# achraf-15/neural_image_compression

Hardware: AMD Instinct MI355X
Metric: images/sec (256x256 RGB, batch 32) fwd+bwd (higher is better)
Workload: dtype f32; 1 GPU; cfg2: JointAutoregressiveHierarchical(M=192,K=1) fwd+rd_loss(lambda=0.01)+bwd+Adam, 32x3x256x256 per GPU, fp32; global_batch=32, parallelism=dp1, step=eager (autograd)

## Files before the change

### include/lic.h

```cpp
#ifndef LIC_H
#define LIC_H

#include <stddef.h>
#include <stdint.h>

#ifdef __cplusplus
extern "C" {
#endif

#define LIC_ABI_VERSION 4

typedef void* lic_stream_t;

enum lic_status {
  LIC_OK = 0,
  LIC_ERR_INVALID = -1,
  LIC_ERR_UNSUPPORTED = -2,
  LIC_ERR_LAUNCH = -3,
  LIC_ERR_WORKSPACE = -4
};

enum lic_epilogue {
  LIC_EPI_NONE = 0,
  LIC_EPI_LEAKY = 1,
// ... 143 lines not shown
                    const float* x_hat, const float* x, int64_t nx, int32_t B, int64_t num_pixels,
                    float lambda_rd, float* out, void* workspace, size_t workspace_bytes,
                    lic_stream_t stream);
int lic_rd_loss_bwd(const float* x_hat, const float* x, int64_t ny, int64_t nz, int64_t nx,
                    int32_t B, int64_t num_pixels, float lambda_rd, const float* gl, float* dlogp_y,
                    float* dlogp_z, float* dx_hat, lic_stream_t stream);
int lic_rd_loss_fwd_lam(const float* logp_y, int64_t ny, const float* logp_z, int64_t nz, const float* x_hat, const float* x,
                        int64_t nx, int32_t B, int64_t num_pixels, const float* lambda_img, float* out, void* workspace,
                        size_t workspace_bytes, lic_stream_t stream);
int lic_rd_loss_bwd_lam(const float* x_hat, const float* x, int64_t ny, int64_t nz, int64_t nx, int32_t B,
                        int64_t num_pixels, const float* lambda_img, const float* gl, float* dlogp_y, float* dlogp_z,
                        float* dx_hat, lic_stream_t stream);

int64_t lic_packed_weight_bf16_elems(int32_t taps, int32_t K, int32_t N);
int lic_pack_weight_bf16(const float* src, void* dst, int32_t taps, int32_t K, int32_t N, int64_t s_tap,
                         int64_t s_k, int64_t s_n, lic_stream_t stream);
int lic_igemm_bf16(const lic_igemm_desc* d, int32_t out_f32, lic_stream_t stream);
size_t lic_igemm_bf16_workspace_bytes(const lic_igemm_desc* d);
int lic_igemm_bf16_fused_gdn_supported(int32_t Cin, int32_t Cout);
int lic_stem_gdn_bf16_supported(int32_t Cin, int32_t Cout, int32_t kh, int32_t kw, int32_t stride, int32_t pad);
int64_t lic_stem_weight_bf16_elems(int32_t Cout);
int lic_pack_stem_weight_bf16(const float* w, void* dst, int32_t Cout, lic_stream_t stream);
int lic_stem_gdn_bf16(const float* x, const void* w_packed, const float* bias, const void* gamma_packed,
                      const float* beta_eff, void* y, void* conv_out, void* norm, int32_t B, int32_t H, int32_t W,
                      int32_t Cout, int32_t inverse, lic_stream_t stream);
int lic_pack_weight_bf16_kperm(const float* src, void* dst, int32_t taps, int32_t K, int32_t N, int64_t s_tap,
                               int64_t s_k, int64_t s_n, lic_stream_t stream);
int lic_igemm_bf16_kernel_name(const lic_igemm_desc* d, char* buf, size_t n);
int lic_wgrad_bf16_kernel_name(const lic_wgrad_desc* d, char* buf, size_t n);
size_t lic_wgrad_bf16_workspace_bytes(const lic_wgrad_desc* d);
int lic_wgrad_bf16(const lic_wgrad_desc* d, void* workspace, size_t workspace_bytes, lic_stream_t stream);
int lic_im2col_bf16(const float* x, void* col, int32_t B, int32_t H, int32_t W, int32_t C, int32_t Ho,
                    int32_t Wo, int32_t kh, int32_t kw, int32_t stride, int32_t pad, int32_t Kpad,
                    lic_stream_t stream);
int lic_col2im_bf16(const void* col, const float* bias, float* out, int32_t B, int32_t Hi, int32_t Wi,
                    int32_t C, int32_t Ho, int32_t Wo, int32_t kh, int32_t kw, int32_t stride, int32_t pad,
                    int32_t Kpad, lic_stream_t stream);
int lic_gdn_bwd_bf16_supported(int32_t C);
int64_t lic_gdn_bwd_bf16_partial_rows(int64_t P);
int lic_gdn_bwd_bf16(const void* g, const void* x, const void* norm, const void* gamma_packed, void* dx, void* t,
                     float* colsum_t_partial, float* colsum_dx_partial, int64_t P, int32_t C, int32_t inverse,
                     lic_stream_t stream);
int lic_gdn_bwd_bf16_recompute(const void* g, const void* x, const void* gamma_packed, const void* gammaT_packed,
                               const float* beta_eff, void* dx, void* t, float* colsum_t_partial,
                               float* colsum_dx_partial, int64_t P, int32_t C, int32_t inverse, lic_stream_t stream);
int lic_colsum2_bf16(const void* in_a, const void* in_b, int64_t ld, int64_t P, int32_t C, float scale, float* out_a,
                     float* out_b, void* workspace, size_t workspace_bytes, lic_stream_t stream);
size_t lic_colsum_bf16_workspace_bytes(int64_t P, int32_t C);
int lic_colsum_bf16(const void* in, int64_t ld, int64_t P, int32_t C, float scale, float* out,
                    void* workspace, size_t workspace_bytes, lic_stream_t stream);
int lic_leaky_bwd_bf16(const void* y, const void* dy, void* dx, int64_t n, float slope, lic_stream_t stream);
int lic_gdn_dnorm_bf16(const void* g, const void* x, const void* norm, void* t, int64_t n, int32_t inverse,
                       lic_stream_t stream);
int lic_quantize_bf16(const float* v, const float* u, float* out, void* v_bf16, void* out_bf16, int64_t n,
                      int32_t training, lic_stream_t stream);
int lic_quantize_anchor_bf16(const float* v, const float* u, float* out, float* out_anchor, void* v_bf16, void* out_bf16,
                             void* anchor_bf16, int32_t B, int32_t h, int32_t w, int32_t C, int32_t training,
                             lic_stream_t stream);

int lic_gdn_supported(int32_t C);
int lic_gdn_fwd(const float* x, const float* gammaT_packed, const float* beta_eff, const float* res, float* y,
                float* norm, int64_t P, int32_t C, int32_t inverse, lic_stream_t stream);
int64_t lic_gdn_bwd_partial_rows(int64_t P);
int lic_gdn_bwd(const float* g, const float* x, const float* norm, const float* gamma_packed, float* dx, float* t,
                float* colsum_t_partial, float* colsum_dx_partial, int64_t P, int32_t C, int32_t inverse,
                lic_stream_t stream);

int lic_factorized_cdf_tables(const float* fe_params, int32_t C, int32_t lo, int32_t S, uint32_t* out,
                              lic_stream_t stream);
int lic_gmm_cdf_tables(const float* params, int64_t P, int32_t M, int32_t K, int32_t W, int32_t* center,
                       uint32_t* out, lic_stream_t stream);

#define LIC_CTX_AUTO 0
#define LIC_CTX_VECTOR 1
#define LIC_CTX_ELEMENT 2
int lic_ctx_gather(const float* y, int64_t y_batch, int64_t y_row, int64_t y_pix, int64_t y_origin, int32_t B,
                   int32_t h, int32_t w, int32_t M, const int32_t* taps, int32_t nt, int32_t slice_rows,
                   const int64_t* pix, int64_t n, float* win, const float* psi, int32_t Cpsi, float* comb,
                   int64_t comb_ld, int32_t path, lic_stream_t stream);

#define LIC_CTX_IMAGE_WORDS 8
#define LIC_CTX_IMAGE_Y_BASE 0
#define LIC_CTX_IMAGE_Y_ROW 1
#define LIC_CTX_IMAGE_Y_ORIGIN 2
#define LIC_CTX_IMAGE_PSI_BASE 3
#define LIC_CTX_IMAGE_H 4
#define LIC_CTX_IMAGE_W 5
#define LIC_CTX_IMAGE_R 6
int lic_ctx_gather_ragged(const float* y, int64_t y_len, int64_t y_pix, const int64_t* images, int32_t nimg, int32_t M,
                          const int32_t* taps, int32_t nt, const int64_t* row_image, const int64_t* row_pix,
                          int64_t rows, float* win, const float* psi, int64_t psi_len, int32_t Cpsi, float* comb,
                          int64_t comb_ld, int32_t path, lic_stream_t stream);

#define LIC_MAX_LAYERS 4
typedef struct lic_ctx_layer {
  float* win;
  float* comb;
  int64_t comb_ld;
  int32_t c0, M;
} lic_ctx_layer;
int lic_ctx_gather_layers(const float* y, int64_t y_batch, int64_t y_row, int64_t y_pix, int64_t y_origin, int32_t B,
                          int32_t h, int32_t w, const int32_t* taps, int32_t nt, int32_t slice_rows, const int64_t* pix,
                          int64_t n, const float* psi, int32_t Cpsi, const lic_ctx_layer* layers, int32_t L,
                          int32_t path, lic_stream_t stream);

int lic_ctx_gather_layers_ragged(const float* y, int64_t y_len, int64_t y_pix, const int64_t* images, int32_t nimg,
                                 const int32_t* taps, int32_t nt, const int64_t* row_image, const int64_t* row_pix,
                                 int64_t rows, const float* psi, int64_t psi_len, int32_t Cpsi,
                                 const lic_ctx_layer* layers, int32_t L, int32_t path, lic_stream_t stream);

#define LIC_RANS_LANES 64
#define LIC_RANS_STATE_WORDS 67
#define LIC_RANS_ERR_RANGE 1u
#define LIC_RANS_ERR_STREAM 2u
int lic_rans_decode_step(const uint8_t* streams, const int64_t* stream_off, const int64_t* stream_bytes,
                         const uint32_t* escapes, const int64_t* esc_off, uint32_t* state, const uint32_t* tables,
                         const int32_t* center, int32_t B, int32_t n, int32_t M, int32_t W, const int64_t* dest,
                         float* ypad, int64_t pixels, lic_stream_t stream);

#define LIC_RANS_MAX_GROUPS 8
int lic_rans_decode_step_groups(const uint8_t* streams, const int64_t* stream_off, const int64_t* stream_bytes,
                                const uint32_t* escapes, const int64_t* esc_off, uint32_t* state,
                                const uint32_t* tables, const int32_t* center, int32_t B, int32_t G, int32_t n,
                                int32_t M, int32_t W, const int64_t* dest, float* ypad, int64_t pixels,
                                lic_stream_t stream);

int lic_rans_decode_step_ragged(const uint8_t* streams, const int64_t* stream_off, const int64_t* stream_bytes,
                                const uint32_t* escapes, const int64_t* esc_off, uint32_t* state,
                                const uint32_t* tables, const int32_t* center, const int32_t* seg, int32_t nimg,
                                int32_t G, int64_t total_rows, int32_t M, int32_t W, const int64_t* dest, float* ypad,
                                const int64_t* y_base, const int64_t* pixels, int64_t ypad_len, lic_stream_t stream);

typedef struct lic_rans_layer {
  const uint32_t* tables;
  const int32_t* center;
  int32_t c0, M;
} lic_rans_layer;
int lic_rans_decode_step_layers(const uint8_t* streams, const int64_t* stream_off, const int64_t* stream_bytes,
                                const uint32_t* escapes, const int64_t* esc_off, uint32_t* state,
                                const lic_rans_layer* layers, int32_t L, int32_t B, int32_t G, int32_t n, int32_t W,
                                const int64_t* dest, float* ypad, int64_t pixels, int64_t y_pix, lic_stream_t stream);

int lic_rans_decode_step_layers_ragged(const uint8_t* streams, const int64_t* stream_off, const int64_t* stream_bytes,
                                       const uint32_t* escapes, const int64_t* esc_off, uint32_t* state,
                                       const lic_rans_layer* layers, int32_t L, const int32_t* seg, int32_t nimg,
                                       int32_t G, int64_t total_rows, int32_t W, const int64_t* dest, float* ypad,
                                       const int64_t* y_base, const int64_t* pixels, int64_t ypad_len, int64_t y_pix,
                                       lic_stream_t stream);

int lic_rans_encode_pick(const uint32_t* tables, const int32_t* center, const int32_t* y, const int64_t* order,
                         int32_t B, int64_t P, int32_t M, int32_t W, uint32_t* sf, uint32_t* exc, uint32_t* state,
                         lic_stream_t stream);
int lic_rans_encode(const uint32_t* sf, const uint32_t* exc, const int64_t* step_len, int64_t nsteps, int32_t B,
                    int64_t nsym, uint8_t* words, int64_t slot, uint32_t* esc_out, uint32_t* state,
                    lic_stream_t stream);

int lic_rans_encode_groups(const uint32_t* sf, const uint32_t* exc, const int64_t* step_len, int64_t nsteps,
                           int32_t B, int32_t G, int64_t nsym, uint8_t* words, int64_t slot, uint32_t* esc_out,
                           int64_t esc_cap, uint32_t* state, lic_stream_t stream);

#define LIC_RANS_IMAGE_WORDS 4
#define LIC_RANS_IMAGE_ROW0 0
#define LIC_RANS_IMAGE_P 1
#define LIC_RANS_IMAGE_STEP0 2
#define LIC_RANS_IMAGE_NSTEPS 3
#define LIC_RANS_BLOCK_WORDS 4
#define LIC_RANS_BLOCK_WORD_OFF 0
#define LIC_RANS_BLOCK_SLOT 1
#define LIC_RANS_BLOCK_ESC_OFF 2
#define LIC_RANS_BLOCK_ESC_CAP 3
int lic_rans_encode_pick_ragged(const uint32_t* tables, const int32_t* center, const int32_t* y, int64_t total_rows,
                                const int64_t* images, int32_t nimg, const int64_t* row_image, const int64_t* order,
                                int32_t M, int32_t W, uint32_t* sf, uint32_t* exc, uint32_t* state,
                                lic_stream_t stream);
int lic_rans_encode_ragged(const uint32_t* sf, const uint32_t* exc, const int64_t* step_len, int64_t steps_len,
                           const int64_t* images, const int64_t* blocks, int32_t nimg, int32_t G, int64_t total_rows,
                           int32_t M, uint8_t* words, int64_t words_len, uint32_t* esc_out, int64_t esc_len,
                           uint32_t* state, lic_stream_t stream);

#define LIC_RANS_Z_AUTO 0
#define LIC_RANS_Z_RESIDENT 1
#define LIC_RANS_Z_GLOBAL 2
#define LIC_RANS_Z_LDS_BYTES 65536
#define LIC_RANS_Z_MAX_S 4096
#define LIC_RANS_Z_MAX_M 65535
int lic_rans_z_pick(const uint32_t* tables, int32_t M, int32_t lo, int32_t S, const int32_t* z, int64_t n, uint32_t* sf,
                    uint32_t* exc, uint32_t* err, lic_stream_t stream);
int lic_rans_z_decode_path(int32_t M, int32_t S);
int lic_rans_z_decode(const uint8_t* streams, const int64_t* stream_off, const int64_t* stream_bytes,
                      const uint32_t* escapes, const int64_t* esc_off, uint32_t* state, const uint32_t* tables,
                      int32_t M, int32_t lo, int32_t S, int32_t nimg, int32_t G, const int64_t* nsym,
                      const int64_t* z_base, float* z, int64_t z_len, int32_t path, lic_stream_t stream);

size_t lic_msssim_workspace_bytes(int32_t B, int32_t C, int32_t H, int32_t W);
int lic_msssim(const float* x, const float* y, int32_t B, int32_t C, int32_t H, int32_t W, int64_t sb,
               int64_t sc, int64_t sh, int64_t sw, float data_range, float* out, float* level_out,
               void* workspace, size_t workspace_bytes, lic_stream_t stream);
size_t lic_msssim_bwd_workspace_bytes(int32_t B, int32_t C, int32_t H, int32_t W);
int lic_msssim_bwd(const float* x, const float* y, int32_t B, int32_t C, int32_t H, int32_t W, int64_t sb,
                   int64_t sc, int64_t sh, int64_t sw, float data_range, const float* level_out,
                   const void* fwd_workspace, size_t fwd_workspace_bytes, const float* gout, float* dx,
                   void* workspace, size_t workspace_bytes, lic_stream_t stream);

int lic_u8_to_f32(const uint8_t* in, float* out, int64_t n, lic_stream_t stream);
size_t lic_tensor_stats_workspace_bytes(void);
int lic_tensor_stats(const float* x, int64_t n, int32_t nbins, float lo, float hi, double* stats,
                     uint64_t* hist, void* workspace, size_t workspace_bytes, lic_stream_t stream);

enum lic_window_border { LIC_WINDOW_ZERO = 0, LIC_WINDOW_REPLICATE = 1, LIC_WINDOW_REFLECT = 2 };
typedef struct lic_window_job {
  int64_t src_offset;
  int32_t Hs, Ws;
  int32_t y0, x0;
  int32_t flags;
  int32_t reserved;
} lic_window_job;
int lic_window_u8_to_f32(const uint8_t* pool, const lic_window_job* jobs_device, int32_t B, int32_t h, int32_t w,
                         int32_t C, int32_t border, float* out, lic_stream_t stream);
int lic_window_f32(const float* src, int64_t sb, int64_t sc, int64_t sh, int64_t sw, int32_t B, int32_t C,
                   int32_t Hs, int32_t Ws, int32_t y0, int32_t x0, int32_t h, int32_t w, int32_t border, float* out,
                   lic_stream_t stream);

typedef struct lic_resample_job {
  int64_t src_offset;
  int32_t Hs, Ws;
  int32_t Hn, Wn;
  int32_t y0, x0;
  int32_t flags;
  int32_t reserved;
} lic_resample_job;
int lic_resample_u8_to_f32(const uint8_t* pool, const lic_resample_job* jobs_device, int32_t B, int32_t h, int32_t w,
                           int32_t C, float* out, lic_stream_t stream);

enum lic_prep_kind { LIC_PREP_PACK_F32 = 0, LIC_PREP_PACK_BF16 = 1, LIC_PREP_MAP = 2, LIC_PREP_MASK_INPLACE = 3,
                     LIC_PREP_PACK_BF16_KPERM = 4 ,
                     LIC_PREP_PACK_BF16_STEM = 5   };
typedef struct lic_prep_job {
  const float* src;
  void* dst;
  const float* mask;
  int64_t s_tap, s_kq, s_kr, s_nq, s_nr;
  int32_t kind;
  int32_t taps, K, N, kdiv, ndiv;
  int32_t transform;
  float bound, pedestal;
  int32_t cpt, npad, tiled, v4, block0, nblocks;
  int64_t total;
} lic_prep_job;
int64_t lic_prep_plan(lic_prep_job* jobs, int32_t njobs);
int lic_prep_run(const lic_prep_job* jobs_device, int32_t njobs, int64_t total_blocks, lic_stream_t stream);

typedef struct lic_adam_job {
  float* p;
  const float* g;
  float* m;
  float* v;
  int64_t n;
  int32_t block0, nblocks;
} lic_adam_job;
int64_t lic_adam_plan(lic_adam_job* jobs, int32_t njobs);
int lic_adam_run(const lic_adam_job* jobs_device, int32_t njobs, int64_t total_blocks, const float* const* grads_host,
                 double lr, double beta1, double beta2, double eps, double weight_decay, double bias_correction1,
                 double bias_correction2, lic_stream_t stream);

int lic_grad_norm_partial(const lic_adam_job* jobs_device, int32_t njobs, int64_t total_blocks,
                          const float* const* grads_host, double* partials, lic_stream_t stream);
int lic_grad_norm_finish(const double* partials, int64_t nparts, double max_norm, int32_t count_skip, float* clip_state,
                         lic_stream_t stream);
int lic_adam_run_scaled(const lic_adam_job* jobs_device, int32_t njobs, int64_t total_blocks,
                        const float* const* grads_host, double lr, double beta1, double beta2, double eps,
                        double weight_decay, double bias_correction1, double bias_correction2, const float* clip_state,
                        int32_t skip_nonfinite, lic_stream_t stream);

int lic_adam_run_ema(const lic_adam_job* jobs_device, int32_t njobs, int64_t total_blocks,
                     const float* const* grads_host, double lr, double beta1, double beta2, double eps,
                     double weight_decay, double bias_correction1, double bias_correction2, float* const* ema_device,
                     double ema_weight, const float* clip_state, int32_t skip_nonfinite, lic_stream_t stream);
int lic_swap_run(const lic_adam_job* jobs_device, int32_t njobs, int64_t total_blocks, float* const* ema_device,
                 lic_stream_t stream);

enum { LIC_REDUCE_SLABS = 0, LIC_REDUCE_COLUMNS = 1 };
enum { LIC_REDUCE_EPI_NONE = 0, LIC_REDUCE_EPI_REPARAM = 1 };
#define LIC_REDUCE_MAX_JOBS 32
typedef struct lic_reduce_job {
  const float* src;
  float* dst;
  const float* param;
  int64_t sm, smr, sn, snr, stap;
  int32_t kind, epilogue;
  int32_t splitk, ntaps, Cm, Cn, Mvalid, Nvalid, mdiv, ndiv;
  float scale, bound;
  int32_t block0, nblocks;
} lic_reduce_job;
int lic_wgrad_bf16_partial(const lic_wgrad_desc* d, void* workspace, size_t workspace_bytes, lic_reduce_job* job,
                           lic_stream_t stream);
int lic_colsum_bf16_partial(const void* in, int64_t ld, int64_t P, int32_t C, float scale, float* out, void* workspace,
                            size_t workspace_bytes, lic_reduce_job* job, lic_stream_t stream);
int lic_colsum2_bf16_partial(const void* in_a, const void* in_b, int64_t ld, int64_t P, int32_t C, float scale,
                             float* out_a, float* out_b, void* workspace, size_t workspace_bytes, lic_reduce_job* jobs2,
                             lic_stream_t stream);
int lic_leaky_bwd_colsum_bf16(const void* y, const void* dy, void* dx, int64_t P, int32_t C, float slope, float* out,
                              void* workspace, size_t workspace_bytes, lic_reduce_job* job, lic_stream_t stream);
int lic_reduce_batch(const lic_reduce_job* jobs, int32_t njobs, lic_stream_t stream);

int lic_head_convt_bf16_supported(int32_t Cin, int32_t Cout, int32_t kh, int32_t kw, int32_t stride, int32_t pad,
                                  int32_t out_pad);
int lic_head_convt_bf16(const void* x, const void* w_packed, const float* bias, float* out, int32_t B, int32_t Hi,
                        int32_t Wi, int32_t Cin, lic_stream_t stream);
int lic_stem_conv_bf16(const float* x, const void* w_packed, const float* bias, void* y, int32_t B, int32_t H, int32_t W,
                       int32_t Cout, lic_stream_t stream);

typedef struct lic_plan lic_plan;
int lic_plan_create(void* hip_graph, lic_plan** out);
int lic_plan_info(const lic_plan* plan, int64_t* info);
int lic_plan_replay(lic_plan* plan, lic_stream_t main, const lic_stream_t* sides, int32_t n_sides);
int lic_plan_tune(lic_plan* plan, lic_stream_t main, const lic_stream_t* sides, int32_t n_sides, double* result);
int lic_plan_dag(const lic_plan* plan, int64_t cap_ops, int64_t cap_edges, int64_t* sizes, int32_t* pred_ptr,
                 int32_t* pred_idx, int32_t* kind, int32_t* flags, double* us);
int lic_plan_commands(lic_plan* plan, int32_t n_sides, int64_t cap, int64_t* n_cmds, int32_t* cmds);
int lic_plan_sched_host(int64_t n_ops, const int32_t* pred_ptr, const int32_t* pred_idx, const double* us,
                        const int32_t* flags, int32_t mode, int32_t ns, double wide_min_us, int32_t n_sides,
                        int64_t cap, int64_t* n_cmds, int32_t* cmds, int64_t* info);
void lic_plan_destroy(lic_plan* plan);
const char* lic_plan_last_error(void);

int lic_version(void);
int lic_last_hip_error(void);
const char* lic_arch(void);

#ifdef __cplusplus
}
#endif
#endif
```

### neural_image_compression_amd/_lib.py

```python
from __future__ import annotations

import ctypes as C
import os

_HERE = os.path.dirname(os.path.abspath(__file__))
LIB_PATH = os.path.join(_HERE, "liblic_hip.so")

EPI_NONE, EPI_LEAKY, EPI_MUL_LEAKY_MASK, EPI_GDN, EPI_IGDN, EPI_GDN_BWD, EPI_IGDN_BWD, EPI_CONV_GDN, EPI_CONV_IGDN = range(9)
FE_NPARAM = 43

_vp, _i32, _i64, _f32, _sz = C.c_void_p, C.c_int32, C.c_int64, C.c_float, C.c_size_t


class IgemmDesc(C.Structure):
    _fields_ = [("in_", _vp), ("w", _vp), ("bias", _vp), ("out", _vp), ("out2", _vp), ("aux", _vp),
                ("aux2", _vp), ("aux3", _vp), ("res", _vp),
                ("in_ld", _i64), ("out_ld", _i64), ("out2_ld", _i64), ("aux_ld", _i64),
                ("aux2_ld", _i64), ("aux3_ld", _i64), ("res_ld", _i64),
                ("B", _i32), ("Hi", _i32), ("Wi", _i32), ("Cin", _i32),
                ("Ho", _i32), ("Wo", _i32), ("Cout", _i32),
                ("kh", _i32), ("kw", _i32), ("stride", _i32), ("pad", _i32),
                ("transposed", _i32), ("prologue", _i32), ("epilogue", _i32),
                ("tap_mask", C.c_uint32), ("slope", _f32), ("workspace", _vp), ("workspace_bytes", _sz),
                ("out3", _vp), ("out3_ld", _i64),
                ("force_bm", _i32), ("force_tn", _i32), ("force_split", _i32), ("reserved0", _i32)]


class WgradDesc(C.Structure):
    _fields_ = [("p", _vp), ("g", _vp), ("dst", _vp),
                ("p_ld", _i64), ("g_ld", _i64),
                ("dst_sm", _i64), ("dst_sn", _i64), ("dst_stap", _i64),
                ("B", _i32), ("Hs", _i32), ("Ws", _i32), ("Cp", _i32),
                ("Hl", _i32), ("Wl", _i32), ("Cg", _i32),
                ("kh", _i32), ("kw", _i32), ("stride", _i32), ("pad", _i32),
                ("g_is_row", _i32), ("sq_p", _i32), ("sq_g", _i32), ("scale", _f32),
                ("force_tm", _i32), ("force_tn", _i32), ("force_split", _i32)]


PREP_PACK_F32, PREP_PACK_BF16, PREP_MAP, PREP_MASK_INPLACE, PREP_PACK_BF16_KPERM, PREP_PACK_BF16_STEM = range(6)


class PrepJob(C.Structure):
    _fields_ = [("src", _vp), ("dst", _vp), ("mask", _vp),
                ("s_tap", _i64), ("s_kq", _i64), ("s_kr", _i64), ("s_nq", _i64), ("s_nr", _i64),
                ("kind", _i32), ("taps", _i32), ("K", _i32), ("N", _i32), ("kdiv", _i32), ("ndiv", _i32),
                ("transform", _i32), ("bound", _f32), ("pedestal", _f32),
                ("cpt", _i32), ("npad", _i32), ("tiled", _i32), ("v4", _i32), ("block0", _i32), ("nblocks", _i32),
                ("total", _i64)]


REDUCE_SLABS, REDUCE_COLUMNS = 0, 1
REDUCE_EPI_NONE, REDUCE_EPI_REPARAM = 0, 1
REDUCE_MAX_JOBS = 32


class ReduceJob(C.Structure):
    _fields_ = [("src", _vp), ("dst", _vp), ("param", _vp),
                ("sm", _i64), ("smr", _i64), ("sn", _i64), ("snr", _i64), ("stap", _i64),
                ("kind", _i32), ("epilogue", _i32),
                ("splitk", _i32), ("ntaps", _i32), ("Cm", _i32), ("Cn", _i32), ("Mvalid", _i32), ("Nvalid", _i32),
                ("mdiv", _i32), ("ndiv", _i32),
                ("scale", _f32), ("bound", _f32),
                ("block0", _i32), ("nblocks", _i32)]


class AdamJob(C.Structure):
    _fields_ = [("p", _vp), ("g", _vp), ("m", _vp), ("v", _vp), ("n", _i64), ("block0", _i32), ("nblocks", _i32)]


RANS_LANES, RANS_STATE_WORDS, RANS_MAX_GROUPS = 64, 67, 8

CTX_AUTO, CTX_VECTOR, CTX_ELEMENT = range(3)
CTX_IMAGE_WORDS = 8
RANS_IMAGE_WORDS = RANS_BLOCK_WORDS = 4

RANS_Z_AUTO, RANS_Z_RESIDENT, RANS_Z_GLOBAL = range(3)
RANS_Z_MAX_S, RANS_Z_MAX_M, RANS_Z_LDS_BYTES = 4096, 65535, 65536

GAIN_SCALE, GAIN_NOISE, GAIN_ROUND = range(3)
GAIN_SLAB_PIXELS, GAIN_SLAB_ROWS = 32, 4
GAIN_ROWS_MAX_TABLES = 4

MAX_LAYERS = 4


class CtxLayer(C.Structure):
    _fields_ = [("win", _vp), ("comb", _vp), ("comb_ld", _i64), ("c0", _i32), ("M", _i32)]


class RansLayer(C.Structure):
    _fields_ = [("tables", _vp), ("center", _vp), ("c0", _i32), ("M", _i32)]


WINDOW_ZERO, WINDOW_REPLICATE, WINDOW_REFLECT = range(3)
WINDOW_FLIP = 1


class WindowJob(C.Structure):
    _fields_ = [("src_offset", _i64), ("Hs", _i32), ("Ws", _i32), ("y0", _i32), ("x0", _i32), ("flags", _i32),
                ("reserved", _i32)]


class ResampleJob(C.Structure):
    _fields_ = [("src_offset", _i64), ("Hs", _i32), ("Ws", _i32), ("Hn", _i32), ("Wn", _i32), ("y0", _i32),
                ("x0", _i32), ("flags", _i32), ("reserved", _i32)]


SIGNATURES = {
    "lic_igemm": (C.c_int, [C.POINTER(IgemmDesc), _vp]),
    "lic_igemm_workspace_bytes": (_sz, [C.POINTER(IgemmDesc)]),
    "lic_igemm_kernel_name": (C.c_int, [C.POINTER(IgemmDesc), C.c_char_p, _sz]),
    "lic_wgrad_stage": (C.c_int, [C.POINTER(WgradDesc), _vp, _sz, _i32, _vp]),
    "lic_wgrad_kernel_name": (C.c_int, [C.POINTER(WgradDesc), C.c_char_p, _sz]),
    "lic_igemm_plan": (C.c_int, [C.POINTER(IgemmDesc), C.POINTER(_i32), C.POINTER(_i32), C.POINTER(_i64)]),
    "lic_igemm_tile_order": (C.c_int, [C.POINTER(IgemmDesc), _vp, _i64, C.POINTER(_i64), C.POINTER(_i32),
                                       C.POINTER(_i32)]),
    "lic_packed_weight_floats": (_i64, [_i32, _i32, _i32]),
    "lic_pack_weight": (C.c_int, [_vp, _vp, _i32, _i32, _i32, _i64, _i64, _i64, _vp]),
    "lic_wgrad_workspace_bytes": (_sz, [C.POINTER(WgradDesc)]),
    "lic_wgrad": (C.c_int, [C.POINTER(WgradDesc), _vp, _sz, _vp]),
    "lic_wgrad_plan": (C.c_int, [C.POINTER(WgradDesc), C.POINTER(_i32), C.POINTER(_i32), C.POINTER(_i32)]),
    "lic_colsum_workspace_bytes": (_sz, [_i64, _i32]),
    "lic_colsum": (C.c_int, [_vp, _i64, _i64, _i32, _f32, _vp, _vp, _sz, _vp]),
    "lic_permute3": (C.c_int, [_vp, _vp, _i32, _i32, _i32, _i64, _i64, _i64, _i64, _i64, _i64, _vp]),
    "lic_im2col": (C.c_int, [_vp, _vp] + [_i32] * 11 + [_vp]),
    "lic_col2im": (C.c_int, [_vp, _vp, _vp] + [_i32] * 11 + [_vp]),
    "lic_mul_inplace": (C.c_int, [_vp, _vp, _i64, _vp]),
    "lic_leaky_bwd": (C.c_int, [_vp, _vp, _vp, _i64, _f32, _vp]),
    "lic_gdn_reparam": (C.c_int, [_vp, _vp, _i64, _f32, _f32, _vp]),
    "lic_gdn_reparam_bwd": (C.c_int, [_vp, _vp, _vp, _i64, _f32, _vp]),
    "lic_gdn_reparam_bwd2": (C.c_int, [_vp, _vp, _vp, _i64, _f32, _vp, _vp, _vp, _i64, _f32, _vp]),
    "lic_gdn_dnorm": (C.c_int, [_vp, _vp, _vp, _vp, _i64, _i32, _vp]),
    "lic_quantize": (C.c_int, [_vp, _vp, _vp, _i64, _i32, _vp]),
    "lic_quantize_anchor": (C.c_int, [_vp, _vp, _vp, _vp, _i32, _i32, _i32, _i32, _i32, _vp]),
    "lic_anchor_add": (C.c_int, [_vp, _vp, _vp, _i32, _i32, _i32, _i32, _vp]),
    "lic_gain_quantize": (C.c_int, [_vp, _vp, _vp, _i64] + [_vp] * 6 + [_i32] * 5 + [_vp]),
    "lic_gain_bwd_workspace_bytes": (_sz, [_i32, _i64, _i32]),
    "lic_gain_bwd": (C.c_int, [_vp, _vp, _i64] + [_vp] * 5 + [_i32] * 4 + [_vp, _sz, _vp]),
    "lic_gain_rows_fwd": (C.c_int, [_vp] * 4 + [_i32] * 4 + [_vp]),
    "lic_gain_rows_bwd": (C.c_int, [_vp] * 7 + [_i32] * 4 + [_vp]),
    "lic_entropy_params_fwd": (C.c_int, [_vp, _vp, _i64, _i32, _i32, _vp]),
    "lic_entropy_params_bwd": (C.c_int, [_vp, _vp, _vp, _vp, _i64, _i32, _i32, _vp]),
    "lic_gmm_likelihood_fwd": (C.c_int, [_vp, _vp, _vp, _vp, _i64, _i32, _i32, _f32, _vp]),
    "lic_gmm_likelihood_bwd": (C.c_int, [_vp, _vp, _vp, _vp, _vp, _vp, _i64, _i32, _i32, _f32, _vp]),
    "lic_factorized_fwd": (C.c_int, [_vp, _vp, _vp, _vp, _i64, _i32, _f32, _vp]),
    "lic_factorized_bwd": (C.c_int, [_vp, _vp, _vp, _vp, _vp, _vp, _i64, _i32, _f32, _vp]),
    "lic_factorized_channel_logits": (C.c_int, [_vp, _i32, _vp, _vp, _i64, _vp]),
    "lic_fe_pack": (C.c_int, [_vp, _vp, _i32, _vp]),
    "lic_fe_unpack": (C.c_int, [_vp, _vp, _i32, _vp]),
    "lic_rd_loss_workspace_bytes": (_sz, [_i32]),
    "lic_rd_loss_fwd": (C.c_int, [_vp, _i64, _vp, _i64, _vp, _vp, _i64, _i32, _i64, _f32, _vp, _vp, _sz, _vp]),
    "lic_rd_loss_bwd": (C.c_int, [_vp, _vp, _i64, _i64, _i64, _i32, _i64, _f32, _vp, _vp, _vp, _vp, _vp]),
    "lic_rd_loss_fwd_lam": (C.c_int, [_vp, _i64, _vp, _i64, _vp, _vp, _i64, _i32, _i64, _vp, _vp, _vp, _sz, _vp]),
    "lic_rd_loss_bwd_lam": (C.c_int, [_vp, _vp, _i64, _i64, _i64, _i32, _i64, _vp, _vp, _vp, _vp, _vp, _vp]),
    "lic_packed_weight_bf16_elems": (_i64, [_i32, _i32, _i32]),
    "lic_pack_weight_bf16": (C.c_int, [_vp, _vp, _i32, _i32, _i32, _i64, _i64, _i64, _vp]),
    "lic_pack_weight_bf16_kperm": (C.c_int, [_vp, _vp, _i32, _i32, _i32, _i64, _i64, _i64, _vp]),
    "lic_igemm_bf16": (C.c_int, [C.POINTER(IgemmDesc), _i32, _vp]),
    "lic_igemm_bf16_kernel_name": (C.c_int, [C.POINTER(IgemmDesc), C.c_char_p, _sz]),
    "lic_igemm_bf16_workspace_bytes": (_sz, [C.POINTER(IgemmDesc)]),
    "lic_igemm_bf16_fused_gdn_supported": (C.c_int, [_i32, _i32]),
    "lic_stem_gdn_bf16_supported": (C.c_int, [_i32] * 6),
    "lic_stem_weight_bf16_elems": (C.c_int64, [_i32]),
    "lic_pack_stem_weight_bf16": (C.c_int, [_vp, _vp, _i32, _vp]),
    "lic_stem_gdn_bf16": (C.c_int, [_vp] * 8 + [_i32] * 5 + [_vp]),
    "lic_wgrad_bf16_kernel_name": (C.c_int, [C.POINTER(WgradDesc), C.c_char_p, _sz]),
    "lic_wgrad_bf16_workspace_bytes": (_sz, [C.POINTER(WgradDesc)]),
    "lic_wgrad_bf16": (C.c_int, [C.POINTER(WgradDesc), _vp, _sz, _vp]),
    "lic_im2col_bf16": (C.c_int, [_vp, _vp] + [_i32] * 11 + [_vp]),
    "lic_col2im_bf16": (C.c_int, [_vp, _vp, _vp] + [_i32] * 11 + [_vp]),
    "lic_colsum_bf16_workspace_bytes": (_sz, [_i64, _i32]),
    "lic_colsum_bf16": (C.c_int, [_vp, _i64, _i64, _i32, _f32, _vp, _vp, _sz, _vp]),
    "lic_quantize_bf16": (C.c_int, [_vp, _vp, _vp, _vp, _vp, _i64, _i32, _vp]),
    "lic_quantize_anchor_bf16": (C.c_int, [_vp] * 7 + [_i32] * 5 + [_vp]),
    "lic_wgrad_bf16_partial": (C.c_int, [C.POINTER(WgradDesc), _vp, _sz, C.POINTER(ReduceJob), _vp]),
    "lic_colsum_bf16_partial": (C.c_int, [_vp, _i64, _i64, _i32, _f32, _vp, _vp, _sz, C.POINTER(ReduceJob), _vp]),
    "lic_colsum2_bf16_partial": (C.c_int, [_vp, _vp, _i64, _i64, _i32, _f32, _vp, _vp, _vp, _sz, C.POINTER(ReduceJob), _vp]),
    "lic_reduce_batch": (C.c_int, [C.POINTER(ReduceJob), _i32, _vp]),
    "lic_colsum2_bf16": (C.c_int, [_vp, _vp, _i64, _i64, _i32, _f32, _vp, _vp, _vp, _sz, _vp]),
    "lic_gdn_dnorm_bf16": (C.c_int, [_vp, _vp, _vp, _vp, _i64, _i32, _vp]),
    "lic_gdn_bwd_bf16_supported": (C.c_int, [_i32]),
    "lic_gdn_bwd_bf16_partial_rows": (_i64, [_i64]),
    "lic_gdn_bwd_bf16": (C.c_int, [_vp, _vp, _vp, _vp, _vp, _vp, _vp, _vp, _i64, _i32, _i32, _vp]),
    "lic_gdn_bwd_bf16_recompute": (C.c_int, [_vp, _vp, _vp, _vp, _vp, _vp, _vp, _vp, _vp, _i64, _i32, _i32, _vp]),
    "lic_leaky_bwd_bf16": (C.c_int, [_vp, _vp, _vp, _i64, _f32, _vp]),
    "lic_leaky_bwd_colsum_bf16": (C.c_int, [_vp, _vp, _vp, _i64, _i32, _f32, _vp, _vp, _sz, C.POINTER(ReduceJob), _vp]),
    "lic_igemm_fused_gdn_supported": (C.c_int, [_i32, _i32]),
    "lic_igemm_fused_gdn_preferred": (C.c_int, [C.POINTER(IgemmDesc)]),
    "lic_gdn_supported": (C.c_int, [_i32]),
    "lic_gdn_fwd": (C.c_int, [_vp, _vp, _vp, _vp, _vp, _vp, _i64, _i32, _i32, _vp]),
    "lic_gdn_bwd_partial_rows": (_i64, [_i64]),
    "lic_gdn_bwd": (C.c_int, [_vp, _vp, _vp, _vp, _vp, _vp, _vp, _vp, _i64, _i32, _i32, _vp]),
    "lic_factorized_cdf_tables": (C.c_int, [_vp, _i32, _i32, _i32, _vp, _vp]),
    "lic_gmm_cdf_tables": (C.c_int, [_vp, _i64, _i32, _i32, _i32, _vp, _vp, _vp]),
    "lic_rans_decode_step": (C.c_int, [_vp] * 8 + [_i32] * 4 + [_vp, _vp, _i64, _vp]),
    "lic_rans_encode_pick": (C.c_int, [_vp] * 4 + [_i32, _i64, _i32, _i32] + [_vp] * 4),
    "lic_rans_encode": (C.c_int, [_vp] * 3 + [_i64, _i32, _i64, _vp, _i64, _vp, _vp, _vp]),
    "lic_rans_decode_step_groups": (C.c_int, [_vp] * 8 + [_i32] * 5 + [_vp, _vp, _i64, _vp]),
    "lic_rans_encode_groups": (C.c_int, [_vp] * 3 + [_i64, _i32, _i32, _i64, _vp, _i64, _vp, _i64, _vp, _vp]),
    "lic_rans_encode_pick_ragged": (C.c_int, [_vp] * 3 + [_i64, _vp, _i32, _vp, _vp, _i32, _i32] + [_vp] * 4),
    "lic_rans_encode_ragged": (C.c_int, [_vp] * 3 + [_i64, _vp, _vp, _i32, _i32, _i64, _i32, _vp, _i64, _vp, _i64,
                                         _vp, _vp]),
    "lic_ctx_gather": (C.c_int, [_vp] + [_i64] * 4 + [_i32] * 4 + [_vp, _i32, _i32, _vp, _i64, _vp, _vp, _i32, _vp, _i64,
                                 _i32, _vp]),
    "lic_ctx_gather_ragged": (C.c_int, [_vp, _i64, _i64, _vp, _i32, _i32, _vp, _i32, _vp, _vp, _i64, _vp, _vp, _i64, _i32,
                                        _vp, _i64, _i32, _vp]),
    "lic_rans_decode_step_ragged": (C.c_int, [_vp] * 9 + [_i32, _i32, _i64, _i32, _i32, _vp, _vp, _vp, _vp, _i64, _vp]),
    "lic_ctx_gather_layers": (C.c_int, [_vp] + [_i64] * 4 + [_i32] * 3 + [_vp, _i32, _i32, _vp, _i64, _vp, _i32,
                                        C.POINTER(CtxLayer), _i32, _i32, _vp]),
    "lic_rans_decode_step_layers": (C.c_int, [_vp] * 6 + [C.POINTER(RansLayer)] + [_i32] * 5 + [_vp, _vp, _i64, _i64,
                                                                                                 _vp]),
    "lic_ctx_gather_layers_ragged": (C.c_int, [_vp, _i64, _i64, _vp, _i32, _vp, _i32, _vp, _vp, _i64, _vp, _i64, _i32,
                                               C.POINTER(CtxLayer), _i32, _i32, _vp]),
    "lic_rans_decode_step_layers_ragged": (C.c_int, [_vp] * 6 + [C.POINTER(RansLayer), _i32, _vp, _i32, _i32, _i64,
                                                                 _i32, _vp, _vp, _vp, _vp, _i64, _i64, _vp]),
    "lic_rans_z_pick": (C.c_int, [_vp, _i32, _i32, _i32, _vp, _i64, _vp, _vp, _vp, _vp]),
    "lic_rans_z_decode_path": (C.c_int, [_i32, _i32]),
    "lic_rans_z_decode": (C.c_int, [_vp] * 7 + [_i32] * 5 + [_vp, _vp, _vp, _i64, _i32, _vp]),
    "lic_msssim_workspace_bytes": (_sz, [_i32, _i32, _i32, _i32]),
    "lic_msssim": (C.c_int, [_vp, _vp, _i32, _i32, _i32, _i32, _i64, _i64, _i64, _i64, _f32, _vp, _vp, _vp, _sz,
                             _vp]),
    "lic_msssim_bwd_workspace_bytes": (_sz, [_i32, _i32, _i32, _i32]),
    "lic_msssim_bwd": (C.c_int, [_vp, _vp, _i32, _i32, _i32, _i32, _i64, _i64, _i64, _i64, _f32, _vp, _vp, _sz, _vp,
                                 _vp, _vp, _sz, _vp]),
    "lic_u8_to_f32": (C.c_int, [_vp, _vp, _i64, _vp]),
    "lic_window_u8_to_f32": (C.c_int, [_vp, _vp, _i32, _i32, _i32, _i32, _i32, _vp, _vp]),
    "lic_window_f32": (C.c_int, [_vp, _i64, _i64, _i64, _i64] + [_i32] * 9 + [_vp, _vp]),
    "lic_resample_u8_to_f32": (C.c_int, [_vp, _vp, _i32, _i32, _i32, _i32, _vp, _vp]),
    "lic_tensor_stats_workspace_bytes": (_sz, []),
    "lic_tensor_stats": (C.c_int, [_vp, _i64, _i32, _f32, _f32, _vp, _vp, _vp, _sz, _vp]),
    "lic_prep_plan": (_i64, [C.POINTER(PrepJob), _i32]),
    "lic_prep_run": (C.c_int, [_vp, _i32, _i64, _vp]),
    "lic_adam_plan": (_i64, [C.POINTER(AdamJob), _i32]),
    "lic_adam_run": (C.c_int, [_vp, _i32, _i64, _vp] + [C.c_double] * 7 + [_vp]),
    "lic_grad_norm_partial": (C.c_int, [_vp, _i32, _i64, _vp, _vp, _vp]),
    "lic_grad_norm_finish": (C.c_int, [_vp, _i64, C.c_double, _i32, _vp, _vp]),
    "lic_adam_run_scaled": (C.c_int, [_vp, _i32, _i64, _vp] + [C.c_double] * 7 + [_vp, _i32, _vp]),
    "lic_adam_run_ema": (C.c_int, [_vp, _i32, _i64, _vp] + [C.c_double] * 7 + [_vp, C.c_double, _vp, _i32, _vp]),
    "lic_swap_run": (C.c_int, [_vp, _i32, _i64, _vp, _vp]),
    "lic_head_convt_bf16_supported": (C.c_int, [_i32] * 7),
    "lic_head_convt_bf16": (C.c_int, [_vp, _vp, _vp, _vp, _i32, _i32, _i32, _i32, _vp]),
    "lic_stem_conv_bf16": (C.c_int, [_vp, _vp, _vp, _vp, _i32, _i32, _i32, _i32, _vp]),
    "lic_plan_create": (C.c_int, [_vp, C.POINTER(C.c_void_p)]),
    "lic_plan_info": (C.c_int, [_vp, C.POINTER(C.c_int64)]),
    "lic_plan_replay": (C.c_int, [_vp, _vp, C.POINTER(C.c_void_p), _i32]),
    "lic_plan_tune": (C.c_int, [_vp, _vp, C.POINTER(C.c_void_p), _i32, C.POINTER(C.c_double)]),
    "lic_plan_dag": (C.c_int, [_vp, _i64, _i64, C.POINTER(C.c_int64), _vp, _vp, _vp, _vp, _vp]),
    "lic_plan_commands": (C.c_int, [_vp, _i32, _i64, C.POINTER(C.c_int64), _vp]),
    "lic_plan_sched_host": (C.c_int, [_i64, _vp, _vp, _vp, _vp, _i32, _i32, C.c_double, _i32, _i64,
                                      C.POINTER(C.c_int64), _vp, _vp]),
    "lic_plan_destroy": (None, [_vp]),
    "lic_plan_last_error": (C.c_char_p, []),
    "lic_version": (C.c_int, []),
    "lic_last_hip_error": (C.c_int, []),
    "lic_arch": (C.c_char_p, []),
}

_lib = None


class LicError(RuntimeError):
    pass


def load():
    global _lib
    if _lib is None:
        if not os.path.exists(LIB_PATH):
            raise LicError(
                f"{LIB_PATH} not found: the HIP extension is not built. Run "
                "`python -c 'import __graft_entry__ as g; g.build()'` (or make -C "
                "neural_image_compression_amd/csrc). There is no CPU fallback.")
        lib = C.CDLL(LIB_PATH)
        for name, (res, args) in SIGNATURES.items():
            fn = getattr(lib, name)
            fn.restype = res
            fn.argtypes = args
        _lib = lib
    return _lib


_STATUS = {-1: "LIC_ERR_INVALID", -2: "LIC_ERR_UNSUPPORTED", -3: "LIC_ERR_LAUNCH", -4: "LIC_ERR_WORKSPACE"}


def check(rc: int, what: str):
    if rc != 0:
        extra = f" (hipError {load().lic_last_hip_error()})" if rc == -3 else ""
        raise LicError(f"{what} failed: {_STATUS.get(rc, rc)}{extra}")
```

### neural_image_compression_amd/csrc/lic_elementwise.hip

```cpp
#include "lic_common.h"
#include "lic_patch.h"

#define EW_BLOCK 256
static bool al16(const void* p) { return (reinterpret_cast<uintptr_t>(p) & 15) == 0; }

__global__ __launch_bounds__(EW_BLOCK) void permute3_kernel(const float* src, float* dst, int n0, int n1,
                                                            int n2, long s0, long s1, long s2, long d0,
                                                            long d1, long d2) {
  const long total = (long)n0 * n1 * n2;
  for (long i = (long)blockIdx.x * EW_BLOCK + threadIdx.x; i < total; i += (long)gridDim.x * EW_BLOCK) {
    const int k = (int)(i % n2);
    const long t = i / n2;
    const int j = (int)(t % n1);
    const int a = (int)(t / n1);
    dst[a * d0 + j * d1 + k * d2] = src[a * s0 + j * s1 + k * s2];
  }
}
LIC_EXPORT int lic_permute3(const float* src, float* dst, int32_t n0, int32_t n1, int32_t n2,
                            int64_t s0, int64_t s1, int64_t s2, int64_t d0, int64_t d1, int64_t d2,
                            lic_stream_t stream) {
  if (!src || !dst || n0 <= 0 || n1 <= 0 || n2 <= 0) return LIC_ERR_INVALID;
  const long total = (long)n0 * n1 * n2;
  hipLaunchKernelGGL(permute3_kernel, dim3(ew_grid(total, EW_BLOCK)), dim3(EW_BLOCK), 0,
                     (hipStream_t)stream, src, dst, n0, n1, n2, (long)s0, (long)s1, (long)s2, (long)d0,
                     (long)d1, (long)d2);
  return lic_check_launch();
}

__global__ __launch_bounds__(EW_BLOCK) void im2col_kernel(const float* x, float* col, int B, int H, int W,
                                                          int C, int Ho, int Wo, int kh, int kw,
                                                          int stride, int pad, int Kpad) {
  const long total = (long)B * Ho * Wo * Kpad;
  const int K = kh * kw * C;
  for (long i = (long)blockIdx.x * EW_BLOCK + threadIdx.x; i < total; i += (long)gridDim.x * EW_BLOCK) {
    const int k = (int)(i % Kpad);
    const long pix = i / Kpad;
    float v = 0.0f;
    if (k < K) {
      const int c = k % C, tap = k / C;
      const int r = tap / kw, s = tap - r * kw;
      const int ow = (int)(pix % Wo);
      const long t = pix / Wo;
      const int oh = (int)(t % Ho);
      const int b = (int)(t / Ho);
      const int ih = oh * stride - pad + r, iw = ow * stride - pad + s;
      if (ih >= 0 && iw >= 0 && ih < H && iw < W) v = x[(((long)b * H + ih) * W + iw) * C + c];
    }
    col[i] = v;
  }
}
LIC_EXPORT int lic_im2col(const float* x, float* col, int32_t B, int32_t H, int32_t W, int32_t C,
                          int32_t Ho, int32_t Wo, int32_t kh, int32_t kw, int32_t stride, int32_t pad,
                          int32_t Kpad, lic_stream_t stream) {
  if (!x || !col || B <= 0 || H <= 0 || W <= 0 || C <= 0 || Ho <= 0 || Wo <= 0 || Kpad < kh * kw * C)
    return LIC_ERR_INVALID;
  const long total = (long)B * Ho * Wo * Kpad;
  if (Kpad <= LIC_PATCH_MAXK && Kpad % 4 == 0 && total / 4 < 0x7FFFFFFFL && al16(col) && kh < 256 && kw < 256 &&
      C < 256 && (long)H * W * C < 0x7FFFFFFFL)
    hipLaunchKernelGGL((im2col_vec_kernel<float, 4>), dim3(ew_grid(total / 4, 256)), dim3(256), 0,
                       (hipStream_t)stream, x, col, (unsigned)((long)B * Ho * Wo), H, W, C, Ho, Wo, kh, kw, stride, pad,
                       Kpad);
  else
    hipLaunchKernelGGL(im2col_kernel, dim3(ew_grid(total, EW_BLOCK)), dim3(EW_BLOCK), 0,
                       (hipStream_t)stream, x, col, B, H, W, C, Ho, Wo, kh, kw, stride, pad, Kpad);
  return lic_check_launch();
}

__global__ __launch_bounds__(EW_BLOCK) void col2im_kernel(const float* col, const float* bias, float* out,
                                                          int B, int Hi, int Wi, int C, int Ho, int Wo,
                                                          int kh, int kw, int stride, int pad, int Kpad) {
  const long total = (long)B * Ho * Wo * C;
  for (long i = (long)blockIdx.x * EW_BLOCK + threadIdx.x; i < total; i += (long)gridDim.x * EW_BLOCK) {
    const int c = (int)(i % C);
    const long pix = i / C;
    const int ox = (int)(pix % Wo);
    const long t = pix / Wo;
    const int oy = (int)(t % Ho);
    const int b = (int)(t / Ho);
    float v = bias ? bias[c] : 0.0f;
    for (int r = 0; r < kh; ++r) {
      const int nh = oy + pad - r;
      if (nh < 0 || (nh % stride) != 0) continue;
      const int ih = nh / stride;
      if (ih >= Hi) continue;
      for (int s = 0; s < kw; ++s) {
        const int nw = ox + pad - s;
        if (nw < 0 || (nw % stride) != 0) continue;
        const int iw = nw / stride;
        if (iw >= Wi) continue;
        v += col[(((long)b * Hi + ih) * Wi + iw) * Kpad + (r * kw + s) * C + c];
      }
    }
    out[i] = v;
  }
}
LIC_EXPORT int lic_col2im(const float* col, const float* bias, float* out, int32_t B, int32_t Hi,
                          int32_t Wi, int32_t C, int32_t Ho, int32_t Wo, int32_t kh, int32_t kw,
                          int32_t stride, int32_t pad, int32_t Kpad, lic_stream_t stream) {
  if (!col || !out || B <= 0 || Hi <= 0 || Wi <= 0 || C <= 0 || Ho <= 0 || Wo <= 0 || stride < 1 ||
      Kpad < kh * kw * C)
    return LIC_ERR_INVALID;
  const long total = (long)B * Ho * Wo * C;
  if (total < 0x7FFFFFFFL && (long)B * Hi * Wi < 0x7FFFFFFFL)
    hipLaunchKernelGGL((col2im_fast_kernel<float>), dim3(ew_grid(total, 256)), dim3(256), 0, (hipStream_t)stream, col,
                       bias, out, (unsigned)total, Hi, Wi, C, Ho, Wo, kh, kw, stride, pad, Kpad);
  else
    hipLaunchKernelGGL(col2im_kernel, dim3(ew_grid(total, EW_BLOCK)), dim3(EW_BLOCK), 0,
                       (hipStream_t)stream, col, bias, out, B, Hi, Wi, C, Ho, Wo, kh, kw, stride, pad, Kpad);
  return lic_check_launch();
}

#define CS_MAXCHUNK 256
__global__ __launch_bounds__(256) void colsum_stage1(const float* in, long ld, long P, int C, float* part,
                                                     int nchunk, int vec) {
  __shared__ float red[16][64 + 4];
  const int cg = threadIdx.x & 15, ry = threadIdx.x >> 4;
  const int c = blockIdx.x * 64 + cg * 4;
  f32x4 acc = {0.f, 0.f, 0.f, 0.f};
  if (c < C) {
    if (vec) {
      for (long pr = (long)blockIdx.y * 16 + ry; pr < P; pr += (long)nchunk * 16)
        acc += *reinterpret_cast<const f32x4*>(in + pr * ld + c);
    } else {
      for (long pr = (long)blockIdx.y * 16 + ry; pr < P; pr += (long)nchunk * 16)
#pragma unroll
        for (int e = 0; e < 4; ++e)
          if (c + e < C) acc[e] += in[pr * ld + c + e];
    }
  }
#pragma unroll
  for (int e = 0; e < 4; ++e) red[ry][cg * 4 + e] = acc[e];
  __syncthreads();
  if (threadIdx.x < 64) {
    const int cc = blockIdx.x * 64 + threadIdx.x;
    float s = 0.0f;
#pragma unroll
    for (int r = 0; r < 16; ++r) s += red[r][threadIdx.x];
    if (cc < C) part[(long)blockIdx.y * C + cc] = s;
  }
}
__global__ __launch_bounds__(256) void colsum3_stage1(const float* in, long P, float* part, int nchunk) {
  __shared__ float red[4][3];
  const long ngroup = P / 4;
  f32x4 a0 = {0.f, 0.f, 0.f, 0.f}, a1 = a0, a2 = a0;
  for (long g = (long)blockIdx.x * 256 + threadIdx.x; g < ngroup; g += (long)nchunk * 256) {
    const f32x4* q = reinterpret_cast<const f32x4*>(in + g * 12);
    a0 += q[0];
    a1 += q[1];
    a2 += q[2];
  }
  float c0 = a0[0] + a0[3] + a1[2] + a2[1];
  float c1 = a0[1] + a1[0] + a1[3] + a2[2];
  float c2 = a0[2] + a1[1] + a2[0] + a2[3];
  if (blockIdx.x == 0 && threadIdx.x == 0)
    for (long r = ngroup * 4; r < P; ++r) {
      c0 += in[r * 3];
      c1 += in[r * 3 + 1];
      c2 += in[r * 3 + 2];
    }
  c0 = wave_sum(c0);
  c1 = wave_sum(c1);
  c2 = wave_sum(c2);
  const int w = threadIdx.x >> 6;
  if ((threadIdx.x & 63) == 0) {
    red[w][0] = c0;
    red[w][1] = c1;
    red[w][2] = c2;
  }
  __syncthreads();
  if (threadIdx.x < 3)
    part[(long)blockIdx.x * 3 + threadIdx.x] =
        (red[0][threadIdx.x] + red[1][threadIdx.x]) + (red[2][threadIdx.x] + red[3][threadIdx.x]);
}
__global__ __launch_bounds__(256) void colsum_stage2(const float* part, int C, int nchunk, float scale,
                                                     float* out) {
  __shared__ double red[16][17];
  const int cx = threadIdx.x & 15, ly = threadIdx.x >> 4;
  const int c = blockIdx.x * 16 + cx;
  double acc = 0.0;
  if (c < C)
    for (int y = ly; y < nchunk; y += 16) acc += (double)part[(long)y * C + c];
  red[ly][cx] = acc;
  __syncthreads();
  if (ly == 0 && c < C) {
    double t = 0.0;
#pragma unroll
    for (int q = 0; q < 16; ++q) t += red[q][cx];
    out[c] = (float)(t * (double)scale);
  }
}
static int colsum_chunks(int64_t P) {
  int64_t n = cdiv64(P, 16 * 8);
  if (n > CS_MAXCHUNK) n = CS_MAXCHUNK;
  if (n < 1) n = 1;
  return (int)n;
}
LIC_EXPORT size_t lic_colsum_workspace_bytes(int64_t P, int32_t C) {
  if (P <= 0 || C <= 0) return 0;
  return (size_t)colsum_chunks(P) * C * sizeof(float);
}
LIC_EXPORT int lic_colsum(const float* in, int64_t ld, int64_t P, int32_t C, float scale, float* out,
                          void* workspace, size_t workspace_bytes, lic_stream_t stream) {
  if (!in || !out || !workspace || P <= 0 || C <= 0) return LIC_ERR_INVALID;
  const int nchunk = colsum_chunks(P);
  if (workspace_bytes < (size_t)nchunk * C * sizeof(float)) return LIC_ERR_WORKSPACE;
  hipStream_t s = (hipStream_t)stream;
  const int vec = (C % 4 == 0) && (ld % 4 == 0) && al16(in);
  if (C == 3 && ld == 3 && al16(in))
    hipLaunchKernelGGL(colsum3_stage1, dim3(nchunk), dim3(256), 0, s, in, (long)P, (float*)workspace, nchunk);
  else
    hipLaunchKernelGGL(colsum_stage1, dim3((C + 63) / 64, nchunk), dim3(256), 0, s, in, (long)ld, (long)P, C,
                       (float*)workspace, nchunk, vec);
  int rc = lic_check_launch();
  if (rc != LIC_OK) return rc;
  hipLaunchKernelGGL(colsum_stage2, dim3((C + 15) / 16), dim3(256), 0, s, (const float*)workspace, C,
                     nchunk, scale, out);
  return lic_check_launch();
}

template <typename F>
__global__ __launch_bounds__(EW_BLOCK) void ew_kernel(long n, F f) {
  for (long i = (long)blockIdx.x * EW_BLOCK + threadIdx.x; i < n; i += (long)gridDim.x * EW_BLOCK) f(i);
}
template <typename F>
static int ew_launch(long n, lic_stream_t stream, F f) {
  if (n <= 0) return LIC_OK;
  hipLaunchKernelGGL((ew_kernel<F>), dim3(ew_grid(n, EW_BLOCK)), dim3(EW_BLOCK), 0, (hipStream_t)stream, n, f);
  return lic_check_launch();
}
template <typename F4, typename F1>
static int ew_launch_vec(long n, bool can_vec, lic_stream_t stream, F4 f4, F1 f1) {
  if (n <= 0) return LIC_OK;
  if (!can_vec) return ew_launch(n, stream, f1);
  const long n4 = n / 4;
  int rc = ew_launch(n4, stream, f4);
  if (rc != LIC_OK) return rc;
  const long tail0 = n4 * 4;
  if (tail0 < n) return ew_launch(n - tail0, stream, [=] __device__(long i) { f1(tail0 + i); });
  return LIC_OK;
}

LIC_EXPORT int lic_mul_inplace(float* w, const float* mask, int64_t n, lic_stream_t stream) {
  if (!w || !mask || n < 0) return LIC_ERR_INVALID;
  return ew_launch(n, stream, [=] __device__(long i) { w[i] *= mask[i]; });
}

LIC_EXPORT int lic_leaky_bwd(const float* y, const float* dy, float* dx, int64_t n, float slope,
                             lic_stream_t stream) {
  if (!y || !dy || !dx || n < 0) return LIC_ERR_INVALID;
  return ew_launch_vec(
      n, al16(y) && al16(dy) && al16(dx), stream,
      [=] __device__(long i) {
        const f32x4 a = reinterpret_cast<const f32x4*>(y)[i], g = reinterpret_cast<const f32x4*>(dy)[i];
        f32x4 o;
#pragma unroll
        for (int e = 0; e < 4; ++e) o[e] = a[e] > 0.0f ? g[e] : g[e] * slope;
        reinterpret_cast<f32x4*>(dx)[i] = o;
      },
      [=] __device__(long i) { dx[i] = y[i] > 0.0f ? dy[i] : dy[i] * slope; });
}

LIC_EXPORT int lic_gdn_reparam(const float* p, float* out, int64_t n, float bound, float pedestal,
                               lic_stream_t stream) {
  if (!p || !out || n < 0) return LIC_ERR_INVALID;
  return ew_launch(n, stream, [=] __device__(long i) { out[i] = lic_reparam(p[i], bound, pedestal); });
}
LIC_EXPORT int lic_gdn_reparam_bwd(const float* p, const float* dout, float* dp, int64_t n, float bound,
                                   lic_stream_t stream) {
  if (!p || !dout || !dp || n < 0) return LIC_ERR_INVALID;
  return ew_launch(n, stream, [=] __device__(long i) {
    const float v = p[i] > bound ? p[i] : bound;
    const float g = dout[i] * 2.0f * v;
    dp[i] = (p[i] >= bound || g < 0.0f) ? g : 0.0f;
  });
}

LIC_EXPORT int lic_gdn_reparam_bwd2(const float* pb, const float* dob, float* dpb, int64_t nb, float bound_b,
                                    const float* pg, const float* dog, float* dpg, int64_t ng, float bound_g,
                                    lic_stream_t stream) {
  if (nb < 0 || ng < 0 || (nb > 0 && (!pb || !dob || !dpb)) || (ng > 0 && (!pg || !dog || !dpg))) return LIC_ERR_INVALID;
  if (nb + ng == 0) return LIC_OK;
  return ew_launch(nb + ng, stream, [=] __device__(long i) {
    const bool isb = i < nb;
    const long j = isb ? i : i - nb;
    const float pv = isb ? pb[j] : pg[j], dv = isb ? dob[j] : dog[j], bound = isb ? bound_b : bound_g;
    const float v = pv > bound ? pv : bound;
    const float g = dv * 2.0f * v;
    (isb ? dpb : dpg)[j] = (pv >= bound || g < 0.0f) ? g : 0.0f;
  });
}

__device__ __forceinline__ float gdn_t1(float g, float x, float n, int inverse) {
  const float rs = __builtin_amdgcn_rsqf(n);
  return inverse ? 0.5f * g * x * rs : -0.5f * g * x * rs * (rs * rs);
}
LIC_EXPORT int lic_gdn_dnorm(const float* g, const float* x, const float* norm, float* t, int64_t n,
                             int32_t inverse, lic_stream_t stream) {
  if (!g || !x || !norm || !t || n < 0) return LIC_ERR_INVALID;
  return ew_launch_vec(
      n, al16(g) && al16(x) && al16(norm) && al16(t), stream,
      [=] __device__(long i) {
        const f32x4 gv = reinterpret_cast<const f32x4*>(g)[i], xv = reinterpret_cast<const f32x4*>(x)[i],
                    nv = reinterpret_cast<const f32x4*>(norm)[i];
        f32x4 o;
#pragma unroll
        for (int e = 0; e < 4; ++e) o[e] = gdn_t1(gv[e], xv[e], nv[e], inverse);
        reinterpret_cast<f32x4*>(t)[i] = o;
      },
      [=] __device__(long i) { t[i] = gdn_t1(g[i], x[i], norm[i], inverse); });
}

LIC_EXPORT int lic_quantize(const float* v, const float* u, float* out, int64_t n, int32_t training,
                            lic_stream_t stream) {
  if (!v || !out || n < 0 || (training && !u)) return LIC_ERR_INVALID;
  if (training) return ew_launch(n, stream, [=] __device__(long i) { out[i] = v[i] + (u[i] - 0.5f); });
  return ew_launch(n, stream, [=] __device__(long i) { out[i] = rintf(v[i]); });
}

__device__ __forceinline__ bool lic_is_anchor(long pix, int h, int w) {
  const long row = pix / w;
  return (((row % h) + (pix - row * w)) & 1) == 0;
}
LIC_EXPORT int lic_quantize_anchor(const float* v, const float* u, float* out, float* out_anchor, int32_t B, int32_t h,
                                   int32_t w, int32_t C, int32_t training, lic_stream_t stream) {
  if (!v || !out || !out_anchor || B <= 0 || h <= 0 || w <= 0 || C <= 0 || (training && !u)) return LIC_ERR_INVALID;
  const long n = (long)B * h * w * C;
  return ew_launch(n, stream, [=] __device__(long i) {
    const float q = training ? v[i] + (u[i] - 0.5f) : rintf(v[i]);
    out[i] = q;
    out_anchor[i] = lic_is_anchor(i / C, h, w) ? q : 0.0f;
  });
}
LIC_EXPORT int lic_anchor_add(const float* g, const float* g_anchor, float* out, int32_t B, int32_t h, int32_t w, int32_t C,
                              lic_stream_t stream) {
  if (!g || !g_anchor || !out || B <= 0 || h <= 0 || w <= 0 || C <= 0) return LIC_ERR_INVALID;
  const long n = (long)B * h * w * C;
  return ew_launch_vec(
      n, C % 4 == 0 && al16(g) && al16(g_anchor) && al16(out), stream,
      [=] __device__(long i) {
        const f32x4 a = reinterpret_cast<const f32x4*>(g)[i];
        f32x4 b = {};
        if (lic_is_anchor(4 * i / C, h, w)) b = reinterpret_cast<const f32x4*>(g_anchor)[i];
        reinterpret_cast<f32x4*>(out)[i] = a + b;
      },
      [=] __device__(long i) { out[i] = g[i] + (lic_is_anchor(i / C, h, w) ? g_anchor[i] : 0.0f); });
}

#define LIC_MAXK 8
LIC_EXPORT int lic_entropy_params_fwd(const float* raw, float* out, int64_t P, int32_t M, int32_t K,
                                      lic_stream_t stream) {
  if (!raw || !out || P <= 0 || M <= 0 || K < 1 || K > LIC_MAXK) return LIC_ERR_INVALID;
  const long CH = (long)(K == 1 ? 2 : 3) * K * M;
  const long T = (long)K * M;
  return ew_launch(P * M, stream, [=] __device__(long i) {
    const long pix = i / M;
    const int m = (int)(i - pix * M);
    const float* r = raw + pix * CH;
    float* o = out + pix * CH;
    if (K == 1) {
      o[m] = r[m];
      o[M + m] = lic_softplus(r[M + m]) + 1e-6f;
    } else {
      float mx = -INFINITY;
      for (int k = 0; k < K; ++k) mx = fmaxf(mx, r[k * M + m]);
      float den = 0.0f;
      for (int k = 0; k < K; ++k) den += expf(r[k * M + m] - mx);
      for (int k = 0; k < K; ++k) {
        o[k * M + m] = expf(r[k * M + m] - mx) / den;
        o[T + k * M + m] = r[T + k * M + m];
        o[2 * T + k * M + m] = lic_softplus(r[2 * T + k * M + m]) + 1e-6f;
      }
    }
  });
}
LIC_EXPORT int lic_entropy_params_bwd(const float* raw, const float* out, const float* dout, float* draw,
                                      int64_t P, int32_t M, int32_t K, lic_stream_t stream) {
  if (!raw || !out || !dout || !draw || P <= 0 || M <= 0 || K < 1 || K > LIC_MAXK) return LIC_ERR_INVALID;
  const long CH = (long)(K == 1 ? 2 : 3) * K * M;
  const long T = (long)K * M;
  return ew_launch(P * M, stream, [=] __device__(long i) {
    const long pix = i / M;
    const int m = (int)(i - pix * M);
    const float* r = raw + pix * CH;
    const float* o = out + pix * CH;
    const float* g = dout + pix * CH;
    float* d = draw + pix * CH;
    if (K == 1) {
      d[m] = g[m];
      d[M + m] = g[M + m] * lic_softplus_grad(r[M + m]);
    } else {
      float dot = 0.0f;
      for (int k = 0; k < K; ++k) dot += g[k * M + m] * o[k * M + m];
      for (int k = 0; k < K; ++k) {
        d[k * M + m] = o[k * M + m] * (g[k * M + m] - dot);
        d[T + k * M + m] = g[T + k * M + m];
        d[2 * T + k * M + m] = g[2 * T + k * M + m] * lic_softplus_grad(r[2 * T + k * M + m]);
      }
    }
  });
}

__device__ __forceinline__ float gauss_cdf(float t) { return 0.5f * (1.0f + erff(t / 1.41421356237309515f)); }
__device__ __forceinline__ float gauss_pdf(float t) { return 0.398942280401432678f * expf(-0.5f * t * t); }

LIC_EXPORT int lic_gmm_likelihood_fwd(const float* x, const float* params, float* p, float* logp, int64_t P,
                                      int32_t M, int32_t K, float bound, lic_stream_t stream) {
  if (!x || !params || !p || !logp || P <= 0 || M <= 0 || K < 1 || K > LIC_MAXK) return LIC_ERR_INVALID;
  const long CH = (long)(K == 1 ? 2 : 3) * K * M;
  const long T = (long)K * M;
  return ew_launch(P * M, stream, [=] __device__(long i) {
    const long pix = i / M;
    const int m = (int)(i - pix * M);
    const float* q = params + pix * CH;
    const float xv = x[i];
    float acc = 0.0f;
    for (int k = 0; k < K; ++k) {
      const float mu = (K == 1) ? q[m] : q[T + k * M + m];
      const float sg = (K == 1) ? q[M + m] : q[2 * T + k * M + m];
      const float up = (xv + 0.5f - mu) / sg, lo = (xv - 0.5f - mu) / sg;
      const float mass = gauss_cdf(up) - gauss_cdf(lo);
      acc = (K == 1) ? mass : acc + q[k * M + m] * mass;
    }
    const float pc = acc > bound ? acc : bound;
    p[i] = pc;
    logp[i] = logf(pc);
  });
}
LIC_EXPORT int lic_gmm_likelihood_bwd(const float* x, const float* params, const float* dp,
                                      const float* dlogp, float* dx, float* dparams, int64_t P, int32_t M,
                                      int32_t K, float bound, lic_stream_t stream) {
  if (!x || !params || !dx || !dparams || P <= 0 || M <= 0 || K < 1 || K > LIC_MAXK) return LIC_ERR_INVALID;
  const long CH = (long)(K == 1 ? 2 : 3) * K * M;
  const long T = (long)K * M;
  return ew_launch(P * M, stream, [=] __device__(long i) {
    const long pix = i / M;
    const int m = (int)(i - pix * M);
    const float* q = params + pix * CH;
    float* dq = dparams + pix * CH;
    const float xv = x[i];
    float acc = 0.0f;
    for (int k = 0; k < K; ++k) {
      const float mu = (K == 1) ? q[m] : q[T + k * M + m];
      const float sg = (K == 1) ? q[M + m] : q[2 * T + k * M + m];
      const float up = (xv + 0.5f - mu) / sg, lo = (xv - 0.5f - mu) / sg;
      const float mass = gauss_cdf(up) - gauss_cdf(lo);
      acc = (K == 1) ? mass : acc + q[k * M + m] * mass;
    }
    const float pc = acc > bound ? acc : bound;
    float g = 0.0f;
    if (dp) g += dp[i];
    if (dlogp) g += dlogp[i] / pc;
    if (!(acc >= bound)) g = 0.0f;
    float dxa = 0.0f;
    for (int k = 0; k < K; ++k) {
      const float mu = (K == 1) ? q[m] : q[T + k * M + m];
      const float sg = (K == 1) ? q[M + m] : q[2 * T + k * M + m];
      const float up = (xv + 0.5f - mu) / sg, lo = (xv - 0.5f - mu) / sg;
      const float pu = gauss_pdf(up), pl = gauss_pdf(lo);
      const float wk = (K == 1) ? 1.0f : q[k * M + m];
      const float gm = g * wk;
      if (K == 1) {
        dq[m] = -gm * (pu - pl) / sg;
        dq[M + m] = -gm * (pu * up - pl * lo) / sg;
      } else {
        dq[k * M + m] = g * (gauss_cdf(up) - gauss_cdf(lo));
        dq[T + k * M + m] = -gm * (pu - pl) / sg;
        dq[2 * T + k * M + m] = -gm * (pu * up - pl * lo) / sg;
      }
      dxa += gm * (pu - pl) / sg;
    }
    dx[i] = dxa;
  });
}

__constant__ int FE_MOFF[4] = {0, 3, 12, 21};
__constant__ int FE_BOFF[4] = {24, 27, 30, 33};
__constant__ int FE_FOFF[3] = {34, 37, 40};
__constant__ int FE_DIN[4] = {1, 3, 3, 3};
__constant__ int FE_DOUT[4] = {3, 3, 3, 1};

struct FeTrace {
  float h[4][3];
  float pre[4][3];
};
__device__ __forceinline__ float fe_logits(const float* T, float v, FeTrace* tr) {
  float h[3] = {v, 0.0f, 0.0f};
#pragma unroll
  for (int i = 0; i < 4; ++i) {
    const int din = (i == 0) ? 1 : 3, dout = (i == 3) ? 1 : 3;
    const int mo = (i == 0) ? 0 : (i == 1) ? 3 : (i == 2) ? 12 : 21;
    const int bo = 24 + 3 * i;
    float pre[3] = {0.0f, 0.0f, 0.0f};
#pragma unroll
    for (int o = 0; o < 3; ++o)
      if (o < dout) {
        float acc = 0.0f;
#pragma unroll
        for (int k = 0; k < 3; ++k)
          if (k < din) acc += T[mo + o * din + k] * h[k];
        pre[o] = acc + T[bo + o];
      }
    if (tr) {
#pragma unroll
      for (int k = 0; k < 3; ++k) {
        tr->h[i][k] = h[k];
        tr->pre[i][k] = pre[k];
      }
    }
    if (i < 3) {
#pragma unroll
      for (int o = 0; o < 3; ++o) h[o] = pre[o] + T[34 + 3 * i + o] * tanhf(pre[o]);
    } else {
      h[0] = pre[0];
    }
  }
  return h[0];
}
__device__ __forceinline__ float fe_logits_bwd(const float* T, const float* R, const FeTrace& tr,
                                               float dlogit, float* dP) {
  float dh[3] = {dlogit, 0.0f, 0.0f};
// ... 495 lines not shown
```

### neural_image_compression_amd/csrc/lic_gemm.hip

```cpp
#include "lic_tile_map.h"
#include <stdio.h>
#include <stdlib.h>
#include <algorithm>
#include <type_traits>

thread_local int g_lic_last_hip_error = 0;

struct IgemmParams {
  const float* in;
  const float* w;
  const float* bias;
  float* out;
  float* out2;
  const float* aux;
  const float* aux2;
  const float* aux3;
  const float* res;
  float* out3;
  long in_ld, out_ld, out2_ld, aux_ld, aux2_ld, aux3_ld, res_ld, out3_ld;
  int B, Hi, Wi, Cin, Ho, Wo, Cout;
  int kw, stride, pad, transposed, prologue, epilogue;
  float slope;
  int vec;
  int vec_out;
// ... 1204 lines not shown
      load_chunk(c_begin + c + 3);
      compute(1);
      __syncthreads();
    }
    if (c < nloc) {
      compute(0);
      __syncthreads();
    }
  }
  float* slab = p.slabs + ((long)split * p.ntaps + tap) * p.row.C * p.col.C;
#pragma unroll
  for (int a = 0; a < TM; ++a)
#pragma unroll
    for (int q = 0; q < 16; ++q) {
      const int m = m0 + wm0 + a * 32 + (q & 3) + 8 * (q >> 2) + 4 * lh;
      if (m >= p.row.C) continue;
#pragma unroll
      for (int b = 0; b < TN; ++b) {
        const int n = n0 + wn0 + b * 32 + li;
        if (n < p.col.C) slab[(long)m * p.col.C + n] = acc[a][b][q];
      }
    }
}

template <int TM, int TN, bool SQB = false, bool FULL = true>
__global__ __launch_bounds__(256, (TM * TN >= 6 ? 2 : 1)) void wgrad_glds_kernel(const WgradParams p) {
  constexpr int BMt = 64 * TM, BNt = 64 * TN, NS = TM + TN;
  constexpr int WM = BMt / 2, WN = BNt / 2;
  __shared__ __attribute__((aligned(16))) float smem[2][NS][WG_BK * 64];
  const int tid = threadIdx.x, lane = tid & 63;
  const int wave = __builtin_amdgcn_readfirstlane(tid >> 6);
  const int wm0 = (wave >> 1) * WM, wn0 = (wave & 1) * WN;
  const int li = lane & 31, lh = lane >> 5;
  const WgradTile wt = wgrad_tile(p, xcd_contiguous(blockIdx.x, gridDim.x), BMt, BNt);
  const int m0 = wt.m0, n0 = wt.n0, tap = wt.tap, split = wt.split;
  const int c_begin = wt.c_begin, c_end = wt.c_end, nloc = c_end - c_begin;

  f32x16 acc[TM][TN];
#pragma unroll
  for (int a = 0; a < TM; ++a)
#pragma unroll
    for (int b = 0; b < TN; ++b)
#pragma unroll
      for (int q = 0; q < 16; ++q) acc[a][b][q] = 0.0f;

  const int kr = tid >> 4, c16 = (tid & 15) * 4;
  constexpr unsigned WG_OOB = 0x80000000u, WG_GBIAS = 0x40000000u;
  const unsigned row_ld4 = (unsigned)p.row.ld * 4u, col_ld4 = (unsigned)p.col.ld * 4u;
  const unsigned row_lin = (unsigned)kr * row_ld4 + (unsigned)c16 * 4u;
  const unsigned col_lin = (unsigned)kr * col_ld4 + (unsigned)c16 * 4u;
  const bool row_g = p.row.gathered != 0, col_g = p.col.gathered != 0;
  const unsigned g_ld4 = row_g ? row_ld4 : col_ld4;
  const unsigned HWl = (unsigned)(p.Hl * p.Wl);
  const int tap_h = wt.r - p.pad, tap_w = wt.s - p.pad;
  bool row_live[TM], col_live[TN];
#pragma unroll
  for (int j = 0; j < TM; ++j) row_live[j] = FULL || m0 + c16 + 64 * j < p.row.C;
#pragma unroll
  for (int j = 0; j < TN; ++j) col_live[j] = FULL || n0 + c16 + 64 * j < p.col.C;
  const float* const row_base = p.row.ptr + m0;
  const float* const col_base = p.col.ptr + n0;
  auto issue = [&](int c, int buf) {
    const int cc = c < c_end ? c : c_end - 1;
    const int pk0 = cc * WG_BK;
    const int b0 = fdiv(pk0, p.dHW);
    const int rem0 = pk0 - b0 * p.Hs * p.Ws;
    const int hs0 = fdiv(rem0, p.dW), ws0 = rem0 - hs0 * p.Ws;
    const long g0 = ((long)b0 * p.Hl + (hs0 * p.stride + tap_h)) * p.Wl + (ws0 * p.stride + tap_w);
    const unsigned pk = (unsigned)pk0 + (unsigned)kr;
    const int pix = pk < (unsigned)p.Ps ? (int)pk : 0;
    const int b = fdiv(pix, p.dHW);
    const int rem = pix - b * p.Hs * p.Ws;
    const int hs = fdiv(rem, p.dW), ws = rem - hs * p.Ws;
    const int hl = hs * p.stride + tap_h, wl = ws * p.stride + tap_w;
    const bool gok = pk < (unsigned)p.Ps && (unsigned)hl < (unsigned)p.Hl && (unsigned)wl < (unsigned)p.Wl;
    const unsigned dpix = (unsigned)b * HWl + (unsigned)hl * (unsigned)p.Wl + (unsigned)wl - (unsigned)g0;
    const unsigned gokm = (unsigned)(-(int)gok);
    const unsigned g_off = ((dpix * g_ld4 + (WG_GBIAS + (unsigned)c16 * 4u)) & gokm) | (~gokm & WG_OOB);
    const long left = p.Ps - pk0;
    const unsigned lin_rec = (unsigned)(left < WG_BK ? left : WG_BK);
    auto rsrc = [&](const float* base, long ld, unsigned ld4, bool gathered) {
      const long px = gathered ? g0 : (long)pk0;
      const float* b_ = base + (px * ld - (gathered ? (long)(WG_GBIAS / 4) : 0L));
      return __builtin_amdgcn_make_buffer_rsrc(const_cast<float*>(b_), 0, gathered ? (int)WG_OOB : (int)(lin_rec * ld4),
                                               0x00020000);
    };
    const __amdgpu_buffer_rsrc_t rs_row = rsrc(row_base, p.row.ld, row_ld4, row_g);
    const __amdgpu_buffer_rsrc_t rs_col = rsrc(col_base, p.col.ld, col_ld4, col_g);
    const unsigned row_off = row_g ? g_off : row_lin, col_off = col_g ? g_off : col_lin;
#pragma unroll
    for (int j = 0; j < TM; ++j)
      __builtin_amdgcn_raw_ptr_buffer_load_lds(rs_row, (lic_lptr_t)&smem[buf][j][wave * 256], 16,
                                               (int)(row_live[j] ? row_off : WG_OOB), 256 * j, 0, 0);
#pragma unroll
    for (int j = 0; j < TN; ++j)
      __builtin_amdgcn_raw_ptr_buffer_load_lds(rs_col, (lic_lptr_t)&smem[buf][TM + j][wave * 256], 16,
                                               (int)(col_live[j] ? col_off : WG_OOB), 256 * j, 0, 0);
  };
  auto compute = [&](int buf) {
    float af[TM][8], bf[TN][8];
#pragma unroll
    for (int a = 0; a < TM; ++a) {
      const int ch = wm0 + a * 32;
#pragma unroll
      for (int t = 0; t < 8; ++t) af[a][t] = smem[buf][ch >> 6][(lh * 8 + t) * 64 + (ch & 63) + li];
    }
#pragma unroll
    for (int b = 0; b < TN; ++b) {
      const int ch = wn0 + b * 32;
#pragma unroll
      for (int t = 0; t < 8; ++t) {
        const float v = smem[buf][TM + (ch >> 6)][(lh * 8 + t) * 64 + (ch & 63) + li];
        bf[b][t] = SQB ? v * v : v;
      }
    }
#pragma unroll
    for (int t = 0; t < 8; ++t)
#pragma unroll
      for (int a = 0; a < TM; ++a)
#pragma unroll
        for (int b = 0; b < TN; ++b)
          acc[a][b] = __builtin_amdgcn_mfma_f32_32x32x2f32(af[a][t], bf[b][t], acc[a][b], 0, 0, 0);
  };

  if (nloc > 0) {
    issue(c_begin, 0);
    int c = 0;
    for (; c + 1 < nloc; c += 2) {
      __syncthreads();
      issue(c_begin + c + 1, 1);
      compute(0);
      __builtin_amdgcn_sched_barrier(0);
      __syncthreads();
      issue(c_begin + c + 2, 0);
      compute(1);
      __builtin_amdgcn_sched_barrier(0);
    }
    __syncthreads();
    if (c < nloc) compute(0);
  }
  float* slab = p.slabs + ((long)split * p.ntaps + tap) * p.row.C * p.col.C;
#pragma unroll
  for (int a = 0; a < TM; ++a)
#pragma unroll
    for (int q = 0; q < 16; ++q) {
      const int m = m0 + wm0 + a * 32 + (q & 3) + 8 * (q >> 2) + 4 * lh;
      if (!FULL && m >= p.row.C) continue;
#pragma unroll
      for (int b = 0; b < TN; ++b) {
        const int n = n0 + wn0 + b * 32 + li;
        if (FULL || n < p.col.C) slab[(long)m * p.col.C + n] = acc[a][b][q];
      }
    }
}

__global__ __launch_bounds__(256) void wgrad_reduce_kernel(const float* slabs, float* dst, int splitk,
                                                           int ntaps, int Cm, int Cn, long sm, long sn,
                                                           long stap, float scale) {
  const long total = (long)ntaps * Cm * Cn;
  for (long i = (long)blockIdx.x * 256 + threadIdx.x; i < total; i += (long)gridDim.x * 256) {
    float a8[8] = {0.f, 0.f, 0.f, 0.f, 0.f, 0.f, 0.f, 0.f};
    int z = 0;
    for (; z + 8 <= splitk; z += 8) {
#pragma unroll
      for (int k = 0; k < 8; ++k) a8[k] += slabs[(long)(z + k) * total + i];
    }
    for (; z < splitk; ++z) a8[0] += slabs[(long)z * total + i];
    const float acc = ((a8[0] + a8[1]) + (a8[2] + a8[3])) + ((a8[4] + a8[5]) + (a8[6] + a8[7]));
    const int n = (int)(i % Cn);
    const long t2 = i / Cn;
    const int m = (int)(t2 % Cm);
    const int tap = (int)(t2 / Cm);
    dst[m * sm + n * sn + tap * stap] = acc * scale;
  }
}

long lic_pick_splits(long base, long slots, long max_sk) {
  long best = 1;
  double best_eff = 0.0;
  if (max_sk > 512) max_sk = 512;
  if (max_sk < 1) max_sk = 1;
  for (long r = 1; r <= 4; ++r) {
    long sk = (r * slots) / base;
    if (sk < 1) continue;
    if (sk > max_sk) sk = max_sk;
    const long wgs = base * sk;
    const double eff = (double)wgs / ((double)((wgs + slots - 1) / slots) * (double)slots);
    if (eff > best_eff + 0.03) {
      best = sk;
      best_eff = eff;
    }
    if (eff >= 0.9 || sk == max_sk) break;
  }
  return best;
}

static bool wgrad_dma_addressable(const lic_wgrad_desc* d) {
  const long lim = 1L << 30;
  if (d->p_ld < 0 || d->g_ld < 0 || d->p_ld > lim || d->g_ld > lim) return false;
  if (16 * d->p_ld * 4 > lim) return false;
  const long HWs = (long)d->Hs * d->Ws, HWl = (long)d->Hl * d->Wl, st = d->stride;
  const long n = std::min<long>(16, d->B * HWs) - 1;
  const long lines = std::min<long>((long)d->B * d->Hs - 1, dma_wraps(n, 16, d->Ws));
  const long images = std::min<long>(d->B - 1, dma_wraps(n, 16, HWs));
  const long D = n * st + lines * st * labs((long)d->Wl - d->Ws) + images * d->Wl * labs((long)d->Hl - st * d->Hs);
  if (D > lim || HWl > 0x7FFFFFFFL) return false;
  return std::max<long>(D, 16) * d->g_ld * 4 + (long)d->Cg * 4 <= lim;
}

static int wg_plan(const lic_wgrad_desc* d, WgPlan* pl) {
  if (wgrad_desc_check(d) != LIC_OK) return LIC_ERR_INVALID;
  pl->dma = wgrad_dma_addressable(d);
  pl->Cm = d->g_is_row ? d->Cg : d->Cp;
  pl->Cn = d->g_is_row ? d->Cp : d->Cg;
  pl->ntaps = d->kh * d->kw;
  pl->vec = (d->Cp % 4 == 0) && (d->p_ld % 4 == 0) && aligned16(d->p) && (d->Cg % 4 == 0) &&
            (d->g_ld % 4 == 0) && aligned16(d->g);
  pl->TM = (pl->vec && pl->Cm > 64 && (pl->Cm % 128 == 0 || pl->Cm > 256 || pl->Cm <= 128)) ? 2 : 1;
  pl->TN = (pl->vec && pl->Cn > 128) ? 3 : (pl->vec && pl->Cn > 64 ? 2 : 1);
  if (pl->TM == 1 && pl->TN == 2) pl->TN = 1;
  const long chunks16 = ((long)d->B * d->Hs * d->Ws + 255) / 256;
  if (pl->vec && pl->dma && pl->Cm % 192 == 0 && pl->Cn % 192 == 0 &&
      chunks16 * pl->ntaps >= 512 &&
      !(d->g_is_row ? d->sq_g : d->sq_p)) {
    pl->TM = 3;
    pl->TN = 3;
  }
  if (d->force_tm || d->force_tn) {
    const int tm = d->force_tm, tn = d->force_tn;
    const bool sq_row = d->g_is_row ? d->sq_g : d->sq_p;
    const bool t33 = tm == 3 && tn == 3 && pl->dma && pl->Cm % 192 == 0 && pl->Cn % 192 == 0 && !sq_row;
    const bool listed = (tm == 1 && (tn == 1 || tn == 3)) || (tm == 2 && tn >= 1 && tn <= 3);
    if (!pl->vec || !(t33 || listed)) return LIC_ERR_UNSUPPORTED;
    pl->TM = tm;
    pl->TN = tn;
  }
  pl->MTt = (pl->Cm + 64 * pl->TM - 1) / (64 * pl->TM);
  pl->NTt = (pl->Cn + 64 * pl->TN - 1) / (64 * pl->TN);
  const long Ps = (long)d->B * d->Hs * d->Ws;
  pl->nchunks = (int)((Ps + WG_BK - 1) / WG_BK);
  const long base = (long)pl->MTt * pl->NTt * pl->ntaps;
  const long resident = 256L * (pl->TM == 1 ? 4 : 2);
  long sk = (resident * 5 / 2 + base - 1) / base;
  const long max_sk = (pl->nchunks + 15) / 16;
  if (sk > max_sk) sk = max_sk;
  if (sk < 1) sk = 1;
  if (sk > 256) sk = 256;
  if (sk > 8) sk = (sk + 7) & ~7L;
  if (pl->TM >= 2) sk = lic_pick_splits(base, resident, max_sk);
  if (sk > max_sk) sk = max_sk;
  if (d->force_split > 0) sk = d->force_split < pl->nchunks ? d->force_split : pl->nchunks;
  pl->cps = (int)((pl->nchunks + sk - 1) / sk);
  pl->splitk = (pl->nchunks + pl->cps - 1) / pl->cps;
  return LIC_OK;
}

LIC_EXPORT size_t lic_wgrad_workspace_bytes(const lic_wgrad_desc* d) {
  WgPlan pl;
  if (wg_plan(d, &pl) != LIC_OK) return 0;
  return wgrad_slab_bytes(pl);
}

constexpr unsigned wgrad_key(bool glds, int TM, int TN, bool vec_or_sqb, bool full) {
  return lic_variant_key(TM, TN, vec_or_sqb, full, glds);
}
#define WGRAD_ROW(...) LIC_VARIANT(wgrad_key(false, __VA_ARGS__), 256, wgrad_kernel<__VA_ARGS__>)
#define WGRAD_GLDS_ROW(...) LIC_VARIANT(wgrad_key(true, __VA_ARGS__), 256, wgrad_glds_kernel<__VA_ARGS__>)
static const KernelVariant<WgradParams> g_wgrad_variants[] = {
    WGRAD_ROW(1, 1, false, false),
    WGRAD_ROW(1, 1, true, false),      WGRAD_ROW(1, 1, true, true),
    WGRAD_ROW(1, 3, true, false),      WGRAD_ROW(1, 3, true, true),
    WGRAD_ROW(2, 1, true, false),      WGRAD_ROW(2, 1, true, true),
    WGRAD_ROW(2, 2, true, false),      WGRAD_ROW(2, 2, true, true),
    WGRAD_ROW(2, 3, true, false),      WGRAD_ROW(2, 3, true, true),
    WGRAD_GLDS_ROW(1, 1, false, false), WGRAD_GLDS_ROW(1, 1, false, true),
    WGRAD_GLDS_ROW(1, 1, true, false),  WGRAD_GLDS_ROW(1, 1, true, true),
    WGRAD_GLDS_ROW(1, 3, false, false), WGRAD_GLDS_ROW(1, 3, false, true),
    WGRAD_GLDS_ROW(1, 3, true, false),  WGRAD_GLDS_ROW(1, 3, true, true),
    WGRAD_GLDS_ROW(2, 1, false, false), WGRAD_GLDS_ROW(2, 1, false, true),
    WGRAD_GLDS_ROW(2, 1, true, false),  WGRAD_GLDS_ROW(2, 1, true, true),
    WGRAD_GLDS_ROW(2, 2, false, false), WGRAD_GLDS_ROW(2, 2, false, true),
    WGRAD_GLDS_ROW(2, 2, true, false),  WGRAD_GLDS_ROW(2, 2, true, true),
    WGRAD_GLDS_ROW(2, 3, false, false), WGRAD_GLDS_ROW(2, 3, false, true),
    WGRAD_GLDS_ROW(2, 3, true, false),  WGRAD_GLDS_ROW(2, 3, true, true),
    WGRAD_GLDS_ROW(3, 3, false, true),  WGRAD_GLDS_ROW(3, 3, true, true),
};
#undef WGRAD_ROW
#undef WGRAD_GLDS_ROW
static const KernelVariant<WgradParams>* find_variant(const lic_wgrad_desc* d, const WgPlan& pl) {
  if (!pl.vec) return lic_find_variant(g_wgrad_variants, wgrad_key(false, 1, 1, false, false));
  const bool full = (pl.Cm % (64 * pl.TM) == 0) && (pl.Cn % (64 * pl.TN) == 0);
  const bool sq_row = d->g_is_row ? d->sq_g : d->sq_p, sq_col = d->g_is_row ? d->sq_p : d->sq_g;
  if (sq_row || !pl.dma) return lic_find_variant(g_wgrad_variants, wgrad_key(false, pl.TM, pl.TN, true, full));
  return lic_find_variant(g_wgrad_variants, wgrad_key(true, pl.TM, pl.TN, sq_col, full));
}

LIC_EXPORT int lic_wgrad_kernel_name(const lic_wgrad_desc* d, char* buf, size_t n) {
  WgPlan pl;
  const int rc = wg_plan(d, &pl);
  if (rc != LIC_OK) return rc;
  return lic_variant_name(find_variant(d, pl), buf, n);
}
static int wgrad_run(const lic_wgrad_desc* d, void* workspace, size_t workspace_bytes, int stage,
                     lic_stream_t stream) {
  WgPlan pl;
  int rc = wg_plan(d, &pl);
  if (rc != LIC_OK) return rc;
  rc = wgrad_launch_check(d, pl, workspace, workspace_bytes, d->stride < 1 ? LIC_ERR_UNSUPPORTED : LIC_OK);
  if (rc != LIC_OK) return rc;
  const KernelVariant<WgradParams>* v = find_variant(d, pl);
  if (!v) return LIC_ERR_UNSUPPORTED;
  hipStream_t s = (hipStream_t)stream;
  if (stage != 2) {
    const WgradParams p = wgrad_fill<WgradParams>(d, pl, workspace);
    hipLaunchKernelGGL(v->kernel, dim3(pl.MTt * pl.NTt * pl.ntaps * pl.splitk), dim3(v->block), 0, s, p);
    rc = lic_check_launch();
    if (rc != LIC_OK) return rc;
  }
  if (stage == 1) return LIC_OK;
  const long total = (long)pl.ntaps * pl.Cm * pl.Cn;
  hipLaunchKernelGGL(wgrad_reduce_kernel, dim3(ew_grid(total, 256)), dim3(256), 0, s,
                     (const float*)workspace, d->dst, pl.splitk, pl.ntaps, pl.Cm, pl.Cn, (long)d->dst_sm,
                     (long)d->dst_sn, (long)d->dst_stap, d->scale);
  return lic_check_launch();
}
LIC_EXPORT int lic_wgrad(const lic_wgrad_desc* d, void* workspace, size_t workspace_bytes,
                         lic_stream_t stream) {
  return wgrad_run(d, workspace, workspace_bytes, 0, stream);
}
LIC_EXPORT int lic_wgrad_stage(const lic_wgrad_desc* d, void* workspace, size_t workspace_bytes,
                               int32_t stage, lic_stream_t stream) {
  if (stage < 0 || stage > 2) return LIC_ERR_INVALID;
  return wgrad_run(d, workspace, workspace_bytes, stage, stream);
}

LIC_EXPORT int lic_wgrad_plan(const lic_wgrad_desc* d, int32_t* TM, int32_t* TN, int32_t* splitk) {
  WgPlan pl;
  const int rc = wg_plan(d, &pl);
  if (rc != LIC_OK) return rc;
  if (TM) *TM = pl.vec ? pl.TM : 1;
  if (TN) *TN = pl.vec ? pl.TN : 1;
  if (splitk) *splitk = pl.splitk;
  return LIC_OK;
}

LIC_EXPORT int lic_version(void) { return LIC_ABI_VERSION; }
LIC_EXPORT int lic_last_hip_error(void) { return g_lic_last_hip_error; }
LIC_EXPORT const char* lic_arch(void) { return "gfx950"; }
```

### neural_image_compression_amd/csrc/lic_gemm_bf16.hip

```cpp
#include "lic_tile_map.h"
#include "lic_epilogue_bf16.h"
#include <algorithm>
#include <type_traits>

typedef __bf16 bf16x4 __attribute__((ext_vector_type(4)));

constexpr int HB_BK = 32;

__device__ __attribute__((aligned(16))) float g_lic_zero16h[4];

struct IgemmHParams {
  const bf16_t* in;
  const bf16_t* w;
  const float* bias;
  void* out;
  bf16_t* out2;
  const bf16_t* aux;
  const bf16_t* aux2;
  const bf16_t* aux3;
  bf16_t* out3;
  const float* beta;
  long in_ld, out_ld, out2_ld, aux_ld, aux2_ld, aux3_ld, out3_ld;
  int B, Hi, Wi, Cin, Ho, Wo, Cout;
  int kw, stride, pad, transposed, prologue, epilogue, out_f32;
// ... 733 lines not shown
                       out_f32 ? 1 : 0, d->epilogue == LIC_EPI_LEAKY ? 1 : 0, d->slope);
  }
  return lic_check_launch();
}

struct WgHOperand {
  const bf16_t* ptr;
  long ld;
  int C;
  int gathered;
  int sq;
};
struct WgradHParams {
  WgHOperand row, col;
  float* slabs;
  int B, Hs, Ws, Hl, Wl;
  int kw, stride, pad, ntaps;
  int MTt, NTt;
  int chunks_per_split, nchunks;
  long Ps;
  FastDiv dHW, dW;
};
typedef short s16x4 __attribute__((ext_vector_type(4)));
typedef short s16x8 __attribute__((ext_vector_type(8)));

constexpr int WH_BK = 32;

template <int TM, int TN, bool SQB = false>
__global__ __launch_bounds__(256, 2) void wgrad_bf16_kernel(const WgradHParams p) {
  constexpr int BK = WH_BK;
  constexpr int NPASS = BK / 32;
  constexpr int SUB = BK * 64;
  constexpr int NS = TM + TN;
  constexpr int NL = NS * NPASS;
  constexpr int BMt = 64 * TM, BNt = 64 * TN;
  constexpr int WM = BMt / 2, WN = BNt / 2;
  __shared__ __attribute__((aligned(16))) bf16_t smem[3][NS][SUB];
  const int tid = threadIdx.x, lane = tid & 63;
  const int wave = __builtin_amdgcn_readfirstlane(tid >> 6);
  const int wm0 = (wave >> 1) * WM, wn0 = (wave & 1) * WN;
  const int li = lane & 31, lh = lane >> 5;
  const WgradTile wt = wgrad_tile(p, xcd_contiguous(blockIdx.x, gridDim.x), BMt, BNt);
  const int m0 = wt.m0, n0 = wt.n0, tap = wt.tap, split = wt.split;
  const int c_begin = wt.c_begin, c_end = wt.c_end, nloc = c_end - c_begin;

  f32x16 acc[TM][TN];
#pragma unroll
  for (int a = 0; a < TM; ++a)
#pragma unroll
    for (int b = 0; b < TN; ++b)
#pragma unroll
      for (int q = 0; q < 16; ++q) acc[a][b][q] = 0.0f;

  const int kr = tid >> 3;
  const int c8 = (((tid & 7) ^ (((tid >> 4) & 1) << 2))) * 8;
  const bf16_t* zsrc = reinterpret_cast<const bf16_t*>(g_lic_zero16h);
  auto issue = [&](int c, int buf) {
    const int cc = c < c_end ? c : c_end - 1;
#pragma unroll
    for (int j = 0; j < NPASS; ++j) {
      const WgradPixel w = wgrad_pixel(p, (long)cc * BK + kr + 32 * j, wt.r, wt.s);
      const bool rok = p.row.gathered ? w.gok : w.inb, cok = p.col.gathered ? w.gok : w.inb;
      const long rpx = p.row.gathered ? w.gpix : (long)w.pix, cpx = p.col.gathered ? w.gpix : (long)w.pix;
#pragma unroll
      for (int t = 0; t < TM; ++t) {
        const int ch = m0 + 64 * t + c8;
        const bool ok = rok && ch < p.row.C;
        const bf16_t* src = ok ? p.row.ptr + rpx * p.row.ld + ch : zsrc;
        __builtin_amdgcn_global_load_lds((lic_gptr_t)src, (lic_lptr_t)&smem[buf][t][j * 2048 + wave * 512], 16, 0,
                                         0);
      }
#pragma unroll
      for (int t = 0; t < TN; ++t) {
        const int ch = n0 + 64 * t + c8;
        const bool ok = cok && ch < p.col.C;
        const bf16_t* src = ok ? p.col.ptr + cpx * p.col.ld + ch : zsrc;
        __builtin_amdgcn_global_load_lds((lic_gptr_t)src, (lic_lptr_t)&smem[buf][TM + t][j * 2048 + wave * 512],
                                         16, 0, 0);
      }
    }
  };
  const int tq = (lane >> 2) & 3, tp = lane & 3, tg = (lane >> 4) & 1;
  unsigned tr_addr[2];
  {
    const unsigned base = (unsigned)(size_t)(__attribute__((address_space(3))) void*)&smem[0][0][0];
#pragma unroll
    for (int half = 0; half < 2; ++half) {
      const int cs = 32 * half + 16 * tg + 4 * tp;
      const int slot = (cs >> 3) ^ ((tq >> 1) << 2);
      tr_addr[half] = base + 2u * (unsigned)((8 * lh + tq) * 64 + slot * 8 + (cs & 7));
    }
  }
  auto compute = [&](auto bufc) {
    constexpr int buf = decltype(bufc)::value;
#pragma unroll
    for (int ks = 0; ks < BK / 16; ++ks) {
      unsigned long long lo[NS], hi[NS];
#pragma unroll
      for (int t = 0; t < TM + TN; ++t) {
        const int ch = t < TM ? wm0 + t * 32 : wn0 + (t - TM) * 32;
        const int sub = t < TM ? (ch >> 6) : TM + (ch >> 6);
        const unsigned addr = tr_addr[(ch >> 5) & 1] + 2u * (unsigned)((buf * NS + sub) * SUB + 16 * ks * 64);
        asm volatile("ds_read_b64_tr_b16 %0, %1" : "=v"(lo[t]) : "v"(addr));
        asm volatile("ds_read_b64_tr_b16 %0, %1 offset:512" : "=v"(hi[t]) : "v"(addr));
      }
      if constexpr (NS == 2)
        asm volatile("s_waitcnt lgkmcnt(0)" : "+v"(lo[0]), "+v"(hi[0]), "+v"(lo[1]), "+v"(hi[1]));
      else if constexpr (NS == 3)
        asm volatile("s_waitcnt lgkmcnt(0)"
                     : "+v"(lo[0]), "+v"(hi[0]), "+v"(lo[1]), "+v"(hi[1]), "+v"(lo[2]), "+v"(hi[2]));
      else if constexpr (NS == 4)
        asm volatile("s_waitcnt lgkmcnt(0)"
                     : "+v"(lo[0]), "+v"(hi[0]), "+v"(lo[1]), "+v"(hi[1]), "+v"(lo[2]), "+v"(hi[2]), "+v"(lo[3]),
                       "+v"(hi[3]));
      else if constexpr (NS == 5)
        asm volatile("s_waitcnt lgkmcnt(0)"
                     : "+v"(lo[0]), "+v"(hi[0]), "+v"(lo[1]), "+v"(hi[1]), "+v"(lo[2]), "+v"(hi[2]), "+v"(lo[3]),
                       "+v"(hi[3]), "+v"(lo[4]), "+v"(hi[4]));
      else
        asm volatile("s_waitcnt lgkmcnt(0)"
                     : "+v"(lo[0]), "+v"(hi[0]), "+v"(lo[1]), "+v"(hi[1]), "+v"(lo[2]), "+v"(hi[2]), "+v"(lo[3]),
                       "+v"(hi[3]), "+v"(lo[4]), "+v"(hi[4]), "+v"(lo[5]), "+v"(hi[5]));
      bf16x8 fr[NS];
#pragma unroll
      for (int t = 0; t < NS; ++t) {
        struct {
          unsigned long long a, b;
        } pr{lo[t], hi[t]};
        fr[t] = __builtin_bit_cast(bf16x8, pr);
        if constexpr (SQB)
          if (t >= TM) fr[t] = sq8(fr[t]);
      }
#pragma unroll
      for (int a = 0; a < TM; ++a)
#pragma unroll
        for (int b = 0; b < TN; ++b)
          acc[a][b] = __builtin_amdgcn_mfma_f32_32x32x16_bf16(fr[a], fr[TM + b], acc[a][b], 0, 0, 0);
    }
  };

  if (nloc > 0) {
    issue(c_begin, 0);
    issue(c_begin + 1, 1);
    auto step = [&](int c, auto cur, auto fill) {
      asm volatile("s_waitcnt vmcnt(%0)\n\ts_barrier" ::"i"(NL) : "memory");
      issue(c_begin + c + 2, decltype(fill)::value);
      compute(cur);
      __builtin_amdgcn_sched_barrier(0);
    };
    using I0 = std::integral_constant<int, 0>;
    using I1 = std::integral_constant<int, 1>;
    using I2 = std::integral_constant<int, 2>;
    int c = 0;
    for (; c + 2 < nloc; c += 3) {
      step(c, I0{}, I2{});
      step(c + 1, I1{}, I0{});
      step(c + 2, I2{}, I1{});
    }
    if (c < nloc) step(c, I0{}, I2{});
    if (c + 1 < nloc) step(c + 1, I1{}, I0{});
    asm volatile("s_waitcnt vmcnt(0)" ::: "memory");
  }
  float* slab = p.slabs + ((long)split * p.ntaps + tap) * p.row.C * p.col.C;
#pragma unroll
  for (int a = 0; a < TM; ++a)
#pragma unroll
    for (int b = 0; b < TN; ++b) {
      const int n = n0 + wn0 + b * 32 + li;
#pragma unroll
      for (int q = 0; q < 16; ++q) {
        const int m = m0 + wm0 + a * 32 + (q & 3) + 8 * (q >> 2) + 4 * lh;
        if (m < p.row.C && n < p.col.C) slab[(long)m * p.col.C + n] = acc[a][b][q];
      }
      __builtin_amdgcn_sched_barrier(0);
    }
}

__global__ __launch_bounds__(256) void wgrad_bf16_reduce_kernel(const float* slabs, float* dst, int splitk,
                                                                int ntaps, int Cm, int Cn, long sm, long sn,
                                                                long stap, float scale) {
  const long total = (long)ntaps * Cm * Cn;
  for (long i = (long)blockIdx.x * 256 + threadIdx.x; i < total; i += (long)gridDim.x * 256) {
    float a8[8] = {0.f, 0.f, 0.f, 0.f, 0.f, 0.f, 0.f, 0.f};
    int z = 0;
    for (; z + 8 <= splitk; z += 8) {
#pragma unroll
      for (int k = 0; k < 8; ++k) a8[k] += slabs[(long)(z + k) * total + i];
    }
    for (; z < splitk; ++z) a8[0] += slabs[(long)z * total + i];
    const float acc = ((a8[0] + a8[1]) + (a8[2] + a8[3])) + ((a8[4] + a8[5]) + (a8[6] + a8[7]));
    const int n = (int)(i % Cn);
    const long t2 = i / Cn;
    const int m = (int)(t2 % Cm);
    const int tap = (int)(t2 / Cm);
    dst[m * sm + n * sn + tap * stap] = acc * scale;
  }
}

static int wgh_plan(const lic_wgrad_desc* d, WgPlan* pl) {
  if (wgrad_desc_check(d) != LIC_OK) return LIC_ERR_INVALID;
  if (d->Cp % 8 || d->Cg % 8 || d->p_ld % 8 || d->g_ld % 8) return LIC_ERR_UNSUPPORTED;
  pl->vec = 1;
  pl->Cm = d->g_is_row ? d->Cg : d->Cp;
  pl->Cn = d->g_is_row ? d->Cp : d->Cg;
  pl->ntaps = d->kh * d->kw;
  auto pick = [](int C) {
    const int u = (C + 63) / 64;
    return u % 3 == 0 ? 3 : (u % 2 == 0 ? 2 : (u == 1 ? 1 : (u > 4 ? 3 : 2)));
  };
  pl->TM = pick(pl->Cm);
  pl->TN = pick(pl->Cn);
  pl->MTt = (pl->Cm + 64 * pl->TM - 1) / (64 * pl->TM);
  pl->NTt = (pl->Cn + 64 * pl->TN - 1) / (64 * pl->TN);
  const long Ps = (long)d->B * d->Hs * d->Ws;
  pl->nchunks = (int)((Ps + WH_BK - 1) / WH_BK);
  const long base = (long)pl->MTt * pl->NTt * pl->ntaps;
  const long max_sk = (pl->nchunks + 15) / 16;
  const long per_cu = pl->TM + pl->TN >= 5 ? 2 : 3;
  const long sk = lic_pick_splits(base, 256L * per_cu, max_sk);
  pl->cps = (int)((pl->nchunks + sk - 1) / sk);
  pl->splitk = (pl->nchunks + pl->cps - 1) / pl->cps;
  return LIC_OK;
}
LIC_EXPORT size_t lic_wgrad_bf16_workspace_bytes(const lic_wgrad_desc* d) {
  WgPlan pl;
  if (wgh_plan(d, &pl) != LIC_OK) return 0;
  return wgrad_slab_bytes(pl);
}

constexpr unsigned wgradh_key(int TM, int TN, bool sq_col, bool sq_row = false) {
  return lic_variant_key(TM, TN, sq_col, sq_row);
}
#define WGRADH_ROW(...) LIC_VARIANT(wgradh_key(__VA_ARGS__), 256, wgrad_bf16_kernel<__VA_ARGS__>)
static const KernelVariant<WgradHParams> g_wgradh_variants[] = {
    WGRADH_ROW(1, 1, false), WGRADH_ROW(1, 2, false), WGRADH_ROW(1, 3, false),
    WGRADH_ROW(2, 1, false), WGRADH_ROW(2, 2, false), WGRADH_ROW(2, 3, false),
    WGRADH_ROW(3, 1, false), WGRADH_ROW(3, 2, false), WGRADH_ROW(3, 3, false),
    WGRADH_ROW(1, 1, true),  WGRADH_ROW(2, 2, true),  WGRADH_ROW(3, 3, true),
};
#undef WGRADH_ROW
static const KernelVariant<WgradHParams>* find_variant(const lic_wgrad_desc* d, const WgPlan& pl) {
  const bool sq_row = d->g_is_row ? d->sq_g : d->sq_p, sq_col = d->g_is_row ? d->sq_p : d->sq_g;
  return lic_find_variant(g_wgradh_variants, wgradh_key(pl.TM, pl.TN, sq_col, sq_row));
}

LIC_EXPORT int lic_wgrad_bf16_kernel_name(const lic_wgrad_desc* d, char* buf, size_t n) {
  WgPlan pl;
  const int rc = wgh_plan(d, &pl);
  if (rc != LIC_OK) return rc;
  return lic_variant_name(find_variant(d, pl), buf, n);
}
static int wgrad_bf16_impl(const lic_wgrad_desc* d, void* workspace, size_t workspace_bytes, lic_reduce_job* job,
                           lic_stream_t stream) {
  WgPlan pl;
  int rc = wgh_plan(d, &pl);
  if (rc != LIC_OK) return rc;
  rc = wgrad_launch_check(d, pl, workspace, workspace_bytes,
                          aligned16(d->p) && aligned16(d->g) ? LIC_OK : LIC_ERR_INVALID);
  if (rc != LIC_OK) return rc;
  const KernelVariant<WgradHParams>* v = find_variant(d, pl);
  if (!v) return LIC_ERR_UNSUPPORTED;
  const WgradHParams p = wgrad_fill<WgradHParams>(d, pl, workspace);
  hipStream_t s = (hipStream_t)stream;
  hipLaunchKernelGGL(v->kernel, dim3(pl.MTt * pl.NTt * pl.ntaps * pl.splitk), dim3(v->block), 0, s, p);
  rc = lic_check_launch();
  if (rc != LIC_OK) return rc;
  const long total = (long)pl.ntaps * pl.Cm * pl.Cn;
  if (job) {
    *job = lic_reduce_job{};
    job->src = (const float*)workspace;
    job->dst = d->dst;
    job->kind = LIC_REDUCE_SLABS;
    job->splitk = pl.splitk;
    job->ntaps = pl.ntaps;
    job->Cm = pl.Cm;
    job->Cn = pl.Cn;
    job->Mvalid = pl.Cm;
    job->Nvalid = pl.Cn;
    job->sm = d->dst_sm;
    job->sn = d->dst_sn;
    job->stap = d->dst_stap;
    job->scale = d->scale;
    return LIC_OK;
  }
  hipLaunchKernelGGL(wgrad_bf16_reduce_kernel, dim3(ew_grid(total, 256)), dim3(256), 0, s, (const float*)workspace,
                     d->dst, pl.splitk, pl.ntaps, pl.Cm, pl.Cn, (long)d->dst_sm, (long)d->dst_sn, (long)d->dst_stap,
                     d->scale);
  return lic_check_launch();
}
LIC_EXPORT int lic_wgrad_bf16(const lic_wgrad_desc* d, void* workspace, size_t workspace_bytes,
                              lic_stream_t stream) {
  return wgrad_bf16_impl(d, workspace, workspace_bytes, nullptr, stream);
}
LIC_EXPORT int lic_wgrad_bf16_partial(const lic_wgrad_desc* d, void* workspace, size_t workspace_bytes,
                                      lic_reduce_job* job, lic_stream_t stream) {
  if (!job) return LIC_ERR_INVALID;
  return wgrad_bf16_impl(d, workspace, workspace_bytes, job, stream);
}

struct ReduceTable {
  lic_reduce_job j[LIC_REDUCE_MAX_JOBS];
  int n;
};
__global__ __launch_bounds__(256) void reduce_batch_kernel(const ReduceTable tb) {
  int ji = 0;
  while (ji + 1 < tb.n && (int)blockIdx.x >= tb.j[ji + 1].block0) ++ji;
  const lic_reduce_job& q = tb.j[ji];
  const int blk = (int)blockIdx.x - q.block0;
  if (q.kind == LIC_REDUCE_SLABS) {
    const long total = (long)q.ntaps * q.Cm * q.Cn;
    for (long i = (long)blk * 256 + threadIdx.x; i < total; i += (long)q.nblocks * 256) {
      float a8[8] = {0.f, 0.f, 0.f, 0.f, 0.f, 0.f, 0.f, 0.f};
      const float* sp = q.src + i;
      int z = 0;
      for (; z + 32 <= q.splitk; z += 32) {
        float v[32];
#pragma unroll
        for (int k = 0; k < 32; ++k) v[k] = sp[(long)(z + k) * total];
#pragma unroll
        for (int r = 0; r < 4; ++r)
#pragma unroll
          for (int k = 0; k < 8; ++k) a8[k] += v[8 * r + k];
      }
      for (; z + 8 <= q.splitk; z += 8) {
        float v[8];
#pragma unroll
        for (int k = 0; k < 8; ++k) v[k] = sp[(long)(z + k) * total];
#pragma unroll
        for (int k = 0; k < 8; ++k) a8[k] += v[k];
      }
      if (z < q.splitk) {
        float v[7];
#pragma unroll
        for (int k = 0; k < 7; ++k) v[k] = sp[(long)(z + k < q.splitk ? z + k : q.splitk - 1) * total];
#pragma unroll
        for (int k = 0; k < 7; ++k)
          if (z + k < q.splitk) a8[0] += v[k];
      }
      const float acc = ((a8[0] + a8[1]) + (a8[2] + a8[3])) + ((a8[4] + a8[5]) + (a8[6] + a8[7]));
      const int n = (int)(i % q.Cn);
      const long t2 = i / q.Cn;
      const int m = (int)(t2 % q.Cm);
      const int tap = (int)(t2 / q.Cm);
      if (m >= q.Mvalid || n >= q.Nvalid) continue;
      const long mo = q.mdiv ? (long)(m / q.mdiv) * q.sm + (long)(m % q.mdiv) * q.smr : (long)m * q.sm;
      const long no = q.ndiv ? (long)(n / q.ndiv) * q.sn + (long)(n % q.ndiv) * q.snr : (long)n * q.sn;
      const long o = mo + no + tap * q.stap;
      float v = acc * q.scale;
      if (q.epilogue == LIC_REDUCE_EPI_REPARAM) {
        const float pv = q.param[o], w = pv > q.bound ? pv : q.bound;
        const float g = v * 2.0f * w;
        v = (pv >= q.bound || g < 0.0f) ? g : 0.0f;
      }
      q.dst[o] = v;
    }
  } else {
    __shared__ double red[16][17];
    const int cx = threadIdx.x & 15, ly = threadIdx.x >> 4;
    const int c = blk * 16 + cx;
    double acc = 0.0;
    if (c < q.Cn) {
      int y = ly;
      for (; y + 16 * 7 < q.splitk; y += 16 * 8) {
        float v[8];
#pragma unroll
        for (int k = 0; k < 8; ++k) v[k] = q.src[(long)(y + 16 * k) * q.Cn + c];
#pragma unroll
        for (int k = 0; k < 8; ++k) acc += (double)v[k];
      }
      for (; y < q.splitk; y += 16) acc += (double)q.src[(long)y * q.Cn + c];
    }
    red[ly][cx] = acc;
    __syncthreads();
    if (ly == 0 && c < q.Cn) {
      double t = 0.0;
#pragma unroll
      for (int k = 0; k < 16; ++k) t += red[k][cx];
      float v = (float)(t * (double)q.scale);
      if (q.epilogue == LIC_REDUCE_EPI_REPARAM) {
        const float pv = q.param[c], w = pv > q.bound ? pv : q.bound;
        const float g = v * 2.0f * w;
        v = (pv >= q.bound || g < 0.0f) ? g : 0.0f;
      }
      q.dst[c] = v;
    }
  }
}
LIC_EXPORT int lic_reduce_batch(const lic_reduce_job* jobs, int32_t njobs, lic_stream_t stream) {
  if (njobs < 0 || (njobs > 0 && !jobs)) return LIC_ERR_INVALID;
  for (int base = 0; base < njobs; base += LIC_REDUCE_MAX_JOBS) {
    ReduceTable tb;
    tb.n = njobs - base < LIC_REDUCE_MAX_JOBS ? njobs - base : LIC_REDUCE_MAX_JOBS;
    int blocks = 0;
    int order[LIC_REDUCE_MAX_JOBS];
    for (int i = 0; i < tb.n; ++i) order[i] = i;
    auto depth = [&](int i) {
      const lic_reduce_job& q = jobs[base + i];
      return q.kind == LIC_REDUCE_COLUMNS ? (long)q.splitk * 2 : (long)q.splitk;
    };
    std::stable_sort(order, order + tb.n, [&](int a, int b) { return depth(a) > depth(b); });
    for (int oi = 0; oi < tb.n; ++oi) {
      const int i = oi;
      lic_reduce_job q = jobs[base + order[oi]];
      if (!q.src || !q.dst || q.splitk <= 0 || q.Cn <= 0 || (q.epilogue == LIC_REDUCE_EPI_REPARAM && !q.param)) return LIC_ERR_INVALID;
      if (q.kind == LIC_REDUCE_SLABS) {
        if (q.ntaps <= 0 || q.Cm <= 0 || q.mdiv < 0 || q.ndiv < 0) return LIC_ERR_INVALID;
        if (q.Mvalid <= 0 || q.Mvalid > q.Cm) q.Mvalid = q.Cm;
        if (q.Nvalid <= 0 || q.Nvalid > q.Cn) q.Nvalid = q.Cn;
        q.nblocks = ew_grid((long)q.ntaps * q.Cm * q.Cn, 256);
      } else if (q.kind == LIC_REDUCE_COLUMNS) {
        q.nblocks = (q.Cn + 15) / 16;
      } else {
        return LIC_ERR_INVALID;
      }
      q.block0 = blocks;
      blocks += q.nblocks;
      tb.j[i] = q;
    }
    hipLaunchKernelGGL(reduce_batch_kernel, dim3(blocks), dim3(256), 0, (hipStream_t)stream, tb);
    const int rc = lic_check_launch();
    if (rc != LIC_OK) return rc;
  }
  return LIC_OK;
}
```

### neural_image_compression_amd/functional.py

```python
from __future__ import annotations

import ctypes as C
from typing import Optional, Tuple

import torch

from . import _lib as L
from .reductions import can_defer, defer, flush_point, flush_reductions

PEDESTAL = float(2.0 ** -36)
LIKELIHOOD_BOUND = 1e-9

PROFILE = None
PROFILE_MIN_FLOP = 0.0
FORCE_IGEMM = None
FORCE_WGRAD = None
KERNEL_TRACE = None
GRAD_VIEWS = {}
PREPARED = {}
AUX_STREAM = None
PLAN_RECORDING = False


_raw_stream = getattr(torch._C, "_cuda_getCurrentRawStream", None)


def _stream():
    if _raw_stream is not None:
        return C.c_void_p(_raw_stream(torch.cuda.current_device()))
    return C.c_void_p(torch.cuda.current_stream().cuda_stream)


def _ptr(t: Optional[torch.Tensor]):
    return None if t is None else C.c_void_p(t.data_ptr())


def _require_cuda(*ts):
    for t in ts:
        if t is not None and not t.is_cuda:
            raise L.LicError("neural_image_compression_amd runs on MI355X only: got a non-CUDA tensor "
                             "(there is no CPU fallback; the CPU oracle lives in oracle/ for tests)")
        if t is not None and t.device.index != torch.cuda.current_device():
            raise L.LicError(f"tensor on cuda:{t.device.index} but the current device is cuda:"
                             f"{torch.cuda.current_device()}: call torch.cuda.set_device(...) first (one process per GPU)")
        if t is not None and t.dtype != torch.float32:
            raise L.LicError(f"fp32 tensors expected, got {t.dtype}")


def _nhwc(t: torch.Tensor) -> torch.Tensor:
    return t.permute(0, 2, 3, 1).contiguous()


def _nchw_view(t_nhwc: torch.Tensor) -> torch.Tensor:
    return t_nhwc.permute(0, 3, 1, 2)


def _permute3(src, dst, n, s, d):
    L.check(L.load().lic_permute3(_ptr(src), _ptr(dst), n[0], n[1], n[2], s[0], s[1], s[2], d[0], d[1],
                                  d[2], _stream()), "lic_permute3")


def _pack(src: torch.Tensor, taps: int, K: int, N: int, s_tap: int, s_k: int, s_n: int) -> torch.Tensor:
    lib = L.load()
    out = torch.empty((lib.lic_packed_weight_floats(taps, K, N),), device=src.device, dtype=torch.float32)
    L.check(lib.lic_pack_weight(_ptr(src), _ptr(out), taps, K, N, s_tap, s_k, s_n, _stream()),
            "lic_pack_weight")
    return out


def _pack_dense(m: torch.Tensor) -> torch.Tensor:
    K, N = m.shape
    return _pack(m, 1, K, N, 0, N, 1)


def _conv_weight_layout(w: torch.Tensor, transposed_weight: bool, for_dgrad: bool):
    d0, d1, kh, kw = w.shape
    taps = kh * kw
    if transposed_weight:
        cin, cout = d0, d1
        s_ci, s_co = d1 * taps, taps
    else:
        cout, cin = d0, d1
        s_co, s_ci = d1 * taps, taps
    if for_dgrad:
        return taps, cout, cin, 1, s_co, s_ci
    return taps, cin, cout, 1, s_ci, s_co


def _pack_conv_weight(w: torch.Tensor, transposed_weight: bool, for_dgrad: bool) -> torch.Tensor:
    hit = prepared(w, "f32.dgrad" if for_dgrad else "f32.fwd")
    if hit is not None:
        return hit
    w = w.contiguous()
    return _pack(w, *_conv_weight_layout(w, transposed_weight, for_dgrad))


def _igemm_desc(inp, w_packed, out, B, Hi, Wi, Cin, Ho, Wo, Cout, kh, kw, stride, pad, transposed, bias, prologue, epilogue,
                slope, tap_mask, out2, aux, aux2, aux3, out3, out_ld, res=None, in_ld=None):
    d = L.IgemmDesc()
    d.in_, d.w, d.bias, d.out, d.out2 = _ptr(inp), _ptr(w_packed), _ptr(bias), _ptr(out), _ptr(out2)
    d.aux, d.aux2, d.aux3, d.res, d.out3 = _ptr(aux), _ptr(aux2), _ptr(aux3), _ptr(res), _ptr(out3)
    d.in_ld = Cin if in_ld is None else in_ld
    d.out_ld = Cout if out_ld is None else out_ld
    d.out2_ld = d.aux_ld = d.aux2_ld = d.aux3_ld = d.res_ld = d.out3_ld = Cout
    d.B, d.Hi, d.Wi, d.Cin, d.Ho, d.Wo, d.Cout = B, Hi, Wi, Cin, Ho, Wo, Cout
    d.kh, d.kw, d.stride, d.pad = kh, kw, stride, pad
    d.transposed, d.prologue, d.epilogue = int(transposed), prologue, epilogue
    d.tap_mask, d.slope = tap_mask, slope
    return d


def _wgrad_desc(p, g, dst, B, Hs, Ws, Cp, Hl, Wl, Cg, kh, kw, stride, pad, g_is_row, dst_sm, dst_sn, dst_stap, sq_p, sq_g,
                scale):
    d = L.WgradDesc()
    d.p, d.g, d.dst = _ptr(p), _ptr(g), _ptr(dst)
    d.p_ld, d.g_ld = Cp, Cg
    d.dst_sm, d.dst_sn, d.dst_stap = dst_sm, dst_sn, dst_stap
    d.B, d.Hs, d.Ws, d.Cp, d.Hl, d.Wl, d.Cg = B, Hs, Ws, Cp, Hl, Wl, Cg
    d.kh, d.kw, d.stride, d.pad = kh, kw, stride, pad
    d.g_is_row, d.sq_p, d.sq_g, d.scale = int(g_is_row), sq_p, sq_g, scale
    return d


def _kernel_name(fn, d) -> str:
    nm = C.create_string_buffer(96)
    L.check(fn(C.byref(d), nm, 96), "kernel_name")
    return nm.value.decode()


def _trace(name):
    if KERNEL_TRACE is not None:
        KERNEL_TRACE.add(name() if callable(name) else name)


def _timed(name, flops, act_bytes, launch, staged=None):
    if PROFILE is None or flops < PROFILE_MIN_FLOP:
        launch()
        return
    e0, e1 = torch.cuda.Event(enable_timing=True), torch.cuda.Event(enable_timing=True)
    e0.record()
    if staged is None:
        launch()
        e1.record()
    else:
        staged(1)
        e1.record()
        staged(2)
    if callable(name):
        name = name()
    PROFILE.append((name, flops, act_bytes, e0, e1) if isinstance(name, str) else (*name, e0, e1))


def _igemm(inp, w_packed, out, *, B, Hi, Wi, Cin, Ho, Wo, Cout, kh, kw, stride, pad, transposed,
           bias=None, prologue=0, epilogue=L.EPI_NONE, slope=0.01, tap_mask=0, out2=None, aux=None,
           aux2=None, aux3=None, res=None, in_ld=None, out_ld=None, out3=None):
    d = _igemm_desc(inp, w_packed, out, B, Hi, Wi, Cin, Ho, Wo, Cout, kh, kw, stride, pad, transposed, bias, prologue,
                    epilogue, slope, tap_mask, out2, aux, aux2, aux3, out3, out_ld, res, in_ld)
    lib = L.load()
    if FORCE_IGEMM is not None:
        d.force_bm, d.force_tn, d.force_split = FORCE_IGEMM[:3]
    _trace(lambda: _kernel_name(lib.lic_igemm_kernel_name, d))
    if Ho * Wo <= 1024 and out2 is None and res is None:
        nbytes = lib.lic_igemm_workspace_bytes(C.byref(d))
        if nbytes:
            ws = torch.empty(nbytes // 4, device=inp.device, dtype=torch.float32)
            d.workspace, d.workspace_bytes = _ptr(ws), nbytes

    def row():
        bm, bn, macs = C.c_int32(0), C.c_int32(0), C.c_int64(0)
        lib.lic_igemm_plan(C.byref(d), C.byref(bm), C.byref(bn), C.byref(macs))
        flops, act_bytes = 2 * macs.value, 4 * (B * Hi * Wi * Cin + B * Ho * Wo * Cout)
        if epilogue in (L.EPI_CONV_GDN, L.EPI_CONV_IGDN):
            flops += 2 * B * Ho * Wo * Cout * Cout
            act_bytes += 4 * 2 * B * Ho * Wo * Cout
        return _kernel_name(lib.lic_igemm_kernel_name, d), flops, act_bytes
    _timed(row, 2.0 * B * Ho * Wo * Cout * Cin * kh * kw, None,
           lambda: L.check(lib.lic_igemm(C.byref(d), _stream()), "lic_igemm"))


def _wgrad(p, g, dst, *, B, Hs, Ws, Cp, Hl, Wl, Cg, kh, kw, stride, pad, g_is_row, dst_sm, dst_sn,
           dst_stap, sq_p=0, sq_g=0, scale=1.0):
    d = _wgrad_desc(p, g, dst, B, Hs, Ws, Cp, Hl, Wl, Cg, kh, kw, stride, pad, g_is_row, dst_sm, dst_sn, dst_stap, sq_p,
                    sq_g, scale)
    lib = L.load()
    if FORCE_WGRAD is not None:
        d.force_tm, d.force_tn, d.force_split = FORCE_WGRAD
    _trace(lambda: _kernel_name(lib.lic_wgrad_kernel_name, d))
    nbytes = lib.lic_wgrad_workspace_bytes(C.byref(d))
    ws = torch.empty((max(nbytes, 4) + 3) // 4, device=p.device, dtype=torch.float32)

    def stage(k):
        L.check(lib.lic_wgrad_stage(C.byref(d), _ptr(ws), nbytes, k, _stream()), "lic_wgrad_stage")
    _timed(lambda: _kernel_name(lib.lic_wgrad_kernel_name, d), 2 * B * Hs * Ws * kh * kw * Cp * Cg,
           4 * (B * Hs * Ws * Cp + B * Hl * Wl * Cg),
           lambda: L.check(lib.lic_wgrad(C.byref(d), _ptr(ws), nbytes, _stream()), "lic_wgrad"),
           staged=stage)


def _colsum(t2d: torch.Tensor, P: int, Cc: int, scale: float = 1.0) -> torch.Tensor:
    lib = L.load()
    nbytes = lib.lic_colsum_workspace_bytes(P, Cc)
    ws = torch.empty((nbytes + 3) // 4, device=t2d.device, dtype=torch.float32)
    out = torch.empty((Cc,), device=t2d.device, dtype=torch.float32)
    L.check(lib.lic_colsum(_ptr(t2d), Cc, P, Cc, scale, _ptr(out), _ptr(ws), nbytes, _stream()),
            "lic_colsum")
    return out


def prepared(param: torch.Tensor, kind: str):
    e = PREPARED.get((id(param), kind))
    if e is not None and e[0] == param._version and e[2]() is param:
        return e[1]
    return None


def grad_like(param: torch.Tensor) -> torch.Tensor:
    e = GRAD_VIEWS.get(id(param)) if GRAD_VIEWS else None
    if e is not None and e[0]() is param and param.grad is None and not e[2]:
        e[2] = True
        return e[1].detach()
    return torch.empty_like(param, memory_format=torch.contiguous_format)


def _reparam_bwd2(beta_c, dbe, beta_bound, gamma_c, dge, gamma_bound):
    dbeta = torch.empty_like(beta_c) if beta_c is not None else None
    dgamma = torch.empty_like(gamma_c) if gamma_c is not None else None
    if dbeta is None and dgamma is None:
        return None, None
    L.check(L.load().lic_gdn_reparam_bwd2(_ptr(beta_c), _ptr(dbe), _ptr(dbeta), 0 if dbeta is None else dbeta.numel(),
                                          beta_bound, _ptr(gamma_c), _ptr(dge), _ptr(dgamma),
                                          0 if dgamma is None else dgamma.numel(), gamma_bound, _stream()),
            "lic_gdn_reparam_bwd2")
    return dbeta, dgamma


def _leaky_bwd(y, dy, slope):
    dx = torch.empty_like(y)
    L.check(L.load().lic_leaky_bwd(_ptr(y), _ptr(dy), _ptr(dx), y.numel(), slope, _stream()),
            "lic_leaky_bwd")
    return dx


def conv_out_size(H, W, k, stride, pad, transposed, out_pad=0):
    if transposed:
        return (H - 1) * stride - 2 * pad + k + out_pad, (W - 1) * stride - 2 * pad + k + out_pad
    return (H + 2 * pad - k) // stride + 1, (W + 2 * pad - k) // stride + 1


class _ConvFn(torch.autograd.Function):

    @staticmethod
    def forward(ctx, x, weight, bias, stride, pad, out_pad, transposed, leaky, slope, tap_mask, res, out_view=None):
        _require_cuda(x, weight, bias, res)
        xh = _nhwc(x)
        B, Hi, Wi, Cin = xh.shape
        kh, kw = weight.shape[2], weight.shape[3]
        Cout = weight.shape[1] if transposed else weight.shape[0]
        Ho, Wo = conv_out_size(Hi, Wi, kh, stride, pad, transposed, out_pad)
        wp = _pack_conv_weight(weight, transposed, for_dgrad=False)
        out_ld = None
        if out_view is not None:
            if leaky or res is not None or tuple(out_view.shape) != (B, Ho, Wo, Cout) or out_view.stride(3) != 1 or \
                    out_view.stride(1) != Wo * out_view.stride(2) or out_view.stride(0) != Ho * out_view.stride(1):
                raise ValueError("out_view must be a [B,Ho,Wo,Cout] channel slice of a contiguous NHWC buffer")
            out, out_ld = out_view, out_view.stride(2)
        else:
            out = torch.empty((B, Ho, Wo, Cout), device=x.device, dtype=torch.float32)
        resh = None if res is None else _nhwc(res)
        out2 = torch.empty_like(out) if (leaky and res is not None) else None
        _igemm(xh, wp, out, B=B, Hi=Hi, Wi=Wi, Cin=Cin, Ho=Ho, Wo=Wo, Cout=Cout, kh=kh, kw=kw,
               stride=stride, pad=pad, transposed=transposed, bias=bias,
               epilogue=L.EPI_LEAKY if leaky else L.EPI_NONE, slope=slope, tap_mask=tap_mask,
               res=resh, out2=out2, out_ld=out_ld)
        ctx.save_for_backward(xh, weight, out if leaky else None)
        ctx.cfg = (stride, pad, transposed, leaky, slope, tap_mask, bias is not None, res is not None)
        return _nchw_view(out2 if out2 is not None else out)

    @staticmethod
    def backward(ctx, gy):
        xh, weight, yh = ctx.saved_tensors
        stride, pad, transposed, leaky, slope, tap_mask, has_bias, has_res = ctx.cfg
        g = _nhwc(gy)
        if leaky:
            g = _leaky_bwd(yh, g, slope)
        elif not has_res:
            _carry_partial(gy, g)
        dx, dw, db = _conv_backward(xh, weight, g, stride, pad, transposed, tap_mask,
                                    ctx.needs_input_grad[0], ctx.needs_input_grad[1],
                                    has_bias and ctx.needs_input_grad[2])
        return dx, dw, db, None, None, None, None, None, None, None, (gy if has_res else None), None


def _conv_backward(xh, weight, g, stride, pad, transposed, tap_mask, need_dx, need_dw, need_db):
    B, Hi, Wi, Cin = xh.shape
    _, Ho, Wo, Cout = g.shape
    kh, kw = weight.shape[2], weight.shape[3]
    dx = dw = db = None
    if need_dx:
        wp = _pack_conv_weight(weight, transposed, for_dgrad=True)
        dxh = torch.empty_like(xh)
        _igemm(g, wp, dxh, B=B, Hi=Ho, Wi=Wo, Cin=Cout, Ho=Hi, Wo=Wi, Cout=Cin, kh=kh, kw=kw,
               stride=stride, pad=pad, transposed=not transposed, tap_mask=tap_mask)
        dx = _nchw_view(dxh)
    if need_dw:
        dw = grad_like(weight)
        taps = kh * kw
        if transposed:
            _wgrad(xh, g, dw, B=B, Hs=Hi, Ws=Wi, Cp=Cin, Hl=Ho, Wl=Wo, Cg=Cout, kh=kh, kw=kw,
                   stride=stride, pad=pad, g_is_row=False, dst_sm=Cout * taps, dst_sn=taps, dst_stap=1)
        else:
            _wgrad(g, xh, dw, B=B, Hs=Ho, Ws=Wo, Cp=Cout, Hl=Hi, Wl=Wi, Cg=Cin, kh=kh, kw=kw,
                   stride=stride, pad=pad, g_is_row=True, dst_sm=taps, dst_sn=Cin * taps, dst_stap=1)
    if need_db:
        db = _bias_grad(g, B * Ho * Wo, Cout)
    return dx, dw, db


def _carry_partial(src, dst):
    part = getattr(src, "_lic_colsum_partial", None)
    if part is not None:
        dst._lic_colsum_partial = part


def _bias_grad(g, P, Cout):
    part = getattr(g, "_lic_colsum_partial", None)
    if part is not None and part.shape[1] == Cout:
        return _colsum(part, part.shape[0], Cout)
    return _colsum(g, P, Cout)


def conv2d(x, weight, bias, stride=1, padding=0, leaky=False, slope=0.01, tap_mask=0, residual=None, out=None):
    return _ConvFn.apply(x, weight, bias, stride, padding, 0, False, leaky, slope, tap_mask, residual, out)


class _JoinChannelsFn(torch.autograd.Function):

    @staticmethod
    def forward(ctx, a, b, buf):
        ca, cb = a.shape[1], b.shape[1]
        if buf.shape[-1] != ca + cb or a.data_ptr() != buf.data_ptr() or \
                b.data_ptr() != buf.data_ptr() + buf.element_size() * ca:
            raise ValueError("join_channels: the operands are not the two channel ranges of the buffer")
        ctx.ca = ca
        return _nchw_view(buf)

    @staticmethod
    def backward(ctx, g):
        return g[:, :ctx.ca], g[:, ctx.ca:], None


def join_channels(a, b, buf):
    return _JoinChannelsFn.apply(a, b, buf)


def pack_conv_weight(weight: torch.Tensor) -> torch.Tensor:
    _require_cuda(weight)
    return _pack_conv_weight(weight.detach(), False, for_dgrad=False)


@torch.no_grad()
def conv2d_prepacked(x, w_packed, bias, cout, kernel, stride=1, padding=0, leaky=False, slope=0.01, tap_mask=0,
                     pin_tile=False, out=None):
    _require_cuda(x, w_packed, bias, out)
    xh = _nhwc(x)
    B, Hi, Wi, Cin = xh.shape
    Ho, Wo = conv_out_size(Hi, Wi, kernel, stride, padding, False)
    out_ld = None
    if out is None:
        out = torch.empty((B, Ho, Wo, cout), device=x.device, dtype=torch.float32)
    else:
        if tuple(out.shape) != (B, Ho, Wo, cout) or out.stride(3) != 1 or out.stride(1) != Wo * out.stride(2) or \
                out.stride(0) != Ho * out.stride(1):
            raise ValueError("out must be a [B,Ho,Wo,cout] channel slice of a contiguous NHWC buffer")
        out_ld = out.stride(2)
    global FORCE_IGEMM
    saved = FORCE_IGEMM
    if pin_tile and Cin % 4 == 0 and cout % 64 == 0:
        FORCE_IGEMM = (64, 1, 0)
    try:
        _igemm(xh, w_packed, out, B=B, Hi=Hi, Wi=Wi, Cin=Cin, Ho=Ho, Wo=Wo, Cout=cout, kh=kernel, kw=kernel,
               stride=stride, pad=padding, transposed=False, bias=bias,
               epilogue=L.EPI_LEAKY if leaky else L.EPI_NONE, slope=slope, tap_mask=tap_mask, out_ld=out_ld)
    finally:
        FORCE_IGEMM = saved
    return _nchw_view(out)


def conv_transpose2d(x, weight, bias, stride=1, padding=0, output_padding=0, leaky=False, slope=0.01,
                     residual=None):
    return _ConvFn.apply(x, weight, bias, stride, padding, output_padding, True, leaky, slope, 0, residual)


def _kpad(kh, kw, c):
    return (kh * kw * c + 3) // 4 * 4


def _image_conv_columns(xh, weight, stride, pad):
    B, Hi, Wi, Cin = xh.shape
    Cout, _, kh, kw = weight.shape
    Ho, Wo = conv_out_size(Hi, Wi, kh, stride, pad, False)
    Kp = _kpad(kh, kw, Cin)
    P = B * Ho * Wo
    col = torch.empty((P, Kp), device=xh.device, dtype=torch.float32)
    L.check(L.load().lic_im2col(_ptr(xh), _ptr(col), B, Hi, Wi, Cin, Ho, Wo, kh, kw, stride, pad, Kp,
                                _stream()), "lic_im2col")
    taps = kh * kw
    wpk = prepared(weight, "f32.stem")
    if wpk is None:
        wp = torch.zeros((Kp, Cout), device=xh.device, dtype=torch.float32)
        _permute3(weight.contiguous(), wp, (taps, Cin, Cout), (1, taps, Cin * taps), (Cin * Cout, Cout, 1))
        wpk = _pack_dense(wp)
    return col, wpk, Ho, Wo, Kp


def _image_conv_backward(col, weight, g, stride, pad, in_shape, need_dx, need_dw, need_db):
    B, Hi, Wi, Cin = in_shape
    _, Ho, Wo, Cout = g.shape
    _, _, kh, kw = weight.shape
    taps, Kp, P = kh * kw, col.shape[1], B * Ho * Wo
    lib = L.load()
    dx = dw = db = None
    if need_dx:
        wpT = torch.zeros((Cout, Kp), device=g.device, dtype=torch.float32)
        _permute3(weight.contiguous(), wpT, (Cout, Cin, taps), (Cin * taps, taps, 1), (Kp, 1, Cin))
        dcol = torch.empty((P, Kp), device=g.device, dtype=torch.float32)
        _igemm(g, _pack_dense(wpT), dcol, B=1, Hi=1, Wi=P, Cin=Cout, Ho=1, Wo=P, Cout=Kp, kh=1, kw=1, stride=1,
               pad=0, transposed=False)
        dxh = torch.empty((B, Hi, Wi, Cin), device=g.device, dtype=torch.float32)
        L.check(lib.lic_col2im(_ptr(dcol), None, _ptr(dxh), B, Ho, Wo, Cin, Hi, Wi, kh, kw, stride,
                               pad, Kp, _stream()), "lic_col2im")
        dx = _nchw_view(dxh)
    if need_dw:
        dw = grad_like(weight)
        tmp = torch.empty((Kp, Cout), device=g.device, dtype=torch.float32)
        _wgrad(col, g, tmp, B=1, Hs=1, Ws=P, Cp=Kp, Hl=1, Wl=P, Cg=Cout, kh=1, kw=1, stride=1, pad=0,
               g_is_row=False, dst_sm=Cout, dst_sn=1, dst_stap=0)
        _permute3(tmp, dw, (taps, Cin, Cout), (Cin * Cout, Cout, 1), (1, taps, Cin * taps))
    if need_db:
        db = _bias_grad(g, P, Cout)
    return dx, dw, db


class _ImageConvFn(torch.autograd.Function):

    @staticmethod
    def forward(ctx, x, weight, bias, stride, pad, leaky, slope):
        _require_cuda(x, weight, bias)
        xh = _nhwc(x)
        B = xh.shape[0]
        Cout = weight.shape[0]
        col, wp, Ho, Wo, Kp = _image_conv_columns(xh, weight, stride, pad)
        P = B * Ho * Wo
        out = torch.empty((B, Ho, Wo, Cout), device=x.device, dtype=torch.float32)
        _igemm(col, wp, out, B=1, Hi=1, Wi=P, Cin=Kp, Ho=1, Wo=P, Cout=Cout, kh=1, kw=1, stride=1,
               pad=0, transposed=False, bias=bias, epilogue=L.EPI_LEAKY if leaky else L.EPI_NONE,
               slope=slope)
        ctx.save_for_backward(col, weight, out if leaky else None)
        ctx.cfg = (stride, pad, leaky, slope, tuple(xh.shape), bias is not None)
        return _nchw_view(out)

    @staticmethod
    def backward(ctx, gy):
        col, weight, yh = ctx.saved_tensors
        stride, pad, leaky, slope, in_shape, has_bias = ctx.cfg
        g = _nhwc(gy)
        if leaky:
            g = _leaky_bwd(yh, g, slope)
        else:
            _carry_partial(gy, g)
        dx, dw, db = _image_conv_backward(col, weight, g, stride, pad, in_shape, ctx.needs_input_grad[0],
                                          ctx.needs_input_grad[1], has_bias and ctx.needs_input_grad[2])
        return dx, dw, db, None, None, None, None


class _ImageConvGDNFn(torch.autograd.Function):

    @staticmethod
    def forward(ctx, x, weight, bias, beta, gamma, stride, pad, inverse, beta_bound, gamma_bound, pedestal, keep=True):
        _require_cuda(x, weight, bias, beta, gamma)
        xh = _nhwc(x)
        B = xh.shape[0]
        Cout = weight.shape[0]
        col, wp, Ho, Wo, Kp = _image_conv_columns(xh, weight, stride, pad)
        P = B * Ho * Wo
        beta_e, gT = _gdn_operands(beta, gamma, beta_bound, gamma_bound, pedestal)
        y = torch.empty((B, Ho, Wo, Cout), device=x.device, dtype=torch.float32)
        conv_out = torch.empty_like(y) if keep else None
        norm = torch.empty_like(y) if keep else None
        _igemm(col, wp, y, B=1, Hi=1, Wi=P, Cin=Kp, Ho=1, Wo=P, Cout=Cout, kh=1, kw=1, stride=1,
               pad=0, transposed=False, bias=bias, epilogue=L.EPI_CONV_IGDN if inverse else L.EPI_CONV_GDN,
               out2=norm, out3=conv_out, aux=gT, aux2=beta_e)
        ctx.save_for_backward(col, weight, conv_out, norm, beta, gamma)
        ctx.cfg = (stride, pad, tuple(xh.shape), inverse, beta_bound, gamma_bound, bias is not None, pedestal)
        return _nchw_view(y)

    @staticmethod
    def backward(ctx, gy):
        col, weight, conv_out, norm, beta, gamma = ctx.saved_tensors
        stride, pad, in_shape, inverse, beta_bound, gamma_bound, has_bias, pedestal = ctx.cfg
        need = ctx.needs_input_grad
        g_conv, dbeta, dgamma = _gdn_backward(conv_out, norm, beta, gamma, _nhwc(gy), inverse,
                                              beta_bound, gamma_bound, pedestal, True, need[3], need[4])
        dx, dw, db = _image_conv_backward(col, weight, g_conv, stride, pad, in_shape, need[0], need[1],
                                          has_bias and need[2])
        return dx, dw, db, dbeta, dgamma, None, None, None, None, None, None, None


class _ImageConvTFn(torch.autograd.Function):

    @staticmethod
    def forward(ctx, x, weight, bias, stride, pad, out_pad):
        _require_cuda(x, weight, bias)
        xh = _nhwc(x)
        B, Hi, Wi, Cin = xh.shape
        _, Cout, kh, kw = weight.shape
        Ho, Wo = conv_out_size(Hi, Wi, kh, stride, pad, True, out_pad)
        taps, Kp, P = kh * kw, _kpad(kh, kw, Cout), B * Hi * Wi
        lib = L.load()
        wpk = prepared(weight, "f32.head")
        if wpk is None:
            wp = torch.zeros((Cin, Kp), device=x.device, dtype=torch.float32)
            _permute3(weight.contiguous(), wp, (Cin, Cout, taps), (Cout * taps, taps, 1), (Kp, 1, Cout))
            wpk = _pack_dense(wp)
        col = torch.empty((P, Kp), device=x.device, dtype=torch.float32)
        _igemm(xh, wpk, col, B=1, Hi=1, Wi=P, Cin=Cin, Ho=1, Wo=P, Cout=Kp, kh=1, kw=1, stride=1, pad=0,
               transposed=False)
        out = torch.empty((B, Ho, Wo, Cout), device=x.device, dtype=torch.float32)
        L.check(lib.lic_col2im(_ptr(col), _ptr(bias), _ptr(out), B, Hi, Wi, Cout, Ho, Wo, kh, kw, stride,
                               pad, Kp, _stream()), "lic_col2im")
        ctx.save_for_backward(xh, weight)
        ctx.cfg = (stride, pad, (Ho, Wo), bias is not None)
        return _nchw_view(out)

    @staticmethod
    def backward(ctx, gy):
        xh, weight = ctx.saved_tensors
        stride, pad, (Ho, Wo), has_bias = ctx.cfg
        g = _nhwc(gy)
        B, Hi, Wi, Cin = xh.shape
        _, Cout, kh, kw = weight.shape
        taps, Kp, P = kh * kw, _kpad(kh, kw, Cout), B * Hi * Wi
        lib = L.load()
        dcol = torch.empty((P, Kp), device=g.device, dtype=torch.float32)
        L.check(lib.lic_im2col(_ptr(g), _ptr(dcol), B, Ho, Wo, Cout, Hi, Wi, kh, kw, stride, pad, Kp,
                               _stream()), "lic_im2col")
        dx = dw = db = None
        if ctx.needs_input_grad[0]:
            wpk = prepared(weight, "f32.head_dx")
            if wpk is None:
                wpT = torch.zeros((Kp, Cin), device=g.device, dtype=torch.float32)
                _permute3(weight.contiguous(), wpT, (taps, Cout, Cin), (1, taps, Cout * taps),
                          (Cout * Cin, Cin, 1))
                wpk = _pack_dense(wpT)
            dxh = torch.empty_like(xh)
            _igemm(dcol, wpk, dxh, B=1, Hi=1, Wi=P, Cin=Kp, Ho=1, Wo=P, Cout=Cin, kh=1, kw=1, stride=1,
                   pad=0, transposed=False)
            dx = _nchw_view(dxh)
        if ctx.needs_input_grad[1]:
            dw = grad_like(weight)
            tmp = torch.empty((Cin, Kp), device=g.device, dtype=torch.float32)
            _wgrad(xh, dcol, tmp, B=1, Hs=1, Ws=P, Cp=Cin, Hl=1, Wl=P, Cg=Kp, kh=1, kw=1, stride=1, pad=0,
                   g_is_row=True, dst_sm=1, dst_sn=Kp, dst_stap=0)
            _permute3(tmp, dw, (Cin, taps, Cout), (Kp, Cout, 1), (Cout * taps, 1, taps))
        if has_bias and ctx.needs_input_grad[2]:
            db = _colsum(g, B * Ho * Wo, Cout)
        return dx, dw, db, None, None, None


def image_conv2d(x, weight, bias, stride, padding, leaky=False, slope=0.01):
    return _ImageConvFn.apply(x, weight, bias, stride, padding, leaky, slope)


def image_conv_transpose2d(x, weight, bias, stride, padding, output_padding):
    return _ImageConvTFn.apply(x, weight, bias, stride, padding, output_padding)


class _LeakyFn(torch.autograd.Function):
    @staticmethod
    def forward(ctx, x, slope):
        _require_cuda(x)
        xc = x.contiguous()
        y = _leaky_bwd(xc, xc, slope)
        ctx.save_for_backward(y)
        ctx.slope = slope
        return y

    @staticmethod
    def backward(ctx, gy):
        (y,) = ctx.saved_tensors
        return _leaky_bwd(y, gy.contiguous(), ctx.slope), None


def leaky_relu(x, slope=0.01):
    return _LeakyFn.apply(x, slope)


class _GDNFn(torch.autograd.Function):
    @staticmethod
    def forward(ctx, x, beta, gamma, inverse, beta_bound, gamma_bound, pedestal, res, keep=True):
        _require_cuda(x, beta, gamma, res)
        lib = L.load()
        xh = _nhwc(x)
        B, H, W, Cc = xh.shape
        beta_e, gT = _gdn_operands(beta, gamma, beta_bound, gamma_bound, pedestal)
        out = torch.empty_like(xh)
        norm = torch.empty_like(xh) if keep else None
        resh = None if res is None else _nhwc(res)
        P = B * H * W
        if lib.lic_gdn_supported(Cc):
            _trace(lambda: f"gdn_kernel<{Cc // 64}, {int(inverse)}>")
            _timed(f"gdn_kernel<{Cc // 64}, 0>", 2 * P * Cc * Cc, 4 * 3 * P * Cc,
                   lambda: L.check(lib.lic_gdn_fwd(_ptr(xh), _ptr(gT), _ptr(beta_e), _ptr(resh), _ptr(out), _ptr(norm),
                                                   P, Cc, int(inverse), _stream()), "lic_gdn_fwd"))
        else:
            _igemm(xh, gT, out, B=1, Hi=1, Wi=P, Cin=Cc, Ho=1, Wo=P, Cout=Cc, kh=1, kw=1, stride=1, pad=0,
                   transposed=False, bias=beta_e, prologue=1, epilogue=L.EPI_IGDN if inverse else L.EPI_GDN,
                   out2=norm, aux=xh, res=resh)
        ctx.save_for_backward(xh, norm, beta, gamma)
        ctx.cfg = (inverse, beta_bound, gamma_bound, res is not None, pedestal)
        return _nchw_view(out)

    @staticmethod
    def backward(ctx, gy):
        xh, norm, beta, gamma = ctx.saved_tensors
        inverse, beta_bound, gamma_bound, has_res, pedestal = ctx.cfg
        dxh, dbeta, dgamma = _gdn_backward(xh, norm, beta, gamma, _nhwc(gy), inverse, beta_bound,
                                           gamma_bound, pedestal, *ctx.needs_input_grad[:3])
        dres = gy if has_res else None
        dx = None if dxh is None else _nchw_view(dxh)
        if dx is not None:
            _carry_partial(dxh, dx)
        return dx, dbeta, dgamma, None, None, None, None, dres, None


def _gdn_operands(beta, gamma, beta_bound, gamma_bound, pedestal):
    beta_e, gT = prepared(beta, "f32.beta_e"), prepared(gamma, "f32.gdn_gT")
    if beta_e is None or gT is None:
        Cc = beta.numel()
        _, _, beta_e, gamma_e = _gdn_reparam(beta, gamma, beta_bound, gamma_bound, pedestal)
        gT = _pack(gamma_e, 1, Cc, Cc, 0, 1, Cc)
    return beta_e, gT


def _gdn_gamma_packed(gamma, gamma_bound, pedestal):
    gp = prepared(gamma, "f32.gdn_g")
    if gp is None:
        lib = L.load()
        gamma_c = gamma.contiguous()
        gamma_e = torch.empty_like(gamma_c)
        L.check(lib.lic_gdn_reparam(_ptr(gamma_c), _ptr(gamma_e), gamma_c.numel(), gamma_bound, pedestal, _stream()),
                "lic_gdn_reparam")
        gp = _pack_dense(gamma_e)
    return gp


def _gdn_reparam(beta, gamma, beta_bound, gamma_bound, pedestal):
    lib = L.load()
    Cc = beta.numel()
    beta_c, gamma_c = beta.contiguous(), gamma.contiguous()
    beta_e = torch.empty_like(beta_c)
    gamma_e = torch.empty_like(gamma_c)
    L.check(lib.lic_gdn_reparam(_ptr(beta_c), _ptr(beta_e), Cc, beta_bound, pedestal, _stream()),
            "lic_gdn_reparam")
    L.check(lib.lic_gdn_reparam(_ptr(gamma_c), _ptr(gamma_e), Cc * Cc, gamma_bound, pedestal,
                                _stream()), "lic_gdn_reparam")
    return beta_c, gamma_c, beta_e, gamma_e


def _gdn_backward(xh, norm, beta, gamma, g, inverse, beta_bound, gamma_bound, pedestal, need_dx, need_dbeta,
                  need_dgamma):
    lib = L.load()
    B, H, W, Cc = xh.shape
    P = B * H * W
    t = torch.empty_like(xh)
    dxh = dbeta = dgamma = None
    cs_dx = None
    dbe = None
    beta_c, gamma_c = beta.contiguous(), gamma.contiguous()
    gp = _gdn_gamma_packed(gamma, gamma_bound, pedestal) if need_dx else None
    if need_dx and lib.lic_gdn_supported(Cc):
        dxh = torch.empty_like(xh)
        rows = lib.lic_gdn_bwd_partial_rows(P)
        pt = torch.empty((rows, Cc), device=xh.device, dtype=torch.float32)
        pdx = torch.empty((rows, Cc), device=xh.device, dtype=torch.float32)
        _trace(lambda: f"gdn_bwd_kernel<{Cc // 64}, {int(inverse)}>")
        _timed(f"gdn_bwd_reg_kernel<{Cc // 64}>", 2 * P * Cc * Cc, 4 * 5 * P * Cc,
               lambda: L.check(lib.lic_gdn_bwd(_ptr(g), _ptr(xh), _ptr(norm), _ptr(gp), _ptr(dxh), _ptr(t), _ptr(pt),
                                               _ptr(pdx), P, Cc, int(inverse), _stream()), "lic_gdn_bwd"))
        if need_dbeta:
            dbe = _colsum(pt, rows, Cc)
        cs_dx = pdx
    elif need_dx and Cc % 4 == 0:
        dxh = torch.empty_like(xh)
        _igemm(g, gp, dxh, B=1, Hi=1, Wi=P, Cin=Cc, Ho=1, Wo=P, Cout=Cc, kh=1, kw=1, stride=1,
               pad=0, transposed=False, prologue=3 if inverse else 2,
               epilogue=L.EPI_IGDN_BWD if inverse else L.EPI_GDN_BWD, aux=g, aux2=xh, aux3=norm, out2=t)
    else:
        L.check(lib.lic_gdn_dnorm(_ptr(g), _ptr(xh), _ptr(norm), _ptr(t), xh.numel(), int(inverse),
                                  _stream()), "lic_gdn_dnorm")
        if need_dx:
            dxh = torch.empty_like(xh)
            _igemm(t, gp, dxh, B=1, Hi=1, Wi=P, Cin=Cc, Ho=1, Wo=P, Cout=Cc, kh=1, kw=1,
                   stride=1, pad=0, transposed=False, epilogue=L.EPI_IGDN_BWD if inverse else L.EPI_GDN_BWD,
                   aux=g, aux2=xh, aux3=norm)
    dge = None
    if need_dbeta and dbe is None:
        dbe = _colsum(t, P, Cc)
    if need_dgamma:
        dge = torch.empty_like(gamma_c)
        _wgrad(t, xh, dge, B=1, Hs=1, Ws=P, Cp=Cc, Hl=1, Wl=P, Cg=Cc, kh=1, kw=1, stride=1, pad=0,
               g_is_row=False, dst_sm=Cc, dst_sn=1, dst_stap=0, sq_g=1)
    dbeta, dgamma = _reparam_bwd2(beta_c if need_dbeta else None, dbe, beta_bound,
                                  gamma_c if need_dgamma else None, dge, gamma_bound)
    if cs_dx is not None and dxh is not None:
        dxh._lic_colsum_partial = cs_dx
    return dxh, dbeta, dgamma


class _ConvGDNFn(torch.autograd.Function):

    @staticmethod
    def forward(ctx, x, weight, bias, beta, gamma, stride, pad, out_pad, transposed, inverse, beta_bound,
                gamma_bound, pedestal, keep=True):
        _require_cuda(x, weight, bias, beta, gamma)
        xh = _nhwc(x)
        B, Hi, Wi, Cin = xh.shape
        kh, kw = weight.shape[2], weight.shape[3]
        Cout = weight.shape[1] if transposed else weight.shape[0]
        Ho, Wo = conv_out_size(Hi, Wi, kh, stride, pad, transposed, out_pad)
        wp = _pack_conv_weight(weight, transposed, for_dgrad=False)
        beta_e, gT = _gdn_operands(beta, gamma, beta_bound, gamma_bound, pedestal)
        y = torch.empty((B, Ho, Wo, Cout), device=x.device, dtype=torch.float32)
        conv_out = torch.empty_like(y) if keep else None
        norm = torch.empty_like(y) if keep else None
        _igemm(xh, wp, y, B=B, Hi=Hi, Wi=Wi, Cin=Cin, Ho=Ho, Wo=Wo, Cout=Cout, kh=kh, kw=kw, stride=stride,
               pad=pad, transposed=transposed, bias=bias,
               epilogue=L.EPI_CONV_IGDN if inverse else L.EPI_CONV_GDN, out2=norm, out3=conv_out, aux=gT,
               aux2=beta_e)
        ctx.save_for_backward(xh, weight, conv_out, norm, beta, gamma)
        ctx.cfg = (stride, pad, transposed, inverse, beta_bound, gamma_bound, bias is not None, pedestal)
        return _nchw_view(y)

    @staticmethod
    def backward(ctx, gy):
        xh, weight, conv_out, norm, beta, gamma = ctx.saved_tensors
        stride, pad, transposed, inverse, beta_bound, gamma_bound, has_bias, pedestal = ctx.cfg
        need = ctx.needs_input_grad
        g_conv, dbeta, dgamma = _gdn_backward(conv_out, norm, beta, gamma, _nhwc(gy), inverse,
                                              beta_bound, gamma_bound, pedestal, True, need[3], need[4])
        dx, dw, db = _conv_backward(xh, weight, g_conv, stride, pad, transposed, 0, need[0], need[1],
                                    has_bias and need[2])
        return dx, dw, db, dbeta, dgamma, None, None, None, None, None, None, None, None, None


def will_backprop(*ts) -> bool:
    return torch.is_grad_enabled() and any(t is not None and t.requires_grad for t in ts)


def fused_gdn_supported(cin: int, cout: int) -> bool:
    return bool(L.load().lic_igemm_fused_gdn_supported(int(cin), int(cout)))


def fused_gdn_preferred(x_shape, weight_shape, stride, padding, transposed, output_padding=0) -> bool:
    B, Cin, Hi, Wi = x_shape
    kh, kw = weight_shape[2], weight_shape[3]
    Cout = weight_shape[1] if transposed else weight_shape[0]
    Ho, Wo = conv_out_size(Hi, Wi, kh, stride, padding, transposed, output_padding)
    d = L.IgemmDesc()
    if not transposed and Cin < 4:
        d.B, d.Hi, d.Wi, d.Cin, d.Ho, d.Wo, d.Cout = 1, 1, B * Ho * Wo, _kpad(kh, kw, Cin), 1, B * Ho * Wo, Cout
        d.kh = d.kw = d.stride = 1
        d.pad = d.transposed = 0
    else:
        d.B, d.Hi, d.Wi, d.Cin, d.Ho, d.Wo, d.Cout = B, Hi, Wi, Cin, Ho, Wo, Cout
        d.kh, d.kw, d.stride, d.pad, d.transposed = kh, kw, stride, padding, int(transposed)
    d.in_ld, d.out_ld, d.out2_ld, d.out3_ld = d.Cin, Cout, Cout, Cout
    return bool(L.load().lic_igemm_fused_gdn_preferred(C.byref(d)))


def conv_gdn(x, weight, bias, beta, gamma, stride, padding, inverse, beta_bound, gamma_bound, pedestal=PEDESTAL,
             transposed=False, output_padding=0):
    if not transposed and weight.shape[1] < 4:
        return _ImageConvGDNFn.apply(x, weight, bias, beta, gamma, stride, padding, bool(inverse),
                                     float(beta_bound), float(gamma_bound), float(pedestal),
                                     will_backprop(x, weight, bias, beta, gamma))
    return _ConvGDNFn.apply(x, weight, bias, beta, gamma, stride, padding, output_padding, bool(transposed),
                            bool(inverse), float(beta_bound), float(gamma_bound), float(pedestal),
                            will_backprop(x, weight, bias, beta, gamma))


def gdn(x, beta, gamma, inverse, beta_bound, gamma_bound, pedestal=PEDESTAL, residual=None):
    return _GDNFn.apply(x, beta, gamma, bool(inverse), float(beta_bound), float(gamma_bound),
                        float(pedestal), residual, will_backprop(x, beta, gamma, residual))


_QUANT_CASTS = [None, None]


class _QuantizeFn(torch.autograd.Function):
    @staticmethod
    def forward(ctx, v, u, training, cast_in=False, cast_out=False):
        _require_cuda(v, u)
        vh = _nhwc(v)
        uh = None if u is None else _nhwc(u)
        out = torch.empty_like(vh)
        _QUANT_CASTS[0] = _QUANT_CASTS[1] = None
        if (cast_in or cast_out) and vh.numel() % 4 == 0:
            v16 = torch.empty_like(vh, dtype=torch.bfloat16) if cast_in else None
            o16 = torch.empty_like(vh, dtype=torch.bfloat16) if cast_out else None
            L.check(L.load().lic_quantize_bf16(_ptr(vh), _ptr(uh), _ptr(out), _ptr(v16), _ptr(o16), vh.numel(),
                                               int(training), _stream()), "lic_quantize_bf16")
            _QUANT_CASTS[0], _QUANT_CASTS[1] = v16, o16
        else:
            L.check(L.load().lic_quantize(_ptr(vh), _ptr(uh), _ptr(out), vh.numel(), int(training), _stream()),
                    "lic_quantize")
        ctx.training = training
        return _nchw_view(out)

    @staticmethod
    def backward(ctx, g):
        return (g if ctx.training else torch.zeros_like(g)), None, None, None, None


def attach_bf16(t: torch.Tensor, t16_nhwc: Optional[torch.Tensor]):
    if t16_nhwc is not None:
        t._lic_bf16 = (t._version, t16_nhwc)


def quantize(v, u=None, training=True, cast_in=False, cast_out=False):
    if not (cast_in or cast_out):
        return _QuantizeFn.apply(v, u, training)
    res = _QuantizeFn.apply(v, u, training, cast_in, cast_out)
    attach_bf16(v, _QUANT_CASTS[0])
    attach_bf16(res, _QUANT_CASTS[1])
    _QUANT_CASTS[0] = _QUANT_CASTS[1] = None
    return res


_QUANT_ANCHOR_CASTS = [None, None, None]


class _QuantizeAnchorFn(torch.autograd.Function):

    @staticmethod
    def forward(ctx, v, u, training, cast_in=False, cast_out=False):
        _require_cuda(v, u)
        vh = _nhwc(v)
        uh = None if u is None else _nhwc(u)
        B, h, w, Cc = vh.shape
        out, anc = torch.empty_like(vh), torch.empty_like(vh)
        _QUANT_ANCHOR_CASTS[:] = [None, None, None]
        if (cast_in or cast_out) and vh.numel() % 4 == 0:
            v16 = torch.empty_like(vh, dtype=torch.bfloat16) if cast_in else None
            o16 = torch.empty_like(vh, dtype=torch.bfloat16) if cast_out else None
            a16 = torch.empty_like(vh, dtype=torch.bfloat16) if cast_out else None
            L.check(L.load().lic_quantize_anchor_bf16(_ptr(vh), _ptr(uh), _ptr(out), _ptr(anc), _ptr(v16), _ptr(o16),
                                                      _ptr(a16), B, h, w, Cc, int(training), _stream()),
                    "lic_quantize_anchor_bf16")
            _QUANT_ANCHOR_CASTS[:] = [v16, o16, a16]
        else:
            L.check(L.load().lic_quantize_anchor(_ptr(vh), _ptr(uh), _ptr(out), _ptr(anc), B, h, w, Cc, int(training),
                                                 _stream()), "lic_quantize_anchor")
        ctx.training = training
        return _nchw_view(out), _nchw_view(anc)

    @staticmethod
    def backward(ctx, g, g_anchor):
        if not ctx.training:
            return torch.zeros_like(g), None, None, None, None
        _require_cuda(g, g_anchor)
        gh, ah = _nhwc(g), _nhwc(g_anchor)
        B, h, w, Cc = gh.shape
        dv = torch.empty_like(gh)
        L.check(L.load().lic_anchor_add(_ptr(gh), _ptr(ah), _ptr(dv), B, h, w, Cc, _stream()), "lic_anchor_add")
        return _nchw_view(dv), None, None, None, None


def quantize_anchor(v, u=None, training=True, cast_in=False, cast_out=False):
    res, anc = _QuantizeAnchorFn.apply(v, u, training, cast_in, cast_out)
    if cast_in or cast_out:
        attach_bf16(v, _QUANT_ANCHOR_CASTS[0])
        attach_bf16(res, _QUANT_ANCHOR_CASTS[1])
        attach_bf16(anc, _QUANT_ANCHOR_CASTS[2])
        _QUANT_ANCHOR_CASTS[:] = [None, None, None]
    return res, anc


_GAIN_CASTS = [None, None, None]


def _gain_rows(s: torch.Tensor, B: int, Cc: int):
    if s.dim() != 2 or s.shape[1] != Cc or s.shape[0] not in (1, B):
        raise L.LicError(f"a gain of shape [1 or {B}][{Cc}] expected, got {tuple(s.shape)}")
    return s.contiguous(), (0 if s.shape[0] == 1 else Cc)


def _gain_backward(vh, sh, s_stride, s_rows, d_vg, d_out, d_anchor, need_dv, need_ds):
    gs = [None if g is None else _nhwc(g) for g in (d_vg, d_out, d_anchor)]
    _require_cuda(*gs)
    B, h, w, Cc = vh.shape
    dv = torch.empty_like(vh)
    ds = torch.empty((B, Cc), device=vh.device, dtype=torch.float32)
    nbytes = L.load().lic_gain_bwd_workspace_bytes(B, h * w, Cc)
    ws = torch.empty(nbytes // 4, device=vh.device, dtype=torch.float32)
    L.check(L.load().lic_gain_bwd(_ptr(vh), _ptr(sh), s_stride, _ptr(gs[0]), _ptr(gs[1]), _ptr(gs[2]), _ptr(dv), _ptr(ds),
                                  B, h, w, Cc, _ptr(ws), nbytes, _stream()), "lic_gain_bwd")
    if s_rows == 1:
        ds = ds.sum(0, keepdim=True) if B > 1 else ds
    return (_nchw_view(dv) if need_dv else None), (ds if need_ds else None)


class _GainQuantizeFn(torch.autograd.Function):

    @staticmethod
    def forward(ctx, v, u, s, training, anchor, cast_in, cast_out):
        _require_cuda(v, u, s)
        vh = _nhwc(v)
        uh = None if (u is None or not training) else _nhwc(u)
        B, h, w, Cc = vh.shape
        sh, s_stride = _gain_rows(s, B, Cc)
        vg, out = torch.empty_like(vh), torch.empty_like(vh)
        anc = torch.empty_like(vh) if anchor else None
        g16 = torch.empty_like(vh, dtype=torch.bfloat16) if cast_in else None
        o16 = torch.empty_like(vh, dtype=torch.bfloat16) if cast_out else None
        a16 = torch.empty_like(vh, dtype=torch.bfloat16) if (cast_out and anchor) else None
        L.check(L.load().lic_gain_quantize(_ptr(vh), _ptr(uh), _ptr(sh), s_stride, _ptr(vg), _ptr(out), _ptr(anc), _ptr(g16),
                                           _ptr(o16), _ptr(a16), B, h, w, Cc, L.GAIN_NOISE if training else L.GAIN_ROUND,
                                           _stream()), "lic_gain_quantize")
        _GAIN_CASTS[:] = [g16, o16, a16]
        ctx.training, ctx.s_stride, ctx.s_rows = training, s_stride, s.shape[0]
        ctx.save_for_backward(vh, sh)
        ctx.set_materialize_grads(False)
        if anchor:
            return _nchw_view(vg), _nchw_view(out), _nchw_view(anc)
        return _nchw_view(vg), _nchw_view(out)

    @staticmethod
    def backward(ctx, d_vg, d_out, d_anchor=None):
        if not ctx.training:
            d_out = d_anchor = None
        if d_vg is None and d_out is None and d_anchor is None:
            return (None,) * 7
        vh, sh = ctx.saved_tensors
        dv, ds = _gain_backward(vh, sh, ctx.s_stride, ctx.s_rows, d_vg, d_out, d_anchor, ctx.needs_input_grad[0],
                                ctx.needs_input_grad[2])
        return dv, None, ds, None, None, None, None


def gain_quantize(v, u, s, training, anchor=False, cast_in=False, cast_out=False):
    res = _GainQuantizeFn.apply(v, u, s, training, anchor, cast_in, cast_out)
    for t, t16 in zip(res, _GAIN_CASTS):
        attach_bf16(t, t16)
    _GAIN_CASTS[:] = [None, None, None]
    return res


class _ChannelScaleFn(torch.autograd.Function):

    @staticmethod
    def forward(ctx, v, s, cast_out):
        _require_cuda(v, s)
        vh = _nhwc(v)
        B, h, w, Cc = vh.shape
        sh, s_stride = _gain_rows(s, B, Cc)
        vg = torch.empty_like(vh)
        g16 = torch.empty_like(vh, dtype=torch.bfloat16) if cast_out else None
        L.check(L.load().lic_gain_quantize(_ptr(vh), None, _ptr(sh), s_stride, _ptr(vg), None, None, _ptr(g16), None, None,
                                           B, h, w, Cc, L.GAIN_SCALE, _stream()), "lic_gain_quantize")
        _GAIN_CASTS[0] = g16
        ctx.s_stride, ctx.s_rows = s_stride, s.shape[0]
        ctx.save_for_backward(vh, sh)
        return _nchw_view(vg)

    @staticmethod
    def backward(ctx, d_vg):
        vh, sh = ctx.saved_tensors
        dv, ds = _gain_backward(vh, sh, ctx.s_stride, ctx.s_rows, d_vg, None, None, ctx.needs_input_grad[0],
                                ctx.needs_input_grad[1])
        return dv, ds, None


def channel_scale(v, s, cast_out=False):
    res = _ChannelScaleFn.apply(v, s, cast_out)
    attach_bf16(res, _GAIN_CASTS[0])
    _GAIN_CASTS[0] = None
    return res


class _GainRowsFn(torch.autograd.Function):

    @staticmethod
    def forward(ctx, q, *tables):
        _require_cuda(q, *tables)
        k, (Qn, M), B = len(tables), tables[0].shape, q.shape[0]
        T = tables[0].contiguous() if k == 1 else torch.stack(tables)
        rows = torch.empty((k, B, M), device=q.device, dtype=torch.float32)
        lvl = torch.empty((2 * B,), device=q.device, dtype=torch.int32)
        L.check(L.load().lic_gain_rows_fwd(_ptr(q), _ptr(T), _ptr(rows), _ptr(lvl), k, Qn, M, B, _stream()),
                "lic_gain_rows_fwd")
        ctx.save_for_backward(rows, lvl)
        ctx.dims = (k, Qn, M, B)
        ctx.set_materialize_grads(False)
        return rows.unbind(0)

    @staticmethod
    def backward(ctx, *d_rows):
        rows, lvl = ctx.saved_tensors
        k, Qn, M, B = ctx.dims
        gs = [None if g is None else g.contiguous() for g in d_rows[:k]]
        if all(g is None for g in gs):
            return (None,) * (1 + k)
        _require_cuda(*gs)
        d_tables = torch.empty((k, Qn, M), device=rows.device, dtype=torch.float32)
        ptrs = [_ptr(g) for g in gs] + [None] * (L.GAIN_ROWS_MAX_TABLES - k)
        L.check(L.load().lic_gain_rows_bwd(_ptr(lvl), _ptr(rows), *ptrs, _ptr(d_tables), k, Qn, M, B, _stream()),
                "lic_gain_rows_bwd")
        return (None, *[d_tables[t] if ctx.needs_input_grad[1 + t] else None for t in range(k)])


def gain_rows_device(q: torch.Tensor, *tables):
    if not 1 <= len(tables) <= L.GAIN_ROWS_MAX_TABLES:
        raise L.LicError(f"1 to {L.GAIN_ROWS_MAX_TABLES} tables expected, got {len(tables)}")
    if not (torch.is_tensor(q) and q.is_cuda and q.dtype == torch.float32 and q.dim() == 1 and q.is_contiguous()):
        raise L.LicError("`q` must be a contiguous CUDA float32 tensor [B]")
    if any(t.dim() != 2 or t.shape != tables[0].shape or t.dtype != torch.float32 for t in tables) or tables[0].shape[0] < 2:
        raise L.LicError("the tables must be float32 [Q >= 2][M] tensors of one shape")
    return _GainRowsFn.apply(q.detach(), *tables)


class _EntropyParamsActFn(torch.autograd.Function):

    @staticmethod
    def forward(ctx, raw, M, K):
        _require_cuda(raw)
        rh = _nhwc(raw)
        B, H, W, CH = rh.shape
        out = torch.empty_like(rh)
        L.check(L.load().lic_entropy_params_fwd(_ptr(rh), _ptr(out), B * H * W, M, K, _stream()),
                "lic_entropy_params_fwd")
        ctx.save_for_backward(rh, out)
        ctx.cfg = (M, K)
        return _nchw_view(out)

    @staticmethod
    def backward(ctx, g):
        rh, out = ctx.saved_tensors
        M, K = ctx.cfg
        gh = _nhwc(g)
        B, H, W, CH = rh.shape
        d = torch.empty_like(rh)
        L.check(L.load().lic_entropy_params_bwd(_ptr(rh), _ptr(out), _ptr(gh), _ptr(d), B * H * W, M, K,
                                                _stream()), "lic_entropy_params_bwd")
        return _nchw_view(d), None, None

# ... 314 lines not shown
```

Measured before the change: 1492 images/s.

## Batch per-layer split-K reduction stages into one fused reduce kernel launch

In each layer's backward pass, wgrad and colsum now run only their partial stage and record a reduce job. All jobs for the layer are then finished by a single multi-job reduce kernel launch. The same mechanism folds the GDN beta/gamma reparameterization backward and the weight-permute copies for image and head convolutions into the reduce epilogue, removing separate kernel launches. The trade-off is that workspaces stay alive longer and correctness depends on the new job descriptors (row-split strides, reparam epilogue) matching the old permute and reparam math.

```diff
diff --git a/include/lic.h b/include/lic.h
--- a/include/lic.h
+++ b/include/lic.h
@@ -469,6 +469,11 @@
 int lic_leaky_bwd_colsum_bf16(const void* y, const void* dy, void* dx, int64_t P, int32_t C, float slope, float* out,
                               void* workspace, size_t workspace_bytes, lic_reduce_job* job, lic_stream_t stream);
 int lic_reduce_batch(const lic_reduce_job* jobs, int32_t njobs, lic_stream_t stream);
+int lic_wgrad_partial(const lic_wgrad_desc* d, void* workspace, size_t workspace_bytes, lic_reduce_job* job,
+                      lic_stream_t stream);
+int lic_colsum_partial(const float* in, int64_t ld, int64_t P, int32_t C, float scale, float* out, void* workspace,
+                       size_t workspace_bytes, lic_reduce_job* job, lic_stream_t stream);
+int lic_reduce_layer(const lic_reduce_job* jobs, int32_t njobs, lic_stream_t stream);
 
 int lic_head_convt_bf16_supported(int32_t Cin, int32_t Cout, int32_t kh, int32_t kw, int32_t stride, int32_t pad,
                                   int32_t out_pad);
diff --git a/neural_image_compression_amd/_lib.py b/neural_image_compression_amd/_lib.py
--- a/neural_image_compression_amd/_lib.py
+++ b/neural_image_compression_amd/_lib.py
@@ -177,6 +177,9 @@
     "lic_colsum_bf16_partial": (C.c_int, [_vp, _i64, _i64, _i32, _f32, _vp, _vp, _sz, C.POINTER(ReduceJob), _vp]),
     "lic_colsum2_bf16_partial": (C.c_int, [_vp, _vp, _i64, _i64, _i32, _f32, _vp, _vp, _vp, _sz, C.POINTER(ReduceJob), _vp]),
     "lic_reduce_batch": (C.c_int, [C.POINTER(ReduceJob), _i32, _vp]),
+    "lic_reduce_layer": (C.c_int, [C.POINTER(ReduceJob), _i32, _vp]),
+    "lic_wgrad_partial": (C.c_int, [C.POINTER(WgradDesc), _vp, _sz, C.POINTER(ReduceJob), _vp]),
+    "lic_colsum_partial": (C.c_int, [_vp, _i64, _i64, _i32, _f32, _vp, _vp, _sz, C.POINTER(ReduceJob), _vp]),
     "lic_colsum2_bf16": (C.c_int, [_vp, _vp, _i64, _i64, _i32, _f32, _vp, _vp, _vp, _sz, _vp]),
     "lic_gdn_dnorm_bf16": (C.c_int, [_vp, _vp, _vp, _vp, _i64, _i32, _vp]),
     "lic_gdn_bwd_bf16_supported": (C.c_int, [_i32]),
diff --git a/neural_image_compression_amd/csrc/lic_elementwise.hip b/neural_image_compression_amd/csrc/lic_elementwise.hip
--- a/neural_image_compression_amd/csrc/lic_elementwise.hip
+++ b/neural_image_compression_amd/csrc/lic_elementwise.hip
@@ -199,8 +199,8 @@
   if (P <= 0 || C <= 0) return 0;
   return (size_t)colsum_chunks(P) * C * sizeof(float);
 }
-LIC_EXPORT int lic_colsum(const float* in, int64_t ld, int64_t P, int32_t C, float scale, float* out,
-                          void* workspace, size_t workspace_bytes, lic_stream_t stream) {
+static int colsum_impl(const float* in, int64_t ld, int64_t P, int32_t C, float scale, float* out, void* workspace,
+                       size_t workspace_bytes, lic_reduce_job* job, lic_stream_t stream) {
   if (!in || !out || !workspace || P <= 0 || C <= 0) return LIC_ERR_INVALID;
   const int nchunk = colsum_chunks(P);
   if (workspace_bytes < (size_t)nchunk * C * sizeof(float)) return LIC_ERR_WORKSPACE;
@@ -213,9 +213,28 @@
                        (float*)workspace, nchunk, vec);
   int rc = lic_check_launch();
   if (rc != LIC_OK) return rc;
+  if (job) {
+    *job = lic_reduce_job{};
+    job->src = (const float*)workspace;
+    job->dst = out;
+    job->kind = LIC_REDUCE_COLUMNS;
+    job->splitk = nchunk;
+    job->Cn = C;
+    job->scale = scale;
+    return LIC_OK;
+  }
   hipLaunchKernelGGL(colsum_stage2, dim3((C + 15) / 16), dim3(256), 0, s, (const float*)workspace, C,
                      nchunk, scale, out);
   return lic_check_launch();
+}
+LIC_EXPORT int lic_colsum(const float* in, int64_t ld, int64_t P, int32_t C, float scale, float* out,
+                          void* workspace, size_t workspace_bytes, lic_stream_t stream) {
+  return colsum_impl(in, ld, P, C, scale, out, workspace, workspace_bytes, nullptr, stream);
+}
+LIC_EXPORT int lic_colsum_partial(const float* in, int64_t ld, int64_t P, int32_t C, float scale, float* out,
+                                  void* workspace, size_t workspace_bytes, lic_reduce_job* job, lic_stream_t stream) {
+  if (!job) return LIC_ERR_INVALID;
+  return colsum_impl(in, ld, P, C, scale, out, workspace, workspace_bytes, job, stream);
 }
 
 template <typename F>
diff --git a/neural_image_compression_amd/csrc/lic_gemm.hip b/neural_image_compression_amd/csrc/lic_gemm.hip
--- a/neural_image_compression_amd/csrc/lic_gemm.hip
+++ b/neural_image_compression_amd/csrc/lic_gemm.hip
@@ -1530,7 +1530,7 @@
   return lic_variant_name(find_variant(d, pl), buf, n);
 }
 static int wgrad_run(const lic_wgrad_desc* d, void* workspace, size_t workspace_bytes, int stage,
-                     lic_stream_t stream) {
+                     lic_stream_t stream, lic_reduce_job* job = nullptr) {
   WgPlan pl;
   int rc = wg_plan(d, &pl);
   if (rc != LIC_OK) return rc;
@@ -1545,6 +1545,22 @@
     rc = lic_check_launch();
     if (rc != LIC_OK) return rc;
   }
+  if (job) {
+    *job = lic_reduce_job{};
+    job->src = (const float*)workspace;
+    job->dst = d->dst;
+    job->kind = LIC_REDUCE_SLABS;
+    job->splitk = pl.splitk;
+    job->ntaps = pl.ntaps;
+    job->Cm = pl.Cm;
+    job->Cn = pl.Cn;
+    job->Mvalid = pl.Cm;
+    job->Nvalid = pl.Cn;
+    job->sm = d->dst_sm;
+    job->sn = d->dst_sn;
+    job->stap = d->dst_stap;
+    job->scale = d->scale;
+  }
   if (stage == 1) return LIC_OK;
   const long total = (long)pl.ntaps * pl.Cm * pl.Cn;
   hipLaunchKernelGGL(wgrad_reduce_kernel, dim3(ew_grid(total, 256)), dim3(256), 0, s,
@@ -1560,6 +1576,11 @@
                                int32_t stage, lic_stream_t stream) {
   if (stage < 0 || stage > 2) return LIC_ERR_INVALID;
   return wgrad_run(d, workspace, workspace_bytes, stage, stream);
+}
+LIC_EXPORT int lic_wgrad_partial(const lic_wgrad_desc* d, void* workspace, size_t workspace_bytes,
+                                 lic_reduce_job* job, lic_stream_t stream) {
+  if (!job) return LIC_ERR_INVALID;
+  return wgrad_run(d, workspace, workspace_bytes, 1, stream, job);
 }
 
 LIC_EXPORT int lic_wgrad_plan(const lic_wgrad_desc* d, int32_t* TM, int32_t* TN, int32_t* splitk) {
diff --git a/neural_image_compression_amd/csrc/lic_gemm_bf16.hip b/neural_image_compression_amd/csrc/lic_gemm_bf16.hip
--- a/neural_image_compression_amd/csrc/lic_gemm_bf16.hip
+++ b/neural_image_compression_amd/csrc/lic_gemm_bf16.hip
@@ -1059,7 +1059,7 @@
   lic_reduce_job j[LIC_REDUCE_MAX_JOBS];
   int n;
 };
-__global__ __launch_bounds__(256) void reduce_batch_kernel(const ReduceTable tb) {
+__device__ __forceinline__ void reduce_table_body(const ReduceTable& tb) {
   int ji = 0;
   while (ji + 1 < tb.n && (int)blockIdx.x >= tb.j[ji + 1].block0) ++ji;
   const lic_reduce_job& q = tb.j[ji];
@@ -1143,7 +1143,9 @@
     }
   }
 }
-LIC_EXPORT int lic_reduce_batch(const lic_reduce_job* jobs, int32_t njobs, lic_stream_t stream) {
+__global__ __launch_bounds__(256) void reduce_batch_kernel(const ReduceTable tb) { reduce_table_body(tb); }
+__global__ __launch_bounds__(256) void reduce_layer_kernel(const ReduceTable tb) { reduce_table_body(tb); }
+static int reduce_launch(const lic_reduce_job* jobs, int32_t njobs, lic_stream_t stream, bool per_layer) {
   if (njobs < 0 || (njobs > 0 && !jobs)) return LIC_ERR_INVALID;
   for (int base = 0; base < njobs; base += LIC_REDUCE_MAX_JOBS) {
     ReduceTable tb;
@@ -1174,9 +1176,16 @@
       blocks += q.nblocks;
       tb.j[i] = q;
     }
-    hipLaunchKernelGGL(reduce_batch_kernel, dim3(blocks), dim3(256), 0, (hipStream_t)stream, tb);
+    hipLaunchKernelGGL(per_layer ? reduce_layer_kernel : reduce_batch_kernel, dim3(blocks), dim3(256), 0,
+                       (hipStream_t)stream, tb);
     const int rc = lic_check_launch();
     if (rc != LIC_OK) return rc;
   }
   return LIC_OK;
 }
+LIC_EXPORT int lic_reduce_batch(const lic_reduce_job* jobs, int32_t njobs, lic_stream_t stream) {
+  return reduce_launch(jobs, njobs, stream, false);
+}
+LIC_EXPORT int lic_reduce_layer(const lic_reduce_job* jobs, int32_t njobs, lic_stream_t stream) {
+  return reduce_launch(jobs, njobs, stream, true);
+}
diff --git a/neural_image_compression_amd/functional.py b/neural_image_compression_amd/functional.py
--- a/neural_image_compression_amd/functional.py
+++ b/neural_image_compression_amd/functional.py
@@ -16,10 +16,12 @@
 FORCE_IGEMM = None
 FORCE_WGRAD = None
 KERNEL_TRACE = None
+FINISH_TRACE = None
 GRAD_VIEWS = {}
 PREPARED = {}
 AUX_STREAM = None
 PLAN_RECORDING = False
+FINISH_BATCHED = True
 
 
 _raw_stream = getattr(torch._C, "_cuda_getCurrentRawStream", None)
@@ -128,7 +130,11 @@
     return nm.value.decode()
 
 
-def _trace(name):
+def _trace(name, finishing=False):
+    if finishing:
+        if FINISH_TRACE is not None:
+            FINISH_TRACE[name] = FINISH_TRACE.get(name, 0) + 1
+        return
     if KERNEL_TRACE is not None:
         KERNEL_TRACE.add(name() if callable(name) else name)
 
@@ -178,8 +184,30 @@
            lambda: L.check(lib.lic_igemm(C.byref(d), _stream()), "lic_igemm"))
 
 
+class _Finish:
+
+    def __init__(self):
+        self.jobs, self.keep = [], []
+
+    def add(self, job, *keep):
+        self.jobs.append(job)
+        self.keep.extend(t for t in keep if t is not None)
+        return job
+
+    def run(self):
+        n = len(self.jobs)
+        if n:
+            _trace("reduce_layer_kernel", finishing=True)
+            L.check(L.load().lic_reduce_layer((L.ReduceJob * n)(*self.jobs), n, _stream()), "lic_reduce_layer")
+        self.jobs, self.keep = [], []
+
+
+def _finish():
+    return _Finish() if FINISH_BATCHED else None
+
+
 def _wgrad(p, g, dst, *, B, Hs, Ws, Cp, Hl, Wl, Cg, kh, kw, stride, pad, g_is_row, dst_sm, dst_sn,
-           dst_stap, sq_p=0, sq_g=0, scale=1.0):
+           dst_stap, sq_p=0, sq_g=0, scale=1.0, fin=None):
     d = _wgrad_desc(p, g, dst, B, Hs, Ws, Cp, Hl, Wl, Cg, kh, kw, stride, pad, g_is_row, dst_sm, dst_sn, dst_stap, sq_p,
                     sq_g, scale)
     lib = L.load()
@@ -188,23 +216,48 @@
     _trace(lambda: _kernel_name(lib.lic_wgrad_kernel_name, d))
     nbytes = lib.lic_wgrad_workspace_bytes(C.byref(d))
     ws = torch.empty((max(nbytes, 4) + 3) // 4, device=p.device, dtype=torch.float32)
+    flops, act_bytes = 2 * B * Hs * Ws * kh * kw * Cp * Cg, 4 * (B * Hs * Ws * Cp + B * Hl * Wl * Cg)
+    if fin is not None:
+        job = L.ReduceJob()
+        _timed(lambda: _kernel_name(lib.lic_wgrad_kernel_name, d), flops, act_bytes,
+               lambda: L.check(lib.lic_wgrad_partial(C.byref(d), _ptr(ws), nbytes, C.byref(job), _stream()),
+                               "lic_wgrad_partial"))
+        return fin.add(job, ws)
+    _trace("wgrad_reduce_kernel", finishing=True)
 
     def stage(k):
         L.check(lib.lic_wgrad_stage(C.byref(d), _ptr(ws), nbytes, k, _stream()), "lic_wgrad_stage")
-    _timed(lambda: _kernel_name(lib.lic_wgrad_kernel_name, d), 2 * B * Hs * Ws * kh * kw * Cp * Cg,
-           4 * (B * Hs * Ws * Cp + B * Hl * Wl * Cg),
+    _timed(lambda: _kernel_name(lib.lic_wgrad_kernel_name, d), flops, act_bytes,
            lambda: L.check(lib.lic_wgrad(C.byref(d), _ptr(ws), nbytes, _stream()), "lic_wgrad"),
            staged=stage)
-
-
-def _colsum(t2d: torch.Tensor, P: int, Cc: int, scale: float = 1.0) -> torch.Tensor:
+    return None
+
+
+def _colsum(t2d: torch.Tensor, P: int, Cc: int, scale: float = 1.0, fin=None, reparam=None) -> torch.Tensor:
     lib = L.load()
     nbytes = lib.lic_colsum_workspace_bytes(P, Cc)
     ws = torch.empty((nbytes + 3) // 4, device=t2d.device, dtype=torch.float32)
     out = torch.empty((Cc,), device=t2d.device, dtype=torch.float32)
+    if fin is not None:
+        job = L.ReduceJob()
+        L.check(lib.lic_colsum_partial(_ptr(t2d), Cc, P, Cc, scale, _ptr(out), _ptr(ws), nbytes, C.byref(job), _stream()),
+                "lic_colsum_partial")
+        if reparam is not None:
+            _reparam_job(job, *reparam)
+        fin.add(job, ws, None if reparam is None else reparam[0])
+        return out
+    _trace("colsum_stage2", finishing=True)
     L.check(lib.lic_colsum(_ptr(t2d), Cc, P, Cc, scale, _ptr(out), _ptr(ws), nbytes, _stream()),
             "lic_colsum")
     return out
+
+
+def _reparam_job(job, param_c, bound):
+    job.epilogue, job.param, job.bound = L.REDUCE_EPI_REPARAM, param_c.data_ptr(), bound
+
+
+def _split_rows_job(job, div, n_valid, s_hi, s_lo, s_col):
+    job.mdiv, job.Mvalid, job.sm, job.smr, job.sn, job.stap = div, n_valid, s_hi, s_lo, s_col, 0
 
 
 def prepared(param: torch.Tensor, kind: str):
@@ -227,6 +280,7 @@
     dgamma = torch.empty_like(gamma_c) if gamma_c is not None else None
     if dbeta is None and dgamma is None:
         return None, None
+    _trace("lic_gdn_reparam_bwd2", finishing=True)
     L.check(L.load().lic_gdn_reparam_bwd2(_ptr(beta_c), _ptr(dbe), _ptr(dbeta), 0 if dbeta is None else dbeta.numel(),
                                           beta_bound, _ptr(gamma_c), _ptr(dge), _ptr(dgamma),
                                           0 if dgamma is None else dgamma.numel(), gamma_bound, _stream()),
@@ -291,7 +345,10 @@
         return dx, dw, db, None, None, None, None, None, None, None, (gy if has_res else None), None
 
 
-def _conv_backward(xh, weight, g, stride, pad, transposed, tap_mask, need_dx, need_dw, need_db):
+def _conv_backward(xh, weight, g, stride, pad, transposed, tap_mask, need_dx, need_dw, need_db, fin=None):
+    own = fin is None
+    if own:
+        fin = _finish()
     B, Hi, Wi, Cin = xh.shape
     _, Ho, Wo, Cout = g.shape
     kh, kw = weight.shape[2], weight.shape[3]
@@ -307,12 +364,14 @@
         taps = kh * kw
         if transposed:
             _wgrad(xh, g, dw, B=B, Hs=Hi, Ws=Wi, Cp=Cin, Hl=Ho, Wl=Wo, Cg=Cout, kh=kh, kw=kw,
-                   stride=stride, pad=pad, g_is_row=False, dst_sm=Cout * taps, dst_sn=taps, dst_stap=1)
+                   stride=stride, pad=pad, g_is_row=False, dst_sm=Cout * taps, dst_sn=taps, dst_stap=1, fin=fin)
         else:
             _wgrad(g, xh, dw, B=B, Hs=Ho, Ws=Wo, Cp=Cout, Hl=Hi, Wl=Wi, Cg=Cin, kh=kh, kw=kw,
-                   stride=stride, pad=pad, g_is_row=True, dst_sm=taps, dst_sn=Cin * taps, dst_stap=1)
+                   stride=stride, pad=pad, g_is_row=True, dst_sm=taps, dst_sn=Cin * taps, dst_stap=1, fin=fin)
     if need_db:
-        db = _bias_grad(g, B * Ho * Wo, Cout)
+        db = _bias_grad(g, B * Ho * Wo, Cout, fin)
+    if own and fin is not None:
+        fin.run()
     return dx, dw, db
 
 
@@ -322,11 +381,11 @@
         dst._lic_colsum_partial = part
 
 
-def _bias_grad(g, P, Cout):
+def _bias_grad(g, P, Cout, fin=None):
     part = getattr(g, "_lic_colsum_partial", None)
     if part is not None and part.shape[1] == Cout:
-        return _colsum(part, part.shape[0], Cout)
-    return _colsum(g, P, Cout)
+        return _colsum(part, part.shape[0], Cout, fin=fin)
+    return _colsum(g, P, Cout, fin=fin)
 
 
 def conv2d(x, weight, bias, stride=1, padding=0, leaky=False, slope=0.01, tap_mask=0, residual=None, out=None):
@@ -413,7 +472,10 @@
     return col, wpk, Ho, Wo, Kp
 
 
-def _image_conv_backward(col, weight, g, stride, pad, in_shape, need_dx, need_dw, need_db):
+def _image_conv_backward(col, weight, g, stride, pad, in_shape, need_dx, need_dw, need_db, fin=None):
+    own = fin is None
+    if own:
+        fin = _finish()
     B, Hi, Wi, Cin = in_shape
     _, Ho, Wo, Cout = g.shape
     _, _, kh, kw = weight.shape
@@ -432,12 +494,19 @@
         dx = _nchw_view(dxh)
     if need_dw:
         dw = grad_like(weight)
-        tmp = torch.empty((Kp, Cout), device=g.device, dtype=torch.float32)
-        _wgrad(col, g, tmp, B=1, Hs=1, Ws=P, Cp=Kp, Hl=1, Wl=P, Cg=Cout, kh=1, kw=1, stride=1, pad=0,
-               g_is_row=False, dst_sm=Cout, dst_sn=1, dst_stap=0)
-        _permute3(tmp, dw, (taps, Cin, Cout), (Cin * Cout, Cout, 1), (1, taps, Cin * taps))
+        if fin is not None:
+            job = _wgrad(col, g, dw, B=1, Hs=1, Ws=P, Cp=Kp, Hl=1, Wl=P, Cg=Cout, kh=1, kw=1, stride=1, pad=0,
+                         g_is_row=False, dst_sm=Cout, dst_sn=1, dst_stap=0, fin=fin)
+            _split_rows_job(job, Cin, taps * Cin, 1, taps, Cin * taps)
+        else:
+            tmp = torch.empty((Kp, Cout), device=g.device, dtype=torch.float32)
+            _wgrad(col, g, tmp, B=1, Hs=1, Ws=P, Cp=Kp, Hl=1, Wl=P, Cg=Cout, kh=1, kw=1, stride=1, pad=0,
+                   g_is_row=False, dst_sm=Cout, dst_sn=1, dst_stap=0)
+            _permute3(tmp, dw, (taps, Cin, Cout), (Cin * Cout, Cout, 1), (1, taps, Cin * taps))
     if need_db:
-        db = _bias_grad(g, P, Cout)
+        db = _bias_grad(g, P, Cout, fin)
+    if own and fin is not None:
+        fin.run()
     return dx, dw, db
 
 
@@ -499,10 +568,13 @@
         col, weight, conv_out, norm, beta, gamma = ctx.saved_tensors
         stride, pad, in_shape, inverse, beta_bound, gamma_bound, has_bias, pedestal = ctx.cfg
         need = ctx.needs_input_grad
+        fin = _finish()
         g_conv, dbeta, dgamma = _gdn_backward(conv_out, norm, beta, gamma, _nhwc(gy), inverse,
-                                              beta_bound, gamma_bound, pedestal, True, need[3], need[4])
+                                              beta_bound, gamma_bound, pedestal, True, need[3], need[4], fin=fin)
         dx, dw, db = _image_conv_backward(col, weight, g_conv, stride, pad, in_shape, need[0], need[1],
-                                          has_bias and need[2])
+                                          has_bias and need[2], fin=fin)
+        if fin is not None:
+            fin.run()
         return dx, dw, db, dbeta, dgamma, None, None, None, None, None, None, None
 
 
@@ -545,6 +617,7 @@
         L.check(lib.lic_im2col(_ptr(g), _ptr(dcol), B, Ho, Wo, Cout, Hi, Wi, kh, kw, stride, pad, Kp,
                                _stream()), "lic_im2col")
         dx = dw = db = None
+        fin = _finish()
         if ctx.needs_input_grad[0]:
             wpk = prepared(weight, "f32.head_dx")
             if wpk is None:
@@ -558,12 +631,19 @@
             dx = _nchw_view(dxh)
         if ctx.needs_input_grad[1]:
             dw = grad_like(weight)
-            tmp = torch.empty((Cin, Kp), device=g.device, dtype=torch.float32)
-            _wgrad(xh, dcol, tmp, B=1, Hs=1, Ws=P, Cp=Cin, Hl=1, Wl=P, Cg=Kp, kh=1, kw=1, stride=1, pad=0,
-                   g_is_row=True, dst_sm=1, dst_sn=Kp, dst_stap=0)
-            _permute3(tmp, dw, (Cin, taps, Cout), (Kp, Cout, 1), (Cout * taps, 1, taps))
+            if fin is not None:
+                job = _wgrad(xh, dcol, dw, B=1, Hs=1, Ws=P, Cp=Cin, Hl=1, Wl=P, Cg=Kp, kh=1, kw=1, stride=1, pad=0,
+                             g_is_row=True, dst_sm=1, dst_sn=Kp, dst_stap=0, fin=fin)
+                _split_rows_job(job, Cout, taps * Cout, 1, taps, Cout * taps)
+            else:
+                tmp = torch.empty((Cin, Kp), device=g.device, dtype=torch.float32)
+                _wgrad(xh, dcol, tmp, B=1, Hs=1, Ws=P, Cp=Cin, Hl=1, Wl=P, Cg=Kp, kh=1, kw=1, stride=1, pad=0,
+                       g_is_row=True, dst_sm=1, dst_sn=Kp, dst_stap=0)
+                _permute3(tmp, dw, (Cin, taps, Cout), (Kp, Cout, 1), (Cout * taps, 1, taps))
         if has_bias and ctx.needs_input_grad[2]:
-            db = _colsum(g, B * Ho * Wo, Cout)
+            db = _colsum(g, B * Ho * Wo, Cout, fin=fin)
+        if fin is not None:
+            fin.run()
         return dx, dw, db, None, None, None
 
 
@@ -668,8 +748,12 @@
 
 
 def _gdn_backward(xh, norm, beta, gamma, g, inverse, beta_bound, gamma_bound, pedestal, need_dx, need_dbeta,
-                  need_dgamma):
+                  need_dgamma, fin=None):
     lib = L.load()
+    own = fin is None
+    if own:
+        fin = _finish()
+    rp_beta = rp_gamma = None
     B, H, W, Cc = xh.shape
     P = B * H * W
     t = torch.empty_like(xh)
@@ -677,6 +761,8 @@
     cs_dx = None
     dbe = None
     beta_c, gamma_c = beta.contiguous(), gamma.contiguous()
+    if fin is not None:
+        rp_beta, rp_gamma = (beta_c, beta_bound), (gamma_c, gamma_bound)
     gp = _gdn_gamma_packed(gamma, gamma_bound, pedestal) if need_dx else None
     if need_dx and lib.lic_gdn_supported(Cc):
         dxh = torch.empty_like(xh)
@@ -688,7 +774,7 @@
                lambda: L.check(lib.lic_gdn_bwd(_ptr(g), _ptr(xh), _ptr(norm), _ptr(gp), _ptr(dxh), _ptr(t), _ptr(pt),
                                                _ptr(pdx), P, Cc, int(inverse), _stream()), "lic_gdn_bwd"))
         if need_dbeta:
-            dbe = _colsum(pt, rows, Cc)
+            dbe = _colsum(pt, rows, Cc, fin=fin, reparam=rp_beta)
         cs_dx = pdx
     elif need_dx and Cc % 4 == 0:
         dxh = torch.empty_like(xh)
@@ -705,13 +791,21 @@
                    aux=g, aux2=xh, aux3=norm)
     dge = None
     if need_dbeta and dbe is None:
-        dbe = _colsum(t, P, Cc)
+        dbe = _colsum(t, P, Cc, fin=fin, reparam=rp_beta)
     if need_dgamma:
         dge = torch.empty_like(gamma_c)
-        _wgrad(t, xh, dge, B=1, Hs=1, Ws=P, Cp=Cc, Hl=1, Wl=P, Cg=Cc, kh=1, kw=1, stride=1, pad=0,
-               g_is_row=False, dst_sm=Cc, dst_sn=1, dst_stap=0, sq_g=1)
-    dbeta, dgamma = _reparam_bwd2(beta_c if need_dbeta else None, dbe, beta_bound,
-                                  gamma_c if need_dgamma else None, dge, gamma_bound)
+        job = _wgrad(t, xh, dge, B=1, Hs=1, Ws=P, Cp=Cc, Hl=1, Wl=P, Cg=Cc, kh=1, kw=1, stride=1, pad=0,
+                     g_is_row=False, dst_sm=Cc, dst_sn=1, dst_stap=0, sq_g=1, fin=fin)
+        if job is not None:
+            _reparam_job(job, *rp_gamma)
+            fin.keep.append(gamma_c)
+    if fin is not None:
+        dbeta, dgamma = dbe, dge
+        if own:
+            fin.run()
+    else:
+        dbeta, dgamma = _reparam_bwd2(beta_c if need_dbeta else None, dbe, beta_bound,
+                                      gamma_c if need_dgamma else None, dge, gamma_bound)
     if cs_dx is not None and dxh is not None:
         dxh._lic_colsum_partial = cs_dx
     return dxh, dbeta, dgamma
@@ -746,10 +840,13 @@
         xh, weight, conv_out, norm, beta, gamma = ctx.saved_tensors
         stride, pad, transposed, inverse, beta_bound, gamma_bound, has_bias, pedestal = ctx.cfg
         need = ctx.needs_input_grad
+        fin = _finish()
         g_conv, dbeta, dgamma = _gdn_backward(conv_out, norm, beta, gamma, _nhwc(gy), inverse,
-                                              beta_bound, gamma_bound, pedestal, True, need[3], need[4])
+                                              beta_bound, gamma_bound, pedestal, True, need[3], need[4], fin=fin)
         dx, dw, db = _conv_backward(xh, weight, g_conv, stride, pad, transposed, 0, need[0], need[1],
-                                    has_bias and need[2])
+                                    has_bias and need[2], fin=fin)
+        if fin is not None:
+            fin.run()
         return dx, dw, db, dbeta, dgamma, None, None, None, None, None, None, None, None, None
 
 
```

New measurement: 1497 images/s (median of 6 runs). About the same (+0.3%).
